# lopunch/CWBNWP-LETKF

Measured on AMD Instinct MI355X. Metric: analysis grid-points/sec (+ wall-clock per cycle) at k=40, 1/2/4/8 MI355X, higher is better.
Workload: dtype f64

## Files before the change

cwbnwp-letkf_amd/csrc/cwbl_abi.hip:

```cpp
#include "../../include/cwb_letkf_core.h"
#include "cwbl_internal.h"

#include <hip/hip_runtime.h>

#include <algorithm>
#include <chrono>
#include <condition_variable>
#include <functional>
#include <mutex>
#include <thread>
#include <cmath>
#include <cstdarg>
#include <cstdio>
#include <cstdlib>
#include <cstring>
#include <memory>
#include <string>
#include <vector>

namespace cwbl {
namespace {

std::string g_err;

// ... 112 lines not shown
      (*fn_)(i);
    }
  }
  void loop(unsigned long seen) {
    for (;;) {
      {
        std::unique_lock<std::mutex> lk(mu_);
        cv_.wait(lk, [&] { return gen_ != seen; });
        seen = gen_;
        if (quit_) return;
      }
      work();
      {
        std::lock_guard<std::mutex> lk(mu_);
        if (--busy_ == 0) done_.notify_all();
      }
    }
  }
  std::vector<std::thread> th_;
  std::mutex mu_;
  std::condition_variable cv_, done_;
  const std::function<void(int)> *fn_ = nullptr;
  int n_ = 0, next_ = 0, busy_ = 0;
  unsigned long gen_ = 0;
  bool quit_ = false;
};

struct ObsType {
  int family = 0, type_id = 0, nvar = 1, nobs = 0;
  std::vector<float> xyz;
  DevBuf obs, error, hdxb, qc;
  DevBuf dxyz;
  bool dxyz_ok = false;
};

struct TreeBufs {
  int entry = -1, dim = 0, depth = 0;
  int bin_div_opt = 0;
  float hinv = 0.0f, vinv = 0.0f;
  DevBuf nodes, rdata, ind, col_bg, col_omm, col_err, col_ok;
  DevBuf bxyz, bstart;
  HostTree host;
  HostBins bins;
  int mode = 0;
  int n = 0, bin_div_used = 0;
  DevBuf ncoord;
  IndexBounds bounds{};
  std::thread worker;
  bool worker_started = false, worker_joined = false, tree_ready = false;
  double worker_ms = 0.0;
  void join() {
    if (worker.joinable()) worker.join();
    worker_joined = worker_started;
  }
  void release() {
    join();
    nodes.release(); rdata.release(); ind.release(); col_bg.release();
    col_omm.release(); col_err.release(); col_ok.release(); bxyz.release(); bstart.release();
    ncoord.release();
  }
  ~TreeBufs() { join(); }
};

enum KernelId {
  KT_SEARCH_BINNED, KT_SEARCH_FLAGGED, KT_SEARCH_TREE, KT_ASSEMBLE_RECORD, KT_SOLVE_TQ40,
  KT_SOLVE_TQ40_MULTI, KT_SOLVE_TQ40_COLUMN, KT_FILL_TQ40_FACTOR, KT_SOLVE_TQ40_FACTOR, KT_SOLVE_TQ_MULTI2, KT_SOLVE_TQ_MULTI4, KT_SOLVE_TQ_MULTI8,
  KT_BIG_HANDOFF, KT_TQB_TAIL, KT_BIG_HANDOFF_MULTI2, KT_BIG_HANDOFF_MULTI4,
  KT_BIG_HANDOFF_MULTI8, KT_TQB_TAIL_MULTI2, KT_TQB_TAIL_MULTI4, KT_TQB_TAIL_MULTI8,
  KT_SOLVE_TQ, KT_SOLVE_TQ_BIG, KT_SOLVE_JACOBI, KT_TUNE_Q,
  KT_COUNT
};
struct KTime { long long launches = 0, points = 0; double ms = 0.0; };

struct RecordKey {
  unsigned long long gen;
  float multi_infl;
  int dims[7];
  cwbl_type_params gts[CWBL_NUM_GTS_TYPES], radar[CWBL_NUM_RADAR_TYPES];
};
struct RecordCache {
  bool valid = false;
  RecordKey key{};
  DevBuf rec, aux, info, sx, sy, salt, flag;
  PinBuf hflag;
  std::vector<std::pair<long long, int>> plan;
  std::vector<size_t> off;
  long long pts = 0;
  size_t nxy = 0, nalt = 0;
  int nt = 0, list_cap = 0;
  long long lz_truncated = 0, q1_undefined = 0;
  size_t bytes() const { return rec.n + aux.n + info.n + sx.n + sy.n + salt.n + flag.n; }
  void release() {
    valid = false;
    for (DevBuf *b : {&rec, &aux, &info, &sx, &sy, &salt, &flag}) b->release();
    hflag.release();
    plan.clear();
    off.clear();
    pts = 0;
  }
};

struct State {
  bool inited = false;
  int k = 0, kp = 0, device = 0, wf = 0, q1_mode = 0;
  int kp_natural = 0;
  float norain = -5.0f;
  size_t ws_bytes = size_t(2) << 30;
  hipStream_t stream = nullptr;
  std::vector<ObsType> obs;
  bool have_obs = false;
  std::vector<std::unique_ptr<TreeBufs>> tree_cache;
  DevBuf tdesc, nbr_cnt, nbr_idx, info, stats;
  DevBuf nbr_cnt2, nbr_idx2;
  hipStream_t sstream = nullptr;
  std::vector<hipEvent_t> cevents;
  int lead_div = 0;
  bool serial_search = false;
  long long max_batch = 160000;
  bool max_batch_set = false;
  long long info_window = 1LL << 25;
  DevBuf sx, sy, salt, svar;
  DevBuf bcol, byo, byb, bxb, bxa, bev, btri;
  DevBuf qxyz, qnf, qidx, qr2;
  DevBuf quad;
  DevBuf wsa;
  DevBuf flags;
  int index_mode = 0;
  DevBuf tdesc_tree;
  DevBuf ix_keys[2], ix_vals[2], ix_hist, ix_part;
  PinBuf ix_pin;
  std::vector<hipEvent_t> pevents;
  bool binned = true;
  int bin_div = 0;
  bool pageable_register = true;
  bool jacobi = false;
  int tq4 = 1;
  long long tq4_sub = 0;
  bool big_split = true;
  long long big_sub = 98304;
  std::vector<hipEvent_t> events;
  hipStream_t h2d = nullptr, d2h = nullptr;
  hipStream_t caller_stream = nullptr;
  hipEvent_t order_ev = nullptr;
  bool ktiming = false;
  KTime ktime[KT_COUNT];
  std::vector<hipEvent_t> kevents;
  int kev_used = 0;
  struct KPend { int id; hipEvent_t e0, e1; long long pts; };
  std::vector<KPend> kpend;
  size_t handoff_budget = 0;
  unsigned long long gen = 0;
  size_t reuse_budget = 0;
  bool factor_reuse = true;
  int column_share = 0;
  int column_levels = 0;
  int ncu = 0;
  RecordCache cache;
  static constexpr int kSlots = 3;
  PinBuf pin_in[kSlots], pin_out[kSlots];
  HostPool pool;
};

State S;

float search_r2() {
  const float gc1999 = 2.0f * std::sqrt(10.0f / 3.0f);
  return gc1999 * gc1999;
}

bool is_gts_assimilated(int id) {
  return id == CWBL_GTS_SYNOP || id == CWBL_GTS_METAR || id == CWBL_GTS_SHIPS ||
         id == CWBL_GTS_SOUND || id == CWBL_GTS_GPSPW;
}

int tree_depth(const HostTree &t, int node = 0) {
  if (t.nodes.empty()) return 0;
  int depth = 0;
  std::vector<std::pair<int, int>> st{{node, 1}};
  while (!st.empty()) {
    auto [nd, lv] = st.back();
    st.pop_back();
    depth = std::max(depth, lv);
    if (t.nodes[nd].cut_dim >= 0) {
      st.push_back({t.nodes[nd].left, lv + 1});
      st.push_back({t.nodes[nd].right, lv + 1});
    }
  }
  return depth;
}

hipError_t stage(DevBuf &dst, const void *src, size_t bytes, int memory) {
  hipError_t e = dst.ensure(bytes);
  if (e != hipSuccess || bytes == 0) return e;
  return hipMemcpyAsync(dst.p, src, bytes,
                        memory == CWBL_MEM_DEVICE ? hipMemcpyDeviceToDevice
                                                  : hipMemcpyHostToDevice,
                        S.stream);
}

hipError_t cevent(int i, hipEvent_t *out) {
  while ((int)S.cevents.size() <= i) {
    hipEvent_t e;
    hipError_t r = hipEventCreateWithFlags(&e, hipEventDisableTiming);
    if (r != hipSuccess) return r;
    S.cevents.push_back(e);
  }
  *out = S.cevents[i];
  return hipSuccess;
}

hipError_t event(int i, hipEvent_t *out) {
  while ((int)S.events.size() <= i) {
    hipEvent_t e;
    hipError_t r = hipEventCreate(&e);
    if (r != hipSuccess) return r;
    S.events.push_back(e);
  }
  *out = S.events[i];
  return hipSuccess;
}

float elapsed(int a, int b) {
  float ms = 0.0f;
  if (hipEventElapsedTime(&ms, S.events[a], S.events[b]) != hipSuccess) return 0.0f;
  return ms;
}

hipError_t kt_event(int i, hipEvent_t *out) {
  while ((int)S.kevents.size() <= i) {
    hipEvent_t e;
    hipError_t r = hipEventCreate(&e);
    if (r != hipSuccess) return r;
    S.kevents.push_back(e);
  }
  *out = S.kevents[i];
  return hipSuccess;
}

hipError_t kt_begin(hipStream_t s, int *ev) {
  *ev = -1;
  if (!S.ktiming) return hipSuccess;
  hipEvent_t e;
  hipError_t r = kt_event(S.kev_used, &e);
  if (r != hipSuccess) return r;
  *ev = S.kev_used;
  S.kev_used += 2;
  return hipEventRecord(e, s);
}

hipError_t kt_end(hipStream_t s, int ev, int id, long long pts) {
  if (ev < 0) return hipSuccess;
  hipEvent_t e;
  hipError_t r = kt_event(ev + 1, &e);
  if (r != hipSuccess) return r;
  S.kpend.push_back({id, S.kevents[ev], e, pts});
  return hipEventRecord(e, s);
}

hipError_t kt_pair(hipStream_t s, hipEvent_t e0, int id0, long long pts0, hipEvent_t e1,
                   int id1, long long pts1, const std::function<hipError_t()> &first,
                   const std::function<hipError_t()> &second) {
  hipError_t r = first();
  if (r != hipSuccess) return r;
  if (S.ktiming) {
    hipEvent_t mid;
    r = kt_event(S.kev_used++, &mid);
    if (r != hipSuccess) return r;
    r = hipEventRecord(mid, s);
    if (r != hipSuccess) return r;
    S.kpend.push_back({id0, e0, mid, pts0});
    S.kpend.push_back({id1, mid, e1, pts1});
  }
  return second();
}

void kt_collect() {
  for (const State::KPend &p : S.kpend) {
    float ms = 0.0f;
    if (hipEventElapsedTime(&ms, p.e0, p.e1) != hipSuccess) continue;
    KTime &t = S.ktime[p.id];
    t.launches += 1;
    t.points += p.pts;
    t.ms += ms;
  }
  S.kpend.clear();
  S.kev_used = 0;
}

std::string kernel_name(int id) {
  const std::string kp = std::to_string(S.kp);
  switch (id) {
    case KT_SEARCH_BINNED: return "search_binned_kernel";
    case KT_SEARCH_FLAGGED: return "search_kernel<FlagQuery>";
    case KT_SEARCH_TREE: return "search_kernel<SlabQuery>";
    case KT_ASSEMBLE_RECORD: return "assemble_record_kernel<" + std::to_string(kRecordWaves) + ">";
    case KT_SOLVE_TQ40: return "solve_tq40_kernel<" + kp + ", 0>";
    case KT_SOLVE_TQ40_MULTI: return "solve_tq40_multi_kernel<" + kp + ">";
    case KT_SOLVE_TQ40_COLUMN: return "solve_tq40_column_kernel<" + kp + ">";
    case KT_FILL_TQ40_FACTOR: return "fill_tq40_factor_kernel<" + kp + ">";
    case KT_SOLVE_TQ40_FACTOR: return "solve_tq40_factor_kernel<" + kp + ">";
    case KT_BIG_HANDOFF:
      return S.kp == 128 ? "solve_tq_rows_kernel<128, 64>"
                         : "solve_tq_big_kernel<" + kp + ", false, " +
                               std::to_string(big_split_j0(S.kp)) + ">";
    case KT_TQB_TAIL:
      return "solve_tqb_tail_kernel<" + kp + ", " + std::to_string(big_split_j0(S.kp)) +
// ... 249 lines not shown
}

int build_family(int family, const cwbl_var_params *vp, std::vector<TreeDesc> &descs,
                 int &list_cap, int &max_depth, std::vector<TreeBufs *> &tbs) {
  struct Pending { int entry; int type_id; const cwbl_type_params *tp; float hinv, vinv; };
  std::vector<Pending> pend;
  const int ntypes = family == 0 ? CWBL_NUM_GTS_TYPES : CWBL_NUM_RADAR_TYPES;
  for (int id = 1; id <= ntypes; ++id) {
    int entry = -1;
    for (size_t e = 0; e < S.obs.size(); ++e)
      if (S.obs[e].family == family && S.obs[e].type_id == id) entry = (int)e;
    if (entry < 0 || S.obs[entry].nobs <= 0) continue;
    if (family == 0 && !is_gts_assimilated(id)) continue;
    const cwbl_type_params *tp = family == 0 ? &vp->gts[id - 1] : &vp->radar[id - 1];
    if (!(tp->use_it && tp->hclr > 0.0f)) continue;
    if (tp->max_lz_pts < 0) return fail(CWBL_ERR_ARG, "max_lz_pts < 0 for type %d", id);
    const float hinv = 1.0f / (tp->hclr * 1e3f);
    const float vinv = tp->vclr > 0.0f ? 1.0f / (tp->vclr * 1e3f) : -1.0f;
    pend.push_back({entry, id, tp, hinv, vinv});
  }
  if (pend.empty()) return CWBL_OK;
  const bool fam3d = pend.back().vinv > 0.0f;
  for (const Pending &pd : pend) {
    ObsType &ot = S.obs[pd.entry];
    const bool own3d = pd.vinv > 0.0f;
    bool dim3 = S.q1_mode == CWBL_Q1_PER_TYPE ? own3d : fam3d;
    int q1u = 0;
    if (dim3 && !own3d) { dim3 = false; q1u = 1; }
    const int n = ot.nobs;
    const int tdim = dim3 ? 3 : 2;
    TreeBufs *tb = nullptr;
    if (S.index_mode == 1) {
      if (int rc = index_entry(pd.entry, tdim, dim3, pd.hinv, pd.vinv, pd.tp->max_lz_pts, tb))
        return rc;
    }
    for (auto &t : S.tree_cache)
      if (S.index_mode == 0 && t->mode == 0 && t->entry == pd.entry && t->dim == tdim &&
          t->hinv == pd.hinv && (!dim3 || t->vinv == pd.vinv) && t->bin_div_opt == S.bin_div)
        tb = t.get();
    if (!tb) {
      std::vector<float> nx(3 * (size_t)n);
      for (int j = 0; j < n; ++j) {
        nx[3 * j + 0] = ot.xyz[3 * j + 0] * pd.hinv;
        nx[3 * j + 1] = ot.xyz[3 * j + 1] * pd.hinv;
        nx[3 * j + 2] = dim3 ? ot.xyz[3 * j + 2] * pd.vinv : -1.0f;
      }
      auto nt = std::make_unique<TreeBufs>();
      nt->entry = pd.entry; nt->dim = tdim; nt->hinv = pd.hinv; nt->vinv = pd.vinv;
      nt->bin_div_opt = S.bin_div;
      nt->n = n;
      const auto t_tree = std::chrono::steady_clock::now();
      build_kdtree(nx.data(), n, tdim, nt->host);
      nt->depth = tree_depth(nt->host);
      P.ms_tree += ms_since(t_tree);
      ++P.trees_built;
      if (nt->depth >= kSearchStackDepth)
        return fail(CWBL_ERR_UNSUPPORTED, "k-d tree too deep (%d obs)", n);
      const HostTree &h = nt->host;
      HIPCHK(nt->nodes.ensure(h.nodes.size() * sizeof(TreeNode)));
      HIPCHK(nt->rdata.ensure(h.rdata.size() * sizeof(float)));
      HIPCHK(nt->ind.ensure(h.ind.size() * sizeof(int) + 4));
      HIPCHK(hipMemcpyAsync(nt->nodes.p, h.nodes.data(), h.nodes.size() * sizeof(TreeNode),
                            hipMemcpyHostToDevice, S.stream));
      HIPCHK(hipMemcpyAsync(nt->rdata.p, h.rdata.data(), h.rdata.size() * sizeof(float),
                            hipMemcpyHostToDevice, S.stream));
      if (!h.ind.empty())
        HIPCHK(hipMemcpyAsync(nt->ind.p, h.ind.data(), h.ind.size() * sizeof(int),
                              hipMemcpyHostToDevice, S.stream));
      const auto t_bins = std::chrono::steady_clock::now();
      build_bins(h, tdim, std::sqrt(search_r2()), nt->bins, bin_div_for(h, tdim));
      P.ms_bins += ms_since(t_bins);
      ++P.bins_built;
      const HostBins &hb = nt->bins;
      HIPCHK(nt->bxyz.ensure(hb.xyzs.size() * sizeof(float) + 16 * kBinPad));
      HIPCHK(nt->bstart.ensure(hb.start.size() * sizeof(int)));
      if (!hb.xyzs.empty())
        HIPCHK(hipMemcpyAsync(nt->bxyz.p, hb.xyzs.data(), hb.xyzs.size() * sizeof(float),
                              hipMemcpyHostToDevice, S.stream));
      HIPCHK(hipMemcpyAsync(nt->bstart.p, hb.start.data(), hb.start.size() * sizeof(int),
                            hipMemcpyHostToDevice, S.stream));
      tb = nt.get();
      S.tree_cache.push_back(std::move(nt));
    }
    const size_t ncol = (size_t)n * ot.nvar;
    HIPCHK(tb->col_bg.ensure(ncol * S.kp * sizeof(float)));
    HIPCHK(tb->col_omm.ensure(ncol * sizeof(float)));
    HIPCHK(tb->col_err.ensure(ncol * sizeof(float)));
    HIPCHK(tb->col_ok.ensure(ncol));
    const cwbl_type_params *tp = pd.tp;
    int is_assim[5] = {0, 0, 0, 0, 0};
    if (family == 0) {
      for (int v = 0; v < ot.nvar; ++v) is_assim[v] = tp->hclr > 0.0f ? tp->is_assim[v] : 0;
    } else {
      is_assim[0] = tp->hclr > 0.0f ? 1 : 0;
    }
    HIPCHK(prep_begin(S.stream, 1));
    HIPCHK(launch_obs_prep(S.stream, S.k, S.kp, family, ot.type_id, ot.nvar, n,
                           ot.obs.as<float>(), ot.error.as<float>(), ot.hdxb.as<float>(),
                           ot.qc.as<int>(), tp->err_muti, tp->err_rej, is_assim, S.norain,
                           tb->mode == 1 ? nullptr : tb->ind.as<int>(), tb->col_bg.as<float>(),
                           tb->col_omm.as<float>(), tb->col_err.as<float>(),
                           tb->col_ok.as<uint8_t>()));
    HIPCHK(prep_end(S.stream));
    TreeDesc d{};
    if (tb->mode == 1) {
      d.rdata = tb->ncoord.as<float4>();
    } else {
      d.nodes = tb->nodes.as<TreeNode>();
      d.rdata = tb->rdata.as<float4>();
      d.ind = tb->ind.as<int>();
    }
    d.col_bg = tb->col_bg.as<float>();
    d.col_omm = tb->col_omm.as<float>();
    d.col_err = tb->col_err.as<float>();
    d.col_ok = tb->col_ok.as<uint8_t>();
    d.hclr_inv = pd.hinv;
    d.vclr_inv = pd.vinv;
    d.tree_dim = dim3 ? 3 : 2;
    d.query3d = own3d ? 1 : 0;
    d.nvar = ot.nvar;
    d.max_lz = tp->max_lz_pts;
    d.list_off = list_cap;
    d.q1_undef = q1u;
    d.bxyz = tb->bxyz.as<float4>();
    d.bstart = tb->bstart.as<int>();
    d.bx0 = tb->bins.x0; d.by0 = tb->bins.y0; d.bz0 = tb->bins.z0; d.binv = tb->bins.binv;
    d.nbx = tb->bins.nbx; d.nby = tb->bins.nby; d.nbz = tb->bins.nbz;
    list_cap += list_span(tp->max_lz_pts);
    if (tb->mode == 0) max_depth = std::max(max_depth, tb->depth);
    descs.push_back(d);
    tbs.push_back(tb);
  }
  return CWBL_OK;
}

void release_obs() {
  for (auto &t : S.tree_cache) t->release();
  S.tree_cache.clear();
  for (auto &o : S.obs) {
    o.obs.release(); o.error.release(); o.hdxb.release(); o.qc.release(); o.dxyz.release();
  }
  S.obs.clear();
  S.have_obs = false;
}

void release_all() {
  release_obs();
  for (hipEvent_t e : S.cevents) (void)hipEventDestroy(e);
  S.cevents.clear();
  for (DevBuf *b : {&S.tdesc, &S.nbr_cnt, &S.nbr_idx, &S.nbr_cnt2, &S.nbr_idx2, &S.info, &S.stats, &S.sx,
                    &S.sy, &S.salt, &S.svar, &S.bcol, &S.byo, &S.byb, &S.bxb, &S.bxa, &S.bev, &S.btri,
                    &S.qxyz, &S.qnf, &S.qidx, &S.qr2, &S.quad, &S.wsa, &S.flags, &S.tdesc_tree,
                    &S.ix_keys[0], &S.ix_keys[1], &S.ix_vals[0], &S.ix_vals[1], &S.ix_hist,
                    &S.ix_part})
    b->release();
  S.ix_pin.release();
  S.cache.release();
  for (hipEvent_t e : S.pevents) (void)hipEventDestroy(e);
  S.pevents.clear();
  g_pspans.clear();
  g_pev_used = 0;
  for (hipEvent_t e : S.events) (void)hipEventDestroy(e);
  S.events.clear();
  for (hipEvent_t e : S.kevents) (void)hipEventDestroy(e);
  S.kevents.clear();
  for (int i = 0; i < State::kSlots; ++i) {
    S.pin_in[i].release();
    S.pin_out[i].release();
  }
  S.pool.stop();
  S.kpend.clear();
  S.kev_used = 0;
  S.ktiming = false;
  for (KTime &t : S.ktime) t = KTime{};
  if (S.order_ev) (void)hipEventDestroy(S.order_ev);
  S.order_ev = nullptr;
  S.caller_stream = nullptr;
  if (S.stream) (void)hipStreamDestroy(S.stream);
  S.stream = nullptr;
  if (S.sstream) (void)hipStreamDestroy(S.sstream);
  S.sstream = nullptr;
  for (hipStream_t *st : {&S.h2d, &S.d2h}) {
    if (*st) (void)hipStreamDestroy(*st);
    *st = nullptr;
  }
  S.inited = false;
}

void select_kp() {
  S.kp = S.kp_natural;
  if ((S.kp == 24 || S.kp == 32) && S.tq4 && !S.jacobi) S.kp = kTq4KP;
}

SolveConsts solve_consts(float inflat, int use_rtpp, float rtpp_a, int use_rtps, float rtps_a) {
  SolveConsts c{};
  c.k = S.k;
  c.kp = S.kp;
  c.weight_function = S.wf;
  c.inflat = inflat;
  c.use_rtpp = use_rtpp;
  c.use_rtps = use_rtps;
  c.rtpp_alpha = rtpp_a;
  c.rtps_alpha = rtps_a;
  c.nmember_inv = 1.0f / (float)S.k;
  c.r2 = search_r2();
  c.max_sweeps = 30;
  c.quad_r = S.quad.as<double2>();
  c.quad = c.quad_r;
#ifdef CWBL_DEBUG_KNOBS
  if (const char *e = std::getenv("CWBL_DEBUG_MAX_SWEEPS")) c.max_sweeps = std::atoi(e);
  if (const char *e = std::getenv("CWBL_DEBUG_TQ_STOP")) c.debug_stop = std::atoi(e);
  if (const char *e = std::getenv("CWBL_DEBUG_TQ_STEPS")) c.debug_steps = std::atoi(e);
#endif
  return c;
}

struct VarCall {
  const cwbl_var_params *vp = nullptr;
  const cwbl_slab *sl = nullptr;
  int nvar = 1;
  bool group = false;
  Tq40Vars tv{};
  long long npts = 0, L = 0;
  SlabDev sd{};
  size_t bvar = 0;
  bool host = false, piped = false, piped_back = false, bounce = false, registered = false;
  std::vector<TreeDesc> descs;
  std::vector<TreeBufs *> tbs;
  bool index1 = false, trees_ready = false;
  int list_cap = 0, max_depth = 1, nt = 0;
  std::vector<std::pair<long long, int>> plan;
  long long B = 0, Bc = 0, info_cap = 0, win0 = 0;
  SolveConsts c{};
  float rbox = 0.0f;
  int ev = 4, cev = 0;
  std::vector<std::pair<int, int>> search_ev, solve_ev;
  std::vector<int> done_ev, h2d_done, d2h_done;
  int reuse = 0;
  long long ncached = 0;
  bool full_hit = false;
  int colshare = 0, nlev = 1, lev = 1;
  long long ncol = 0;
  SlabDev full{};
};

bool record_path() { return S.tq4 && S.kp == kTq4KP && !S.jacobi; }
bool wave_path() { return !record_path() && S.kp <= kMaxWaveKP && !S.jacobi; }
bool handoff_path() {
  return (S.kp == 96 || S.kp == kBigSplitKP) && S.big_split && S.k > big_split_j0(S.kp) + 2;
}

void make_record_key(RecordKey &key, const cwbl_var_params *vp, const cwbl_slab *sl) {
  std::memset(&key, 0, sizeof key);
  key.gen = S.gen;
  key.multi_infl = vp->multi_infl;
  const int dims[7] = {sl->nx, sl->ny, sl->nz, sl->alt_nx, sl->alt_ny, sl->ix_lim, sl->iy_lim};
  std::memcpy(key.dims, dims, sizeof dims);
  std::memcpy(key.gts, vp->gts, sizeof key.gts);
  std::memcpy(key.radar, vp->radar, sizeof key.radar);
}

int coords_match(VarCall &v, bool &same) {
  RecordCache &C = S.cache;
  const auto t0 = std::chrono::steady_clock::now();
  int *flag = C.flag.as<int>();
  HIPCHK(hipMemsetAsync(flag, 0, sizeof(int), S.stream));
  HIPCHK(launch_coord_snapshot(S.stream, false, v.sd.x, C.sx.as<float>(), (long long)C.nxy, flag));
  HIPCHK(launch_coord_snapshot(S.stream, false, v.sd.y, C.sy.as<float>(), (long long)C.nxy, flag));
  HIPCHK(launch_coord_snapshot(S.stream, false, v.sd.alt, C.salt.as<float>(), (long long)C.nalt,
                               flag));
  HIPCHK(hipMemcpyAsync(C.hflag.p, flag, sizeof(int), hipMemcpyDeviceToHost, S.stream));
  HIPCHK(hipStreamSynchronize(S.stream));
  same = *C.hflag.as<int>() == 0;
  R.ms_compare = ms_since(t0);
  return CWBL_OK;
}

int begin_fill(VarCall &v, const RecordKey &key) {
  RecordCache &C = S.cache;
  C.valid = false;
  C.key = key;
  C.plan = v.plan;
  C.off.clear();
  C.pts = 0;
  size_t words = 0;
  for (const auto &b : v.plan) {
    const size_t need = ((size_t)b.second + 1) * AsmRecord<kTq4KP>::WORDS;
    if ((words + need) * sizeof(double) > S.reuse_budget) break;
    C.off.push_back(words);
    words += need;
    C.pts += b.second;
  }
  if (C.off.empty()) return CWBL_OK;
  const cwbl_slab *sl = v.sl;
  C.nxy = (size_t)sl->nx * sl->ny;
  C.nalt = (size_t)sl->alt_nx * sl->alt_ny * sl->nz;
  const size_t need = words * sizeof(double);
  bool ok = need <= C.rec.n ||
            C.rec.ensure(std::min(S.reuse_budget, need + need / 16)) == hipSuccess;
  if (S.factor_reuse) {
    const size_t aneed =
        words / AsmRecord<kTq4KP>::WORDS * FactorAux<kTq4KP>::WORDS * sizeof(double);
    ok = ok && (aneed <= C.aux.n || C.aux.ensure(aneed + aneed / 16) == hipSuccess);
  } else {
    C.aux.release();
  }
  ok = ok && C.info.ensure((size_t)C.pts * sizeof(int2)) == hipSuccess;
  ok = ok && C.sx.ensure(C.nxy * 4) == hipSuccess && C.sy.ensure(C.nxy * 4) == hipSuccess;
  ok = ok && C.salt.ensure(C.nalt * 4) == hipSuccess && C.flag.ensure(sizeof(int)) == hipSuccess;
  ok = ok && C.hflag.ensure(64) == hipSuccess;
  if (!ok) {
    (void)hipGetLastError();
    C.release();
    return CWBL_OK;
  }
  HIPCHK(launch_coord_snapshot(S.stream, true, v.sd.x, C.sx.as<float>(), (long long)C.nxy, nullptr));
  HIPCHK(launch_coord_snapshot(S.stream, true, v.sd.y, C.sy.as<float>(), (long long)C.nxy, nullptr));
  HIPCHK(launch_coord_snapshot(S.stream, true, v.sd.alt, C.salt.as<float>(), (long long)C.nalt,
                               nullptr));
  v.reuse = 1;
  v.ncached = (long long)C.off.size();
  return CWBL_OK;
}

int restore_info(VarCall &v, long long g) {
  const long long n = std::min<long long>(v.info_cap, S.cache.pts - g);
  if (v.reuse != 2 || n <= 0) return CWBL_OK;
  HIPCHK(hipMemcpyAsync(S.info.p, S.cache.info.as<int2>() + g, (size_t)n * sizeof(int2),
                        hipMemcpyDeviceToDevice, S.stream));
  return CWBL_OK;
}

int keep_info(VarCall &v, long long end) {
  const long long n = std::min<long long>(end, S.cache.pts) - v.win0;
  if (v.reuse != 1 || n <= 0) return CWBL_OK;
  HIPCHK(hipMemcpyAsync(S.cache.info.as<int2>() + v.win0, S.info.p, (size_t)n * sizeof(int2),
                        hipMemcpyDeviceToDevice, S.stream));
  return CWBL_OK;
}

int ready_trees(VarCall &v, hipStream_t s) {
  if (v.trees_ready) return CWBL_OK;
  std::vector<TreeDesc> sd = v.descs;
  for (size_t i = 0; i < sd.size(); ++i) {
    TreeBufs *tb = v.tbs[i];
    if (!tb->worker_started) continue;
    if (int rc = ready_tree(tb, s)) return rc;
    sd[i].nodes = tb->nodes.as<TreeNode>();
    sd[i].rdata = tb->rdata.as<float4>();
    sd[i].ind = tb->ind.as<int>();
    v.max_depth = std::max(v.max_depth, tb->depth);
  }
  HIPCHK(S.tdesc_tree.ensure(sd.size() * sizeof(TreeDesc)));
  HIPCHK(hipMemcpyAsync(S.tdesc_tree.p, sd.data(), sd.size() * sizeof(TreeDesc),
                        hipMemcpyHostToDevice, s));
  HIPCHK(hipStreamSynchronize(s));
  v.trees_ready = true;
  return CWBL_OK;
}

int plan_trees(VarCall &v) {
  v.index1 = S.index_mode == 1;
  if (int rc = build_family(0, v.vp, v.descs, v.list_cap, v.max_depth, v.tbs)) return rc;
  if (int rc = build_family(1, v.vp, v.descs, v.list_cap, v.max_depth, v.tbs)) return rc;
  v.nt = (int)v.descs.size();
  if (v.nt == 0 || v.npts == 0) return CWBL_OK;
  HIPCHK(S.tdesc.ensure(v.descs.size() * sizeof(TreeDesc)));
  HIPCHK(hipMemcpyAsync(S.tdesc.p, v.descs.data(), v.descs.size() * sizeof(TreeDesc),
                        hipMemcpyHostToDevice, S.stream));
  if (v.index1 && !S.binned)
    if (int rc = ready_trees(v, S.stream)) return rc;
  return CWBL_OK;
}

int stage_slab(VarCall &v) {
  const cwbl_slab *sl = v.sl;
  v.L = (long long)sl->nx * sl->ny * sl->nz;
  SlabDev &sd = v.sd;
  sd.nx = sl->nx; sd.ny = sl->ny; sd.nz = sl->nz; sd.alt_nx = sl->alt_nx;
  sd.alt_ny = sl->alt_ny; sd.ix_lim = sl->ix_lim; sd.iy_lim = sl->iy_lim; sd.L = v.L;
  const size_t bxy = (size_t)sl->nx * sl->ny * 4;
  const size_t balt = (size_t)sl->alt_nx * sl->alt_ny * sl->nz * 4;
  v.bvar = (size_t)v.L * S.k * 4;
  v.host = sl->memory != CWBL_MEM_DEVICE;
  const bool whole = v.group || v.colshare;
  v.piped = !whole && v.host && sl->ix_lim == sl->nx && sl->iy_lim == sl->ny;
  v.piped_back = v.piped && !v.vp->tune_q;
  v.bounce = !whole && v.host && v.bvar > 0 && !host_pinned(sl->var);
  if (v.bounce && S.pageable_register) {
    if (hipHostRegister(sl->var, v.bvar, hipHostRegisterDefault) == hipSuccess) {
      v.registered = true;
      v.bounce = false;
    } else {
      (void)hipGetLastError();
    }
  }
  if (!v.host) {
    sd.x = sl->x; sd.y = sl->y; sd.alt = sl->alt;
    for (int i = 0; i < v.nvar; ++i) v.tv.var[i] = v.sl[i].var;
  } else {
    HIPCHK(stage(S.sx, sl->x, bxy, CWBL_MEM_HOST));
    HIPCHK(stage(S.sy, sl->y, bxy, CWBL_MEM_HOST));
    HIPCHK(stage(S.salt, sl->alt, balt, CWBL_MEM_HOST));
    sd.x = S.sx.as<float>(); sd.y = S.sy.as<float>(); sd.alt = S.salt.as<float>();
    HIPCHK(S.svar.ensure(v.bvar * (size_t)v.nvar));
    for (int i = 0; i < v.nvar; ++i) {
      v.tv.var[i] = S.svar.as<float>() + (size_t)i * (size_t)v.L * S.k;
      if (v.bvar > 0 && !v.piped && !v.bounce)
        HIPCHK(hipMemcpyAsync(v.tv.var[i], v.sl[i].var, v.bvar, hipMemcpyHostToDevice, S.stream));
    }
  }
  sd.var = v.tv.var[0];
  return CWBL_OK;
}

void plan_batches(VarCall &v) {
  const long long npts = v.npts;
  const size_t per_pt = (size_t)v.list_cap * 4 + (size_t)v.nt * 4 + 8;
  long long B = (long long)(S.ws_bytes / per_pt);
  B = std::min<long long>(B, S.max_batch);
  if (!S.max_batch_set) B = std::min<long long>(B, std::max<long long>(npts / 6, 64000));
  B = std::max<long long>(std::min<long long>(B, npts), 256);
  B = std::min<long long>(B, 1 << 22);
  if (v.list_cap > 0)
    B = std::min<long long>(B, (long long)((((size_t)1 << 32) - 1) / ((size_t)v.list_cap * 4)) /
                                   kListLanes * kListLanes);
  const auto round_up = [](long long x) { return (x + kListLanes - 1) / kListLanes * kListLanes; };
  long long lead = S.lead_div > 0 ? round_up(npts / S.lead_div) : 0;
  if (lead < 4 * kListLanes || lead >= npts) lead = 0;
  if (lead > 0) v.plan.push_back({0, (int)std::min<long long>(lead, B)});
  const long long g1 = v.plan.empty() ? 0 : v.plan[0].second, rest = npts - g1;
  const long long nrest = (rest + B - 1) / B;
  const long long Br = round_up((rest + nrest - 1) / nrest);
  for (long long g = g1; g < npts; g += Br)
    v.plan.push_back({g, (int)std::min<long long>(Br, npts - g)});
  v.B = 0;
  for (const auto &b : v.plan) v.B = std::max<long long>(v.B, b.second);
  v.Bc = std::min<long long>(std::max<long long>(v.B, 1), std::max<long long>(v.L, 1));
  v.info_cap = std::max<long long>(v.B, std::min<long long>(npts, S.info_window));
}

int bounce_whole(VarCall &v, bool up) {
  std::vector<int> evs;
  long long pc0 = 0;
  int pcn = 0;
  const size_t pitch = (size_t)v.L * 4;
  float *const hvar = v.sl->var;
  for (long long c0 = 0, i = 0; c0 < v.L; c0 += v.Bc, ++i) {
    const int cn = (int)std::min<long long>(v.Bc, v.L - c0);
    PinBuf &slot = up ? S.pin_in[i & 1] : S.pin_out[i & 1];
    hipEvent_t e;
    HIPCHK(cevent(v.cev, &e));
    if (up) {
      if (i >= 2) HIPCHK(hipEventSynchronize(S.cevents[evs[(size_t)i - 2]]));
      bounce_rows(S.pool, slot.as<float>(), hvar, v.L, c0, cn, S.k, true);
      HIPCHK(hipMemcpy2DAsync(S.svar.as<float>() + c0, pitch, slot.p, (size_t)cn * 4,
                              (size_t)cn * 4, (size_t)S.k, hipMemcpyHostToDevice, S.stream));
    } else {
      HIPCHK(hipMemcpy2DAsync(slot.p, (size_t)cn * 4, S.svar.as<float>() + c0, pitch,
                              (size_t)cn * 4, (size_t)S.k, hipMemcpyDeviceToHost, S.stream));
    }
    HIPCHK(hipEventRecord(e, S.stream));
    evs.push_back(v.cev++);
    if (!up && i >= 1) {
      HIPCHK(hipEventSynchronize(S.cevents[evs[(size_t)i - 1]]));
      bounce_rows(S.pool, S.pin_out[(i - 1) & 1].as<float>(), hvar, v.L, pc0, pcn, S.k, false);
    }
    pc0 = c0;
    pcn = cn;
  }
  if (!up && !evs.empty()) {
    HIPCHK(hipEventSynchronize(S.cevents[evs.back()]));
    bounce_rows(S.pool, S.pin_out[(evs.size() - 1) & 1].as<float>(), hvar, v.L, pc0, pcn,
                S.k, false);
  }
  return CWBL_OK;
}

int bounce_fill(VarCall &v, long long b) {
  if (b >= State::kSlots) HIPCHK(hipEventSynchronize(S.cevents[v.h2d_done[b - State::kSlots]]));
  bounce_rows(S.pool, S.pin_in[b % State::kSlots].as<float>(), v.sl->var, v.L, v.plan[b].first,
              v.plan[b].second, S.k, true);
  return CWBL_OK;
}

int bounce_drain(VarCall &v, long long b) {
  HIPCHK(hipEventSynchronize(S.cevents[v.d2h_done[b]]));
  bounce_rows(S.pool, S.pin_out[b % State::kSlots].as<float>(), v.sl->var, v.L, v.plan[b].first,
              v.plan[b].second, S.k, false);
  return CWBL_OK;
}

int stage_bounce(VarCall &v) {
  if (v.registered) {
    for (int i = 0; i < State::kSlots; ++i) {
      S.pin_in[i].release();
      S.pin_out[i].release();
    }
  }
  if (!v.bounce) return CWBL_OK;
  const size_t slot_bytes = (size_t)v.Bc * S.k * 4;
  const int nin = v.piped ? State::kSlots : 2, nout = v.piped_back ? State::kSlots : 2;
  for (int i = 0; i < nin; ++i) HIPCHK(S.pin_in[i].ensure(slot_bytes));
  for (int i = 0; i < nout; ++i) HIPCHK(S.pin_out[i].ensure(slot_bytes));
  if (!v.piped) return bounce_whole(v, true);
  return CWBL_OK;
}

int alloc_call_buffers(VarCall &v) {
  const long long B = v.B;
  const size_t bytes_cnt = (size_t)B * v.nt * 4;
  const size_t bytes_idx =
      (size_t)((B + kListLanes - 1) / kListLanes) * kListLanes * std::max(v.list_cap, 1) * 4;
  HIPCHK(S.nbr_cnt.ensure(bytes_cnt));
  HIPCHK(S.nbr_idx.ensure(bytes_idx));
  if (v.plan.size() > 1) {
    HIPCHK(S.nbr_cnt2.ensure(bytes_cnt));
    HIPCHK(S.nbr_idx2.ensure(bytes_idx));
  }
  HIPCHK(S.flags.ensure((size_t)(B + 1) * sizeof(int)));
  HIPCHK(S.stats.ensure(sizeof(DevStats)));
  HIPCHK(hipMemsetAsync(S.stats.p, 0, sizeof(DevStats), S.stream));
  HIPCHK(S.info.ensure((size_t)v.info_cap * sizeof(int2)));
  v.c = solve_consts((float)(S.k - 1) / v.vp->multi_infl,
                     v.vp->use_rtpp, v.vp->rtpp_alpha, v.vp->use_rtps, v.vp->rtps_alpha);
  v.c.ntrees = v.nt;
  v.c.list_cap = v.list_cap;
  v.rbox = std::sqrt(search_r2()) * 1.0001f + 1e-5f;
  return CWBL_OK;
}

int search_batch(VarCall &v, long long bi, int *ncnt, int *nidx, hipEvent_t a, hipEvent_t b) {
  const long long g0 = v.plan[bi].first;
  const int nb = v.plan[bi].second;
  const TreeDesc *dtrees = S.tdesc.as<TreeDesc>();
  DevStats *dst = S.stats.as<DevStats>();
  hipStream_t ss = S.serial_search ? S.stream : S.sstream;
  if (bi >= 2) HIPCHK(hipStreamWaitEvent(ss, S.events[v.done_ev[bi - 2]], 0));
  HIPCHK(hipEventRecord(a, ss));
  int kt;
  if (S.binned) {
    int *fcnt = S.flags.as<int>(), *fidx = fcnt + 1;
    HIPCHK(hipMemsetAsync(fcnt, 0, sizeof(int), ss));
    HIPCHK(kt_begin(ss, &kt));
    HIPCHK(launch_search_binned(ss, dtrees, v.nt, v.list_cap, v.c.r2, v.rbox, v.sd, g0, nb, ncnt,
                                nidx, fcnt, fidx));
    HIPCHK(kt_end(ss, kt, KT_SEARCH_BINNED, nb));
    if (v.index1) {
      HIPCHK(S.ix_pin.ensure(64));
      int *hcnt = S.ix_pin.as<int>();
      HIPCHK(hipMemcpyAsync(hcnt, fcnt, sizeof(int), hipMemcpyDeviceToHost, ss));
      HIPCHK(hipStreamSynchronize(ss));
      if (*hcnt > 0) {
        ++P.flagged_batches;
        if (int rc = ready_trees(v, ss)) return rc;
        HIPCHK(kt_begin(ss, &kt));
        HIPCHK(launch_search_flagged(ss, S.tdesc_tree.as<TreeDesc>(), v.nt, v.max_depth,
                                     v.list_cap, v.c.r2, v.sd, g0, nb, fcnt, fidx, ncnt, nidx,
                                     dst, true));
        HIPCHK(kt_end(ss, kt, KT_SEARCH_FLAGGED, 0));
      }
    } else {
      HIPCHK(kt_begin(ss, &kt));
      HIPCHK(launch_search_flagged(ss, dtrees, v.nt, v.max_depth, v.list_cap, v.c.r2, v.sd, g0,
                                   nb, fcnt, fidx, ncnt, nidx, dst));
      HIPCHK(kt_end(ss, kt, KT_SEARCH_FLAGGED, 0));
    }
  } else if (v.index1) {
    HIPCHK(kt_begin(ss, &kt));
    HIPCHK(launch_search(ss, S.tdesc_tree.as<TreeDesc>(), v.nt, v.max_depth, v.list_cap, v.c.r2,
                         v.sd, g0, nb, ncnt, nidx, nullptr, dst, true));
    HIPCHK(kt_end(ss, kt, KT_SEARCH_TREE, nb));
  } else {
    HIPCHK(kt_begin(ss, &kt));
    HIPCHK(launch_search(ss, dtrees, v.nt, v.max_depth, v.list_cap, v.c.r2, v.sd, g0, nb, ncnt,
                         nidx, nullptr, dst));
    HIPCHK(kt_end(ss, kt, KT_SEARCH_TREE, nb));
  }
  return hipEventRecord(b, ss) == hipSuccess ? CWBL_OK
                                              : fail(CWBL_ERR_HIP, "search event record failed");
}

int upload_batch_var(VarCall &v, long long bi) {
  const long long g0 = v.plan[bi].first;
  const int nb = v.plan[bi].second;
  hipEvent_t hv;
  const int hv_i = v.cev++;
  HIPCHK(cevent(hv_i, &hv));
  const size_t pitch = (size_t)v.L * 4;
  if (v.bounce) {
    if (bi == 0)
      if (int rc = bounce_fill(v, 0)) return rc;
    HIPCHK(hipMemcpy2DAsync(S.svar.as<float>() + g0, pitch, S.pin_in[bi % State::kSlots].p,
                            (size_t)nb * 4, (size_t)nb * 4, (size_t)S.k, hipMemcpyHostToDevice,
                            S.h2d));
  } else {
    HIPCHK(hipMemcpy2DAsync(S.svar.as<float>() + g0, pitch, v.sl->var + g0, pitch,
                            (size_t)nb * 4, (size_t)S.k, hipMemcpyHostToDevice, S.h2d));
  }
  HIPCHK(hipEventRecord(hv, S.h2d));
  v.h2d_done.push_back(hv_i);
  HIPCHK(hipStreamWaitEvent(S.stream, hv, 0));
  return CWBL_OK;
}

int return_batch_var(VarCall &v, long long bi, hipEvent_t dn) {
  const long long g0 = v.plan[bi].first;
  const int nb = v.plan[bi].second;
  HIPCHK(hipStreamWaitEvent(S.d2h, dn, 0));
  const size_t pitch = (size_t)v.L * 4;
  if (v.bounce) {
    hipEvent_t dv;
    const int dv_i = v.cev++;
    HIPCHK(cevent(dv_i, &dv));
    HIPCHK(hipMemcpy2DAsync(S.pin_out[bi % State::kSlots].p, (size_t)nb * 4,
                            S.svar.as<float>() + g0, pitch, (size_t)nb * 4, (size_t)S.k,
                            hipMemcpyDeviceToHost, S.d2h));
    HIPCHK(hipEventRecord(dv, S.d2h));
    v.d2h_done.push_back(dv_i);
  } else {
    HIPCHK(hipMemcpy2DAsync(v.sl->var + g0, pitch, S.svar.as<float>() + g0, pitch,
                            (size_t)nb * 4, (size_t)S.k, hipMemcpyDeviceToHost, S.d2h));
  }
  return CWBL_OK;
}

long long sub_batch(int nb, long long cap) {
  const long long nsub = (nb + cap - 1) / cap;
  const long long Bs = (nb + nsub - 1) / nsub;
  return std::max<long long>(kListLanes, (Bs + kListLanes - 1) / kListLanes * kListLanes);
}

int solve_batch_path(VarCall &v, long long g0, int nb, const int *ncnt, const int *nidx,
                     int2 *infob, hipEvent_t b2, hipEvent_t dn, double *crec = nullptr,
                     bool hit = false, double *caux = nullptr) {
  const TreeDesc *dtrees = S.tdesc.as<TreeDesc>();
  const SolveConsts &c = v.c;
  const SlabDev &sd = v.sd;
  const int nt = v.nt, list_cap = v.list_cap;
  int kt;
  const bool handoff = handoff_path();
  if (record_path()) {
    const long long cap = std::min<long long>(S.tq4_sub > 0 ? S.tq4_sub : nb, 1 << 19);
    const long long Bs = std::min<long long>(sub_batch(nb, cap), 1 << 19);
    if (!crec) HIPCHK(S.wsa.ensure((size_t)(Bs + 1) * 8 * AsmRecord<kTq4KP>::WORDS));
    double *rec = crec ? crec : S.wsa.as<double>();
    const size_t rstep = crec ? AsmRecord<kTq4KP>::WORDS : 0;
    const bool factor = crec && S.factor_reuse && !v.group;
    const int kt_solve = factor ? (hit ? KT_SOLVE_TQ40_FACTOR : KT_FILL_TQ40_FACTOR)
                         : v.group ? KT_SOLVE_TQ40_MULTI : KT_SOLVE_TQ40;
    auto solve = [&](long long g, int n, double *r, int2 *inf) {
      if (factor) {
        double *const ax = caux + (size_t)(r - rec) / rstep * FactorAux<kTq4KP>::WORDS;
        return hit ? launch_solve_tq40_factor(S.stream, S.kp, c, sd, g, n, r, ax, inf)
                   : launch_fill_tq40_factor(S.stream, S.kp, c, sd, g, n, r, ax, inf);
      }
      return v.group ? launch_solve_tq40_multi(S.stream, S.kp, c, sd, v.tv, g, n, r, inf)
                     : launch_solve_tq40(S.stream, S.kp, c, sd, g, n, r, inf);
    };
    if (Bs >= nb && hit) {
      if (S.ktiming) S.kpend.push_back({kt_solve, b2, dn, nb});
      HIPCHK(solve(g0, nb, rec, infob));
      return CWBL_OK;
    }
    if (Bs >= nb) {
      auto asm_ = [&]() {
        return launch_assemble_record(S.stream, S.kp, dtrees, c, sd, g0, nb, ncnt, nidx, infob,
                                      rec);
      };
      auto tq40 = [&]() { return solve(g0, nb, rec, infob); };
      HIPCHK(kt_pair(S.stream, b2, KT_ASSEMBLE_RECORD, nb, dn, kt_solve, nb, asm_, tq40));
      return CWBL_OK;
    }
    for (long long s0 = 0; s0 < nb; s0 += Bs) {
      const int ns = (int)std::min<long long>(Bs, nb - s0);
      double *const srec = rec + (size_t)s0 * rstep;
      if (!hit) {
        HIPCHK(kt_begin(S.stream, &kt));
        HIPCHK(launch_assemble_record(S.stream, S.kp, dtrees, c, sd, g0 + s0, ns,
                                      ncnt + s0 * nt, nidx + s0 * list_cap, infob + s0, srec));
        HIPCHK(kt_end(S.stream, kt, KT_ASSEMBLE_RECORD, ns));
      }
      HIPCHK(kt_begin(S.stream, &kt));
      HIPCHK(solve(g0 + s0, ns, srec, infob + s0));
      HIPCHK(kt_end(S.stream, kt, kt_solve, ns));
    }
    return CWBL_OK;
  }
  if (handoff) {
    const int nv = v.group ? group_var_class(v.nvar) : 1;
    const size_t rec_bytes = 8 * big_handoff_words(S.kp, nv);
// ... 144 lines not shown
      if (n > 1)
        HIPCHK(launch_solve_tq40_multi(S.stream, S.kp, v.c, v.sd, v.tv, g0 + s0, ns, rec, inf));
      else
        HIPCHK(launch_solve_tq40(S.stream, S.kp, v.c, v.sd, g0 + s0, ns, rec, inf));
      HIPCHK(kt_end(S.stream, kt, n > 1 ? KT_SOLVE_TQ40_MULTI : KT_SOLVE_TQ40, (long long)ns * n));
    }
  }
  return CWBL_OK;
}

int finish_call(VarCall &v, cwbl_stats &st) {
  DevStats *dst = S.stats.as<DevStats>();
  if (v.npts > v.win0) {
    HIPCHK(launch_reduce_info(S.stream, S.info.as<int2>(), (int)(v.npts - v.win0), dst));
    if (int rc = keep_info(v, v.npts)) return rc;
  }
  int ev = v.ev;
  for (int i = 0; i < v.nvar; ++i) {
    if (!v.vp[i].tune_q) continue;
    hipEvent_t a, b;
    HIPCHK(event(ev, &a));
    HIPCHK(event(ev + 1, &b));
    HIPCHK(hipEventRecord(a, S.stream));
    SlabDev sdi = v.colshare ? v.full : v.sd;
    sdi.var = v.tv.var[i];
    int kt;
    HIPCHK(kt_begin(S.stream, &kt));
    HIPCHK(launch_tune_q(S.stream, sdi, S.k));
    HIPCHK(kt_end(S.stream, kt, KT_TUNE_Q, v.npts * v.nlev));
    HIPCHK(hipEventRecord(b, S.stream));
    v.solve_ev.push_back({ev, ev + 1});
    ev += 2;
  }
  hipEvent_t e_end, e_back;
  HIPCHK(event(ev, &e_end));
  HIPCHK(event(ev + 1, &e_back));
  if (v.host && !v.piped_back && !v.bounce)
    for (int i = 0; i < v.nvar; ++i)
      HIPCHK(hipMemcpyAsync(v.sl[i].var, v.tv.var[i], v.bvar, hipMemcpyDeviceToHost, S.stream));
  if (v.piped_back) {
    HIPCHK(hipEventRecord(e_back, S.d2h));
    HIPCHK(hipStreamWaitEvent(S.stream, e_back, 0));
  }
  const long long nbat = (long long)v.plan.size();
  if (v.bounce && v.piped_back)
    for (long long bj = std::max<long long>(0, nbat - (State::kSlots - 1)); bj < nbat; ++bj)
      if (int rc = bounce_drain(v, bj)) return rc;
  if (v.bounce && !v.piped_back)
    if (int rc = bounce_whole(v, false)) return rc;
  HIPCHK(hipEventRecord(e_end, S.stream));
  DevStats ds;
  HIPCHK(hipMemcpyAsync(&ds, S.stats.p, sizeof ds, hipMemcpyDeviceToHost, S.stream));
  HIPCHK(hipStreamSynchronize(S.stream));
  kt_collect();
  prep_collect();

  const long long lev = v.nlev;
  st.solved = (long long)ds.solved * lev;
  st.nobs_sum = (long long)ds.nobs_sum * lev;
  st.lz_truncated = v.reuse == 2 ? S.cache.lz_truncated : (long long)ds.lz_truncated * lev;
  st.nonconverged = (long long)ds.nonconverged * lev;
  st.sweeps_sum = (long long)ds.sweeps_sum * lev;
  st.max_p = (int)ds.max_p;
  st.max_sweeps = (int)ds.max_sweeps;
  st.ms_prep = elapsed(0, 1);
  for (auto &p : v.search_ev) st.ms_search += elapsed(p.first, p.second);
  for (auto &p : v.solve_ev) st.ms_solve += elapsed(p.first, p.second);
  st.ms_copy = elapsed(1, 2) + (v.host && !v.piped_back ? elapsed(ev - 1, ev) : 0.0f);
  if (v.bounce) st.ms_copy = g_bounce_ms;
  return CWBL_OK;
}

}

int set_last_error(int code, const char *msg) {
  g_err = msg;
  return code;
}

}

using namespace cwbl;

extern "C" {

int cwbl_abi_version(void) { return CWBL_ABI_VERSION; }

const char *cwbl_last_error(void) { return g_err.c_str(); }

int cwbl_init(const cwbl_init_params *p) {
  if (!p) return fail(CWBL_ERR_ARG, "cwbl_init: null params");
  if (S.inited) release_all();
  if (p->nmember < 2) return fail(CWBL_ERR_ARG, "nmember must be >= 2 (got %d)", p->nmember);
  const int kp = supported_kp(p->nmember);
  if (kp < 0)
    return fail(CWBL_ERR_UNSUPPORTED, "nmember %d > %d not supported by this build",
                p->nmember, CWBL_MAX_MEMBERS);
  int ndev = 0;
  if (hipGetDeviceCount(&ndev) != hipSuccess || ndev == 0)
    return fail(CWBL_ERR_NO_DEVICE, "no HIP device available (the core has no CPU path)");
  int dev = p->device;
  if (dev < 0) HIPCHK(hipGetDevice(&dev));
  if (dev >= ndev) return fail(CWBL_ERR_NO_DEVICE, "device %d >= device count %d", dev, ndev);
  HIPCHK(hipSetDevice(dev));
  hipDeviceProp_t prop;
  HIPCHK(hipGetDeviceProperties(&prop, dev));
  if (std::strncmp(prop.gcnArchName, "gfx950", 6) != 0)
    return fail(CWBL_ERR_NO_DEVICE, "device %d is %s; this library is built for gfx950", dev,
                prop.gcnArchName);
  if (p->weight_function != 0 && p->weight_function != 1)
    return fail(CWBL_ERR_ARG, "weight_function must be 0 or 1");
  S.k = p->nmember;
  S.kp = kp;
  S.device = dev;
  S.wf = p->weight_function;
  S.norain = p->norain_value;
  S.q1_mode = p->q1_mode;
  S.ws_bytes = p->workspace_bytes ? p->workspace_bytes : (size_t(2) << 30);
  size_t fr = 0, tot = 0;
  HIPCHK(hipMemGetInfo(&fr, &tot));
  if (p->workspace_bytes) {
    S.handoff_budget = p->workspace_bytes;
  } else {
    S.handoff_budget = std::min<size_t>((size_t)13 << 30, fr / 10 * 4);
  }
  S.reuse_budget = std::min<size_t>((size_t)40 << 30, fr / 10 * 4);
  ++S.gen;
  HIPCHK(hipStreamCreateWithFlags(&S.stream, hipStreamNonBlocking));
  HIPCHK(hipStreamCreateWithFlags(&S.sstream, hipStreamNonBlocking));
  HIPCHK(hipStreamCreateWithFlags(&S.h2d, hipStreamNonBlocking));
  HIPCHK(hipStreamCreateWithFlags(&S.d2h, hipStreamNonBlocking));
  {
    std::vector<double2> tab((size_t)4 * kQuadLevels * kQuadStride);
    const int rounds[4] = {2, 3, 4, 8};
    for (int r = 0; r < 4; ++r)
      for (int l = 1; l <= kQuadLevels; ++l)
        quad_table(l, &tab[((size_t)r * kQuadLevels + (l - 1)) * kQuadStride],
                   8 * rounds[r] - 1);
    HIPCHK(S.quad.ensure(tab.size() * sizeof(double2)));
    HIPCHK(hipMemcpy(S.quad.p, tab.data(), tab.size() * sizeof(double2), hipMemcpyHostToDevice));
  }
  S.jacobi = false;
  S.tq4 = 1;
  S.tq4_sub = 0;
  S.big_split = true;
  S.big_sub = 98304;
  S.binned = true;
  S.pageable_register = true;
  S.bin_div = 0;
  S.index_mode = 0;
  S.column_share = 0;
  S.column_levels = 0;
  S.factor_reuse = true;
  S.ncu = prop.multiProcessorCount;
  std::memset(&P, 0, sizeof P);
  std::memset(&CI, 0, sizeof CI);
  S.lead_div = 0;
  S.serial_search = false;
#ifdef CWBL_DEBUG_KNOBS
  if (const char *e = std::getenv("CWBL_DEBUG_SERIAL")) S.serial_search = std::atoi(e) != 0;
#endif
  S.kp_natural = kp;
  select_kp();
  S.max_batch = 160000;
  S.max_batch_set = false;
  S.info_window = 1LL << 25;
  S.inited = true;
  return CWBL_OK;
}

int cwbl_set_option(int option, long long value) {
  if (!S.inited) return fail(CWBL_ERR_STATE, "cwbl_set_option before cwbl_init");
  auto range = [&](long long lo, long long hi) { return value >= lo && value <= hi; };
  ++S.gen;
  switch (option) {
    case CWBL_OPT_SOLVER:
      if (!range(0, 1)) break;
      if (value == 1 && S.kp_natural > kMaxWaveKP)
        return fail(CWBL_ERR_UNSUPPORTED, "the Jacobi solver supports k <= %d", kMaxWaveKP);
      S.jacobi = value == 1;
      select_kp();
      return CWBL_OK;
    case CWBL_OPT_SPLIT40:
      if (!range(0, 1)) break;
      S.tq4 = (int)value;
      select_kp();
      return CWBL_OK;
    case CWBL_OPT_SPLIT40_BATCH:
      if (!range(0, 1 << 19)) break;
      S.tq4_sub = value;
      return CWBL_OK;
    case CWBL_OPT_SEARCH:
      if (!range(0, 1)) break;
      S.binned = value == 0;
      return CWBL_OK;
    case CWBL_OPT_BIG_PATH:
      if (!range(0, 1)) break;
      S.big_split = value == 1;
      return CWBL_OK;
    case CWBL_OPT_BIG_BATCH:
      if (!range(64, 1LL << 24)) break;
      S.big_sub = value;
      return CWBL_OK;
    case CWBL_OPT_PAGEABLE:
      if (!range(0, 1)) break;
      S.pageable_register = value == 0;
      return CWBL_OK;
    case CWBL_OPT_BIN_DIV:
      if (!range(0, 8)) break;
      S.bin_div = (int)value;
      return CWBL_OK;
    case CWBL_OPT_LEAD_DIV:
      if (!range(0, 1 << 20)) break;
      S.lead_div = (int)value;
      return CWBL_OK;
    case CWBL_OPT_MAX_BATCH:
      if (value != 0 && !range(256, 1LL << 31)) break;
      S.max_batch = value ? value : 160000;
      S.max_batch_set = value != 0;
      return CWBL_OK;
    case CWBL_OPT_INFO_WINDOW:
      if (value != 0 && !range(256, 1LL << 30)) break;
      S.info_window = value ? value : (1LL << 25);
      return CWBL_OK;
    case CWBL_OPT_INDEX:
      if (!range(0, 1)) break;
      S.index_mode = (int)value;
      return CWBL_OK;
    case CWBL_OPT_COLUMN_SHARE:
      if (!range(0, 2)) break;
      S.column_share = (int)value;
      return CWBL_OK;
    case CWBL_OPT_COLUMN_LEVELS:
      if (!range(0, 1 << 30)) break;
      S.column_levels = (int)value;
      return CWBL_OK;
    case CWBL_OPT_RECORD_REUSE:
      if (!range(0, 1LL << 24)) break;
      S.reuse_budget = (size_t)value << 20;
      S.cache.release();
      return CWBL_OK;
    case CWBL_OPT_FACTOR_REUSE:
      if (!range(0, 1)) break;
      S.factor_reuse = value == 1;
      return CWBL_OK;
    default:
      return fail(CWBL_ERR_ARG, "cwbl_set_option: unknown option %d", option);
  }
  return fail(CWBL_ERR_ARG, "cwbl_set_option: value %lld out of range for option %d", value,
              option);
}

int cwbl_set_stream(void *stream) {
  if (int rc = require_device()) return rc;
  S.caller_stream = static_cast<hipStream_t>(stream);
  return CWBL_OK;
}

int cwbl_set_kernel_timing(int enable) {
  if (int rc = require_device()) return rc;
  S.ktiming = enable != 0;
  for (KTime &t : S.ktime) t = KTime{};
  return CWBL_OK;
}

int cwbl_kernel_times(cwbl_kernel_time *out, int cap, int *n) {
  if (int rc = require_device()) return rc;
  if (!n || cap < 0 || (cap > 0 && !out)) return fail(CWBL_ERR_ARG, "cwbl_kernel_times: bad arguments");
  int m = 0;
  for (int id = 0; id < KT_COUNT; ++id) {
    const KTime &t = S.ktime[id];
    if (t.launches == 0) continue;
    if (m < cap) {
      cwbl_kernel_time &o = out[m];
      std::memset(&o, 0, sizeof o);
      std::snprintf(o.name, sizeof o.name, "%s", kernel_name(id).c_str());
      o.launches = t.launches;
      o.points = t.points;
      o.ms = t.ms;
    }
    ++m;
  }
  *n = m;
  return CWBL_OK;
}

int cwbl_reuse_info(cwbl_reuse_info_t *out) {
  if (int rc = require_device()) return rc;
  if (!out) return fail(CWBL_ERR_ARG, "cwbl_reuse_info: null argument");
  *out = R;
  return CWBL_OK;
}

int cwbl_column_info(cwbl_column_info_t *out) {
  if (int rc = require_device()) return rc;
  if (!out) return fail(CWBL_ERR_ARG, "cwbl_column_info: null argument");
  *out = CI;
  return CWBL_OK;
}

int cwbl_finalize(void) {
  if (S.inited) {
    (void)hipStreamSynchronize(S.stream);
    release_all();
  }
  return CWBL_OK;
}

int cwbl_set_obs(const cwbl_obs_set *o) {
  if (int rc = require_device()) return rc;
  if (!o) return fail(CWBL_ERR_ARG, "null obs set");
  if (o->n_gts < 0 || o->n_radar < 0 || (o->n_gts && !o->gts) || (o->n_radar && !o->radar))
    return fail(CWBL_ERR_ARG, "bad obs set counts/pointers");
  release_obs();
  ++S.gen;
  const int mem = o->memory;
  if (mem == CWBL_MEM_DEVICE) HIPCHK(order_after_caller());
  const size_t k = (size_t)S.k;
  bool seen_g[CWBL_NUM_GTS_TYPES + 1] = {}, seen_r[CWBL_NUM_RADAR_TYPES + 1] = {};
  for (int e = 0; e < o->n_gts; ++e) {
    const cwbl_gts_obs &g = o->gts[e];
    if (g.type_id < 1 || g.type_id > CWBL_NUM_GTS_TYPES || seen_g[g.type_id])
      return fail(CWBL_ERR_ARG, "gts entry %d: bad or duplicate type_id %d", e, g.type_id);
    if (g.nvar < 1 || g.nvar > CWBL_MAX_NVAR || g.nobs < 0)
      return fail(CWBL_ERR_ARG, "gts type %d: bad nvar/nobs", g.type_id);
    if (g.nobs > 0 && (!g.xyz || !g.obs || !g.error || !g.hdxb || !g.qc))
      return fail(CWBL_ERR_ARG, "gts type %d: null array", g.type_id);
    seen_g[g.type_id] = true;
    S.obs.emplace_back();
    ObsType &t = S.obs.back();
    t.family = 0; t.type_id = g.type_id; t.nvar = g.nvar; t.nobs = g.nobs;
    const size_t n = (size_t)g.nobs, nv = (size_t)g.nvar;
    t.xyz.resize(3 * n);
    if (n) {
      if (mem == CWBL_MEM_DEVICE)
        HIPCHK(hipMemcpyAsync(t.xyz.data(), g.xyz, 3 * n * 4, hipMemcpyDeviceToHost, S.stream));
      else
        std::memcpy(t.xyz.data(), g.xyz, 3 * n * 4);
    }
    HIPCHK(stage(t.obs, g.obs, n * nv * 4, mem));
    HIPCHK(stage(t.error, g.error, n * nv * 4, mem));
    HIPCHK(stage(t.hdxb, g.hdxb, n * nv * k * 4, mem));
    HIPCHK(stage(t.qc, g.qc, n * nv * k * 4, mem));
  }
  for (int e = 0; e < o->n_radar; ++e) {
    const cwbl_radar_obs &r = o->radar[e];
    if (r.type_id < 1 || r.type_id > CWBL_NUM_RADAR_TYPES || seen_r[r.type_id])
      return fail(CWBL_ERR_ARG, "radar entry %d: bad or duplicate type_id %d", e, r.type_id);
    if (r.nobs < 0) return fail(CWBL_ERR_ARG, "radar type %d: bad nobs", r.type_id);
    if (r.nobs > 0 && (!r.xyz || !r.obs || !r.hdxb))
      return fail(CWBL_ERR_ARG, "radar type %d: null array", r.type_id);
    seen_r[r.type_id] = true;
    S.obs.emplace_back();
    ObsType &t = S.obs.back();
    t.family = 1; t.type_id = r.type_id; t.nvar = 1; t.nobs = r.nobs;
    const size_t n = (size_t)r.nobs;
    t.xyz.resize(3 * n);
    if (n) {
      if (mem == CWBL_MEM_DEVICE)
        HIPCHK(hipMemcpyAsync(t.xyz.data(), r.xyz, 3 * n * 4, hipMemcpyDeviceToHost, S.stream));
      else
        std::memcpy(t.xyz.data(), r.xyz, 3 * n * 4);
    }
    HIPCHK(stage(t.obs, r.obs, n * 4, mem));
    HIPCHK(stage(t.hdxb, r.hdxb, n * k * 4, mem));
  }
  HIPCHK(hipStreamSynchronize(S.stream));
  S.have_obs = true;
  return CWBL_OK;
}

static int check_slab(const cwbl_var_params *vp, const cwbl_slab *sl) {
  if (!vp || !sl) return fail(CWBL_ERR_ARG, "null argument");
  if (sl->nx < 0 || sl->ny < 0 || sl->nz < 0 || sl->ix_lim < 0 || sl->iy_lim < 0 ||
      sl->ix_lim > sl->nx || sl->iy_lim > sl->ny || sl->ix_lim > sl->alt_nx ||
      sl->iy_lim > sl->alt_ny)
    return fail(CWBL_ERR_ARG, "slab bounds: nx=%d ny=%d ix_lim=%d iy_lim=%d alt=%dx%d",
                sl->nx, sl->ny, sl->ix_lim, sl->iy_lim, sl->alt_nx, sl->alt_ny);
  if (!(vp->multi_infl > 0.0f)) return fail(CWBL_ERR_ARG, "multi_infl must be > 0");
  const long long npts = (long long)sl->ix_lim * sl->iy_lim * sl->nz;
  if (npts >= (1LL << 32))
    return fail(CWBL_ERR_ARG, "slab of %lld points: at most 2^32 - 1 per call", npts);
  return CWBL_OK;
}

static int begin_call(const cwbl_slab *sl) {
  if (sl->memory == CWBL_MEM_DEVICE) HIPCHK(order_after_caller());
  S.kpend.clear();
  S.kev_used = 0;
  g_bounce_ms = 0.0;
  std::memset(&P, 0, sizeof P);
  std::memset(&R, 0, sizeof R);
  std::memset(&CI, 0, sizeof CI);
  g_pspans.clear();
  g_pev_used = 0;
  return CWBL_OK;
}

static int analyze_call(VarCall &v, cwbl_stats *stats) {
  const cwbl_var_params *vp = v.vp;
  const cwbl_slab *sl = v.sl;
  if (int rc = begin_call(sl)) return rc;
  const auto t_start = std::chrono::steady_clock::now();
  cwbl_stats st;
  std::memset(&st, 0, sizeof st);
  const long long npts = (long long)sl->ix_lim * sl->iy_lim * sl->nz;
  st.points = v.npts = npts;
  RecordCache &C = S.cache;
  auto finish = [&]() {
    R.bytes_held = (long long)C.bytes();
    st.ms_total =
        std::chrono::duration<double, std::milli>(std::chrono::steady_clock::now() - t_start).count();
    if (stats) *stats = st;
    return CWBL_OK;
  };
  struct Unregister {
    VarCall &v;
    ~Unregister() {
      if (!v.registered) return;
      (void)hipStreamSynchronize(S.h2d);
      (void)hipStreamSynchronize(S.d2h);
      (void)hipStreamSynchronize(S.stream);
      (void)hipGetLastError();
      (void)hipHostUnregister(v.sl->var);
    }
  } unreg{v};

  hipEvent_t e0, e1, e2, e_ready;
  HIPCHK(event(0, &e0));
  HIPCHK(hipEventRecord(e0, S.stream));
  CI.reason = column_reason(v);
  const bool col_candidate = CI.reason == CWBL_COLUMN_SHARED;
  const bool reuse_on =
      !v.group && !col_candidate && record_path() && S.reuse_budget > 0 && npts > 0;
  RecordKey key;
  bool staged = false;
  if (reuse_on) {
    make_record_key(key, vp, sl);
    if (C.valid && std::memcmp(&key, &C.key, sizeof key) == 0) {
      if (int rc = stage_slab(v)) return rc;
      staged = true;
      bool same = false;
      if (int rc = coords_match(v, same)) return rc;
      if (same) {
        v.reuse = 2;
        v.ncached = (long long)C.off.size();
        v.full_hit = C.off.size() == C.plan.size();
      }
    }
    if (v.reuse != 2) C.valid = false;
  }
  if (v.full_hit) {
    v.nt = C.nt;
    v.list_cap = C.list_cap;
  } else if (int rc = plan_trees(v)) {
    return rc;
  }
  st.ntrees = v.nt;
  if (v.nt == 0 || npts == 0) {
    if (col_candidate) CI.reason = CWBL_COLUMN_REASON_NO_TREES;
    HIPCHK(hipStreamSynchronize(S.stream));
    prep_collect();
    return finish();
  }
  for (const TreeDesc &d : v.descs) st.q1_undefined += d.q1_undef ? npts : 0;
  if (v.full_hit) st.q1_undefined = C.q1_undefined;
  for (const TreeDesc &d : v.descs) {
    if (CI.reason == CWBL_COLUMN_SHARED && (d.tree_dim != 2 || d.query3d))
      CI.reason = CWBL_COLUMN_REASON_3D;
    if ((CI.reason == CWBL_COLUMN_SHARED || CI.reason == CWBL_COLUMN_REASON_3D) && d.q1_undef)
      CI.reason = CWBL_COLUMN_REASON_Q1;
  }
  if (CI.reason == CWBL_COLUMN_SHARED) v.colshare = S.column_share;
  HIPCHK(event(1, &e1));
  HIPCHK(hipEventRecord(e1, S.stream));
  HIPCHK(event(2, &e2));
  if (!staged)
    if (int rc = stage_slab(v)) return rc;
  HIPCHK(hipEventRecord(e2, S.stream));
  if (v.colshare) {
    v.full = v.sd;
    v.sd.nz = 1;
    v.nlev = sl->nz;
    v.npts = v.ncol = (long long)sl->ix_lim * sl->iy_lim;
    CI.shared = 1;
    CI.columns = v.ncol;
    CI.levels = v.nlev;
  }
  plan_batches(v);
  if (v.reuse == 2 && v.plan != C.plan)
    return fail(CWBL_ERR_STATE, "record reuse: the batch plan changed under an equal key");
  if (int rc = stage_bounce(v)) return rc;
  if (int rc = alloc_call_buffers(v)) return rc;
  if (reuse_on && v.reuse != 2)
    if (int rc = begin_fill(v, key)) return rc;
  if (int rc = restore_info(v, 0)) return rc;
  HIPCHK(event(3, &e_ready));
  HIPCHK(hipEventRecord(e_ready, S.stream));
  HIPCHK(hipStreamWaitEvent(S.sstream, e_ready, 0));

  const long long nbat = (long long)v.plan.size();
  for (long long bi = 0; bi < nbat; ++bi) {
    const long long g0 = v.plan[bi].first;
    const int nb = v.plan[bi].second;
    if (g0 + nb - v.win0 > v.info_cap) {
      HIPCHK(launch_reduce_info(S.stream, S.info.as<int2>(), (int)(g0 - v.win0),
                                S.stats.as<DevStats>()));
      if (int rc = keep_info(v, g0)) return rc;
      v.win0 = g0;
      if (int rc = restore_info(v, g0)) return rc;
    }
    int2 *const infob = S.info.as<int2>() + (g0 - v.win0);
    int *ncnt = (bi & 1) ? S.nbr_cnt2.as<int>() : S.nbr_cnt.as<int>();
    int *nidx = (bi & 1) ? S.nbr_idx2.as<int>() : S.nbr_idx.as<int>();
    const int ev = v.ev;
    hipEvent_t a, b, b2, dn;
    HIPCHK(event(ev, &a));
    HIPCHK(event(ev + 1, &b));
    HIPCHK(event(ev + 2, &b2));
    HIPCHK(event(ev + 3, &dn));
    double *const crec = bi < v.ncached ? C.rec.as<double>() + C.off[bi] : nullptr;
    const size_t aoff =
        crec ? C.off[bi] / AsmRecord<kTq4KP>::WORDS * FactorAux<kTq4KP>::WORDS : 0;
    double *const caux = crec && S.factor_reuse ? C.aux.as<double>() + aoff : nullptr;
    const bool hit = crec && v.reuse == 2;
    if (!hit) {
      if (int rc = search_batch(v, bi, ncnt, nidx, a, b)) return rc;
      HIPCHK(hipStreamWaitEvent(S.stream, b, 0));
    }
    if (v.piped)
      if (int rc = upload_batch_var(v, bi)) return rc;
    HIPCHK(hipEventRecord(b2, S.stream));
    if (v.colshare) {
      if (int rc = solve_batch_column(v, g0, nb, ncnt, nidx, infob, b2, dn)) return rc;
    } else if (int rc = solve_batch_path(v, g0, nb, ncnt, nidx, infob, b2, dn, crec, hit,
                                       caux)) {
      return rc;
    }
    HIPCHK(hipEventRecord(dn, S.stream));
    if (v.piped_back)
      if (int rc = return_batch_var(v, bi, dn)) return rc;
    if (v.bounce && v.piped) {
      if (bi + 1 < nbat)
        if (int rc = bounce_fill(v, bi + 1)) return rc;
      if (v.piped_back && bi >= State::kSlots - 1)
        if (int rc = bounce_drain(v, bi - (State::kSlots - 1))) return rc;
    }
    if (!hit) v.search_ev.push_back({ev, ev + 1});
    v.solve_ev.push_back({ev + 2, ev + 3});
    v.done_ev.push_back(ev + 3);
    v.ev += 4;
  }
  if (int rc = finish_call(v, st)) return rc;
  if (v.reuse == 1) {
    C.nt = v.nt;
    C.list_cap = v.list_cap;
    C.lz_truncated = st.lz_truncated;
    C.q1_undefined = st.q1_undefined;
    C.valid = true;
  }
  R.batches_reused = v.reuse == 2 ? v.ncached : 0;
  R.batches_assembled = nbat - R.batches_reused;
  return finish();
}

int cwbl_analyze_var(const cwbl_var_params *vp, const cwbl_slab *sl, cwbl_stats *stats) {
  if (int rc = require_device()) return rc;
  if (!S.have_obs) return fail(CWBL_ERR_STATE, "cwbl_set_obs has not been called");
  if (int rc = check_slab(vp, sl)) return rc;
  VarCall v;
  v.vp = vp;
  v.sl = sl;
  return analyze_call(v, stats);
}

static int check_group(int nvar, const cwbl_var_params *vp, const cwbl_slab *sl) {
  if (nvar < 1 || nvar > CWBL_MAX_GROUP_VARS)
    return fail(CWBL_ERR_ARG, "cwbl_analyze_vars: nvar = %d, must be 1..%d", nvar,
                CWBL_MAX_GROUP_VARS);
  if (int rc = check_slab(vp, sl)) return rc;
  const cwbl_slab &s0 = sl[0];
  const size_t bvar = (size_t)s0.nx * s0.ny * s0.nz * (size_t)S.k * sizeof(float);
  for (int i = 1; i < nvar; ++i) {
    const cwbl_slab &s = sl[i];
    const struct { const char *name; bool same; } f[] = {
        {"nx", s.nx == s0.nx}, {"ny", s.ny == s0.ny}, {"nz", s.nz == s0.nz},
        {"alt_nx", s.alt_nx == s0.alt_nx}, {"alt_ny", s.alt_ny == s0.alt_ny},
        {"ix_lim", s.ix_lim == s0.ix_lim}, {"iy_lim", s.iy_lim == s0.iy_lim},
        {"memory", s.memory == s0.memory}, {"x (pointer)", s.x == s0.x},
        {"y (pointer)", s.y == s0.y}, {"alt (pointer)", s.alt == s0.alt},
        {"multi_infl", std::memcmp(&vp[i].multi_infl, &vp[0].multi_infl, sizeof(float)) == 0},
        {"gts", std::memcmp(vp[i].gts, vp[0].gts, sizeof vp[0].gts) == 0},
        {"radar", std::memcmp(vp[i].radar, vp[0].radar, sizeof vp[0].radar) == 0}};
    for (const auto &e : f)
      if (!e.same)
        return fail(CWBL_ERR_ARG, "cwbl_analyze_vars: variable %d differs from variable 0 in %s",
                    i, e.name);
  }
  for (int i = 0; i < nvar; ++i)
    for (int j = i + 1; j < nvar && bvar > 0; ++j) {
      const uintptr_t a = (uintptr_t)sl[i].var, b = (uintptr_t)sl[j].var;
      if (a < b + bvar && b < a + bvar)
        return fail(CWBL_ERR_ARG, "cwbl_analyze_vars: the var arrays of variables %d and %d overlap",
                    i, j);
    }
  return CWBL_OK;
}

int cwbl_analyze_vars(int nvar, const cwbl_var_params *vp, const cwbl_slab *slabs,
                      cwbl_stats *stats) {
  if (int rc = require_device()) return rc;
  if (!S.have_obs) return fail(CWBL_ERR_STATE, "cwbl_set_obs has not been called");
  if (int rc = check_group(nvar, vp, slabs)) return rc;
  if (record_path() || ((wave_path() || (handoff_path() && !S.jacobi)) && nvar > 1)) {
    VarCall v;
    v.vp = vp;
    v.sl = slabs;
    v.nvar = nvar;
    v.group = true;
    v.tv.nvar = nvar;
    for (int i = 0; i < nvar; ++i) {
      v.tv.use_rtpp[i] = vp[i].use_rtpp;
      v.tv.use_rtps[i] = vp[i].use_rtps;
      v.tv.rtpp_alpha[i] = vp[i].rtpp_alpha;
      v.tv.rtps_alpha[i] = vp[i].rtps_alpha;
    }
    return analyze_call(v, stats);
  }
  const auto t_start = std::chrono::steady_clock::now();
  cwbl_stats st;
  std::memset(&st, 0, sizeof st);
  for (int i = 0; i < nvar; ++i) {
    cwbl_stats si;
    if (int rc = cwbl_analyze_var(&vp[i], &slabs[i], &si)) return rc;
    if (i == 0) {
      st = si;
    } else {
      st.ms_prep += si.ms_prep;
      st.ms_search += si.ms_search;
      st.ms_solve += si.ms_solve;
      st.ms_copy += si.ms_copy;
    }
  }
  st.ms_total =
      std::chrono::duration<double, std::milli>(std::chrono::steady_clock::now() - t_start).count();
  if (stats) *stats = st;
  return CWBL_OK;
}

int cwbl_solve_batch(int npts, const long long *col_off, const float *yo, const float *yb,
                     const float *xb, float inflat, int use_rtpp, float rtpp_alpha,
                     int use_rtps, float rtps_alpha, float *xa, double *evals, int memory) {
  if (int rc = require_device()) return rc;
  if (npts < 0 || (npts > 0 && (!col_off || !xb || !xa)))
    return fail(CWBL_ERR_ARG, "cwbl_solve_batch: bad arguments");
  if (npts == 0) return CWBL_OK;
  const size_t k = (size_t)S.k;
  std::vector<long long> hoff;
  const long long *doff = col_off;
  long long ncol;
  if (memory == CWBL_MEM_DEVICE) {
    HIPCHK(order_after_caller());
    HIPCHK(hipMemcpyAsync(&ncol, col_off + npts, 8, hipMemcpyDeviceToHost, S.stream));
    HIPCHK(hipStreamSynchronize(S.stream));
  } else {
    ncol = col_off[npts];
    for (int i = 0; i < npts; ++i)
      if (col_off[i + 1] < col_off[i]) return fail(CWBL_ERR_ARG, "col_off not monotone");
  }
  if (ncol > 0 && (!yo || !yb)) return fail(CWBL_ERR_ARG, "cwbl_solve_batch: null yo/yb");
  const float *dyo = yo, *dyb = yb, *dxb = xb;
  float *dxa = xa;
  double *dev = evals;
  if (memory != CWBL_MEM_DEVICE) {
    HIPCHK(stage(S.bcol, col_off, (size_t)(npts + 1) * 8, memory));
    HIPCHK(stage(S.byo, yo, (size_t)ncol * 4, memory));
    HIPCHK(stage(S.byb, yb, (size_t)ncol * k * 4, memory));
    HIPCHK(stage(S.bxb, xb, (size_t)npts * k * 4, memory));
    HIPCHK(S.bxa.ensure((size_t)npts * k * 4));
    if (evals) HIPCHK(S.bev.ensure((size_t)npts * k * 8));
    doff = S.bcol.as<long long>(); dyo = S.byo.as<float>(); dyb = S.byb.as<float>();
    dxb = S.bxb.as<float>(); dxa = S.bxa.as<float>(); dev = evals ? S.bev.as<double>() : nullptr;
  }
  HIPCHK(S.info.ensure((size_t)npts * sizeof(int2)));
  SolveConsts c = solve_consts(inflat, use_rtpp, rtpp_alpha, use_rtps, rtps_alpha);
  const bool jacobi = S.jacobi && S.kp <= kMaxWaveKP;
  double *tri = nullptr;
  if (dev && !jacobi) {
    HIPCHK(S.btri.ensure((size_t)npts * 2 * S.kp * sizeof(double)));
    tri = S.btri.as<double>();
  }
  if (S.kp > kMaxWaveKP)
    HIPCHK(launch_solve_tq_big(S.stream, S.kp, true, nullptr, c, SlabDev{}, 0, npts, nullptr,
                               nullptr, doff, dyo, dyb, dxb, dxa, S.info.as<int2>(), tri));
  else if (jacobi)
    HIPCHK(launch_solve_assembled(S.stream, S.kp, c, npts, doff, dyo, dyb, dxb, dxa, dev,
                                  S.info.as<int2>()));
  else
    HIPCHK(launch_solve_tq(S.stream, S.kp, true, nullptr, c, SlabDev{}, 0, npts, nullptr,
                           nullptr, doff, dyo, dyb, dxb, dxa, S.info.as<int2>(), tri));
  if (tri) HIPCHK(launch_tridiag_eigvals(S.stream, S.kp, S.k, npts, tri, dev));
// ... 237 lines not shown
```

cwbnwp-letkf_amd/csrc/cwbl_internal.h:

```cpp
#pragma once

#include <hip/hip_runtime.h>

#include <cstddef>
#include <cstdint>
#include <vector>

namespace cwbl {

struct TreeNode {
  float cut_val, cut_val_left, cut_val_right;
  int   cut_dim;
  float lo[3];
  float hi[3];
  int   left, right;
  int   l, u;
  int   pad_[2];
};
static_assert(sizeof(TreeNode) == 64, "TreeNode layout");

struct HostTree {
  int dim = 3;
  int n = 0;
  std::vector<TreeNode> nodes;
// ... 37 lines not shown
  float x0, y0, z0, binv;
  int nbx, nby, nbz;
};
constexpr int kIndexBoundWords = 12;
struct IndexBounds {
  float lo[3], hi[3];
  float alo[3], ahi[3];
  bool aseen;
};
int index_bound_blocks(int n);
int index_sort_blocks(int n);
hipError_t launch_index_normalize(hipStream_t s, const float *xyz, int n, int dim, float hinv,
                                  float vinv, float4 *ncoord, float *part);
void index_finish_bounds(const float *part, int nblocks, IndexBounds &b);
hipError_t launch_index_sort(hipStream_t s, int n, int ncell, const float4 *ncoord, int dim,
                             IndexGrid g, int *keys[2], int *vals[2], int *hist, int *which);
hipError_t launch_index_finish(hipStream_t s, const float4 *ncoord, int n, int ncell,
                               const int *skeys, const int *svals, float4 *bxyz, int *bstart);

struct SolveConsts {
  int   k;
  int   kp;
  int   ntrees;
  int   list_cap;
  int   weight_function;
  int   use_rtpp, use_rtps;
  float inflat, rtpp_alpha, rtps_alpha;
  float nmember_inv;
  float r2;
  int   max_sweeps;
  const double2 *quad;
  const double2 *quad_r;
  int   debug_stop;
  int   debug_steps;
};
#ifdef CWBL_DEBUG_KNOBS
#define CWBL_DBG_STOP(c) ((c).debug_stop)
#define CWBL_DBG_STEPS(c) ((c).debug_steps)
#else
#define CWBL_DBG_STOP(c) 0
#define CWBL_DBG_STEPS(c) 0
#endif

constexpr int kQuadNodes = 31;
constexpr int kQuadLevels = 24;
constexpr int kQuadLevels31 = 12;
constexpr int kQuadStride = 64;
void quad_table(int level, double2 *out64, int nodes = kQuadNodes);
__host__ __device__ constexpr int quad_rounds(int level) {
  return level <= 3 ? 2 : level <= 5 ? 3 : level <= kQuadLevels31 ? 4 : 8;
}
__host__ __device__ constexpr int quad_passes(int level) { return level <= kQuadLevels31 ? 1 : 2; }
__host__ __device__ inline const double2 *quad_rule(const double2 *quad_r, int R, int level) {
  return quad_r + ((size_t)(R == 8 ? 3 : R - 2) * kQuadLevels + (level - 1)) * kQuadStride;
}

struct SlabDev {
  int nx, ny, nz, alt_nx, alt_ny, ix_lim, iy_lim;
  long long L;
  const float *x, *y, *alt;
  float *var;
};

struct DevStats {
  unsigned long long solved, nobs_sum, lz_truncated, nonconverged, q1_undefined, sweeps_sum;
  unsigned int max_p, max_sweeps;
};

hipError_t launch_obs_prep(hipStream_t s, int k, int kp, int family, int type_id, int nvar,
                           int nobs, const float *obs, const float *error, const float *hdxb,
                           const int *qc, const float err_muti[5], const float err_rej[5],
                           const int is_assim[5], float norain, const int *slot_obs,
                           float *col_bg, float *col_omm, float *col_err, uint8_t *col_ok);

constexpr int kMaxRankDim = 64;
struct Decomp {
  int nx, ny, nz, px, py;
  int cols_before[kMaxRankDim];
  int rows_before[kMaxRankDim];
};
void make_decomp(Decomp &d, int nx, int ny, int nz, int px, int py);
hipError_t launch_pack_columns(hipStream_t s, const float *global, const Decomp &d,
                               float *send);
hipError_t launch_unpack_columns(hipStream_t s, const float *recv, const Decomp &d,
                                 float *global);
hipError_t launch_transpose_columns(hipStream_t s, bool unpack, const float *src,
                                    long long sstride, int nm, const Decomp &d, float *dst,
                                    long long dstride);
hipError_t launch_vcoord_mean(hipStream_t s, const float *ph, long long n2d, int nz_ph, int k,
                              int stagger, float alpha, float *alt);
hipError_t launch_member_sum(hipStream_t s, const float *fields, long long n, int nm,
                             float *out);
hipError_t launch_scale(hipStream_t s, float *x, long long n, float alpha);

hipError_t launch_tune_q(hipStream_t st, SlabDev s, int k);

hipError_t launch_search(hipStream_t s, const TreeDesc *trees, int ntrees, int depth,
                         int list_cap, float r2, SlabDev slab, long long g0, int npts,
                         int *nbr_cnt, int *nbr_idx, float *nbr_r2, DevStats *stats,
                         bool obs_slots = false);

hipError_t launch_solve_neighbors(hipStream_t s, int kp, const TreeDesc *trees,
                                  SolveConsts c, SlabDev slab, long long g0, int npts,
                                  const int *nbr_cnt, const int *nbr_idx, int2 *info);

hipError_t launch_solve_assembled(hipStream_t s, int kp, SolveConsts c, int npts,
                                  const long long *col_off, const float *yo, const float *yb,
                                  const float *xb, float *xa, double *evals, int2 *info);

hipError_t launch_solve_tq(hipStream_t s, int kp, bool assembled, const TreeDesc *trees,
                           SolveConsts c, SlabDev slab, long long g0, int npts,
                           const int *nbr_cnt, const int *nbr_idx,
                           const long long *col_off, const float *yo, const float *yb,
                           const float *xb, float *xa, int2 *info, double *tri = nullptr);

constexpr int kTq4KP = 40;

constexpr int kTq40J0 = 8;
constexpr int kRecordWaves = 4;
template <int KP>
struct AsmRecord {
  static constexpr int TA = 0;
  static constexpr int U1 = KP * (KP + 1) / 2;
  static constexpr int WORDS = (U1 + KP + 1) / 2 * 2;
};
template <int KP>
struct FactorRecord {
  static constexpr int D = 0;
  static constexpr int U1 = KP;
  static constexpr int COL = 2 * KP;
  static constexpr int col(int j) { return COL + j * (KP - 1) - j * (j - 1) / 2; }
  static constexpr int EL = col(KP - 2);
  static constexpr int WORDS = EL + 1;
};
static_assert(FactorRecord<kTq4KP>::WORDS == AsmRecord<kTq4KP>::WORDS,
              "a factor takes its record's slot");
template <int KP>
struct FactorAux {
  static constexpr int B = 0;
  static constexpr int T = KP;
  static constexpr int WORDS = 2 * KP;
};
hipError_t launch_assemble_record(hipStream_t s, int kp, const TreeDesc *trees, SolveConsts c,
                                  SlabDev slab, long long g0, int npts, const int *nbr_cnt,
                                  const int *nbr_idx, int2 *info, double *ws);
hipError_t launch_solve_tq40(hipStream_t s, int kp, SolveConsts c, SlabDev slab, long long g0,
                             int npts, double *ws, int2 *info);
hipError_t launch_fill_tq40_factor(hipStream_t s, int kp, SolveConsts c, SlabDev slab,
                                   long long g0, int npts, double *ws, double *aux, int2 *info);
hipError_t launch_solve_tq40_factor(hipStream_t s, int kp, SolveConsts c, SlabDev slab,
                                    long long g0, int npts, const double *ws, const double *aux,
                                    int2 *info);

constexpr int kMaxGroupVars = 8;
struct Tq40Vars {
  float *var[kMaxGroupVars];
  float rtpp_alpha[kMaxGroupVars], rtps_alpha[kMaxGroupVars];
  int use_rtpp[kMaxGroupVars], use_rtps[kMaxGroupVars];
  int nvar;
};
hipError_t launch_solve_tq40_multi(hipStream_t s, int kp, SolveConsts c, SlabDev slab,
                                   const Tq40Vars &vars, long long g0, int npts, double *ws,
                                   int2 *info);

hipError_t launch_solve_tq40_column(hipStream_t s, int kp, SolveConsts c, SlabDev slab,
                                    long long g0, int npts, int nz, int lw, double *ws,
                                    int2 *info);

constexpr int group_var_class(int nvar) { return nvar <= 2 ? 2 : nvar <= 4 ? 4 : 8; }
hipError_t launch_solve_tq_multi(hipStream_t s, int kp, const TreeDesc *trees, SolveConsts c,
                                 SlabDev slab, const Tq40Vars &vars, long long g0, int npts,
                                 const int *nbr_cnt, const int *nbr_idx, int2 *info);

constexpr int kBigSplitKP = 128;
constexpr int kBigJ0 = 64;
constexpr int big_split_j0(int kp) { return kp - 64; }
template <int KP, int J0>
struct BigHandoff {
  static constexpr int KT = KP - J0;
  static constexpr int TA = 0;
  static constexpr int HV = TA + KT * KT;
  static constexpr int D = HV + J0 * KP;
  static constexpr int E = D + J0;
  static constexpr int TAU = E + J0;
  static constexpr int U1 = TAU + J0;
  static constexpr int U2 = U1 + KP;
  static constexpr int BT = U2 + KP;
  static constexpr int WORDS = BT + KT * KT;
};
hipError_t launch_big_handoff(hipStream_t s, int kp, const TreeDesc *trees, SolveConsts c,
                              SlabDev slab, long long g0, int npts, const int *nbr_cnt,
                              const int *nbr_idx, int2 *info, double *ws);
hipError_t launch_rows_handoff(hipStream_t s, const TreeDesc *trees, SolveConsts c, SlabDev slab,
                               long long g0, int npts, const int *nbr_cnt, const int *nbr_idx,
                               int2 *info, double *ws);
hipError_t launch_solve_tqb_tail(hipStream_t s, int kp, SolveConsts c, SlabDev slab,
                                 long long g0, int npts, double *ws, int2 *info);

template <int KP, int J0, int NV>
struct BigHandoffMulti : BigHandoff<KP, J0> {
  using Base = BigHandoff<KP, J0>;
  static constexpr int U2X = Base::WORDS;
  static constexpr int WORDS = U2X + (NV - 1) * KP;
  __host__ __device__ static constexpr int u2(int i) { return i == 0 ? Base::U2 : U2X + (i - 1) * KP; }
};
constexpr size_t big_handoff_words(int kp, int nv) {
  return (size_t)(kp == 96 ? BigHandoff<96, 32>::WORDS : BigHandoff<kBigSplitKP, kBigJ0>::WORDS) +
         (size_t)(nv > 1 ? nv - 1 : 0) * kp;
}
hipError_t launch_big_handoff_multi(hipStream_t s, int kp, const TreeDesc *trees, SolveConsts c,
                                    SlabDev slab, const Tq40Vars &vars, long long g0, int npts,
                                    const int *nbr_cnt, const int *nbr_idx, int2 *info,
                                    double *ws);
hipError_t launch_rows_handoff_multi(hipStream_t s, const TreeDesc *trees, SolveConsts c,
                                     SlabDev slab, const Tq40Vars &vars, long long g0, int npts,
                                     const int *nbr_cnt, const int *nbr_idx, int2 *info,
                                     double *ws);
hipError_t launch_solve_tqb_tail_multi(hipStream_t s, int kp, SolveConsts c, SlabDev slab,
                                       const Tq40Vars &vars, long long g0, int npts, double *ws,
                                       int2 *info);

hipError_t launch_solve_tq_big(hipStream_t s, int kp, bool assembled, const TreeDesc *trees,
                               SolveConsts c, SlabDev slab, long long g0, int npts,
                               const int *nbr_cnt, const int *nbr_idx,
                               const long long *col_off, const float *yo, const float *yb,
                               const float *xb, float *xa, int2 *info, double *tri = nullptr);

hipError_t launch_tridiag_eigvals(hipStream_t s, int kp, int k, int npts, const double *tri,
                                  double *evals);

hipError_t launch_search_binned(hipStream_t s, const TreeDesc *trees, int ntrees, int list_cap,
                                float r2, float rbox, SlabDev slab, long long g0, int npts,
                                int *nbr_cnt, int *nbr_idx, int *flag_cnt, int *flag_idx);
hipError_t launch_search_flagged(hipStream_t s, const TreeDesc *trees, int ntrees, int depth,
                                 int list_cap, float r2, SlabDev slab, long long g0, int npts,
                                 const int *flag_cnt, const int *flag_idx, int *nbr_cnt,
                                 int *nbr_idx, DevStats *stats, bool obs_slots = false);

hipError_t launch_search_single(hipStream_t s, const TreeDesc *tree, int depth, float r2,
                                int nq, const float *q_xyz, int max_lz, int *nfound, int *idx,
                                float *r2out);

hipError_t launch_reduce_info(hipStream_t s, const int2 *info, int n, DevStats *stats);

hipError_t launch_coord_snapshot(hipStream_t s, bool store, const float *cur, float *snap,
                                 long long n, int *flag);

constexpr int kSearchStackDepth = 40;

constexpr int kListLanes = 64;
constexpr int kListGroup = 4;
constexpr int kBinPad = 8;
__host__ __device__ inline int list_span(int max_lz) {
  return (max_lz + kListGroup - 1) / kListGroup * kListGroup;
}
__host__ __device__ inline long long list_index(long long g, int cap, int off) {
  return (g / kListLanes) * (long long)cap * kListLanes + (long long)off * kListLanes +
         (g % kListLanes) * kListGroup;
}
__host__ __device__ inline unsigned list_slot(int s) {
  return (unsigned)s / kListGroup * (kListGroup * kListLanes) + (unsigned)s % kListGroup;
}

int supported_kp(int k);
int set_last_error(int code, const char *msg);
constexpr int kMaxWaveKP = 64;

}
```

cwbnwp-letkf_amd/csrc/cwbl_tq40_fill.hip:

```cpp
#include "cwbl_tq40_common.h"

#include <utility>

namespace cwbl {

namespace {

__device__ __forceinline__ void rsum16x2(double &a, double &b) {
  double ab[2] = {a, b};
  rsum16xN(ab);
  a = ab[0];
  b = ab[1];
}

__device__ __forceinline__ void touch(double &x) { asm volatile("" : "+v"(x)); }
__device__ __forceinline__ int touched(int x) {
  asm volatile("" : "+v"(x));
  return x;
}
__device__ __forceinline__ long long touched(long long x) {
  asm volatile("" : "+v"(x));
  return x;
}

template <int KP>
__device__ __forceinline__ void tq40_load_xb(const SlabDev &slab, const long long g0,
                                             const bool valid, const int gi, const int l,
                                             const int k, float (&xv)[Tq40Layout<KP>::NV]) {
  const float *__restrict__ const var = slab.var;
  const long long P = tq40_var_index(slab, g0, valid ? gi : 0);
  sfor<Tq40Layout<KP>::NV>([&](auto vv) {
    constexpr int vs = decltype(vv)::value;
    const int i = tq40_vrow<KP>(l, vs);
    xv[vs] = var[P + slab.L * ((valid && i < k) ? i : 0)];
  });
}

template <int KP, bool AHEAD>
__device__ __forceinline__ void tq40_factor_solve(
    const SolveConsts &c, const SlabDev &slab, Tq40Smem<KP> &sm,
    double (&A)[Tq40Layout<KP>::NS][KP], const float (&xbv)[Tq40Layout<KP>::NV], const long long g0,
    const bool valid, const int ptot, const int gi, const int q, const int l,
    int2 *__restrict__ info) {
  using LY = Tq40Layout<KP>;
  constexpr int J0 = LY::J0, KT = LY::KT, NS = LY::NS, NV = LY::NV, H = LY::H;
  using SM = Tq40Smem<KP>;
  const int k = c.k;
  const int lp = l < J0 ? l : 0;
  const bool pre = l < J0;
  auto vrow = [&](int vs) { return tq40_vrow<KP>(l, vs); };
  int *const pkeep = reinterpret_cast<int *>(&sm.tq[q][KP][3]);
  *pkeep = ptot;
  const double trace = tq40_trace(sm, q, l, k);

  const double m = (double)c.inflat;
  const double ratio = trace / m - (double)(k - 1);
  int level = 1;
  double dec = 10.0;
  while (level < kQuadLevels && dec < ratio) {
    dec *= 10.0;
    ++level;
  }
  const int R = tq40_wave_rounds(level);
  const int NQ = 8 * R - 1;
  const double2 *qtab = quad_rule(c.quad_r, R, level);
  double2 twn;
  if constexpr (AHEAD) twn = qtab[min(l & 7, NQ - 1)];
  const int side = l >> 3, n8 = l & 7;
  const double(*T)[4] = sm.tq[q];
  char *const smb = reinterpret_cast<char *>(&sm);
  auto lds = [&](unsigned off) { return *reinterpret_cast<const double *>(smb + off); };
  auto sts = [&](unsigned off, double v) { *reinterpret_cast<double *>(smb + off) = v; };
  const unsigned tq0 = (unsigned)(offsetof(SM, tq) + (size_t)q * sizeof(sm.tq[0])) +
                       (side ? (KP - 1) * 32u : 0u);
  const unsigned dirb = side ? (unsigned)-32 : 32u;
  const unsigned csb = side ? 40u : 8u;
  const unsigned qs0 = (unsigned)(offsetof(SM, qs) + (size_t)q * sizeof(sm.qs[0])) +
                       (side ? (KP - H) * 8u : (H - 1) * 8u);
  const unsigned qz0 = (unsigned)(offsetof(SM, qz) + (size_t)q * sizeof(sm.qz[0]));
  const unsigned bdir = side ? 8u : (unsigned)-8;
  const double sk = sqrt((double)(k - 1));
  auto touch_cols = [&]() {
    sfor<KT - 2>([&](auto jj) {
      constexpr int jl = decltype(jj)::value, J1 = jl + 1, R1 = J1 / 16;
      sfor<NS>([&](auto rr) {
        constexpr int r = decltype(rr)::value;
        if constexpr (16 * r + 15 > J1 || r == R1) touch(A[r][J0 + jl]);
      });
    });
  };

  float *__restrict__ const var = slab.var;
  const int use_rtpp = c.use_rtpp, use_rtps = c.use_rtps;
  const float rtpp_alpha = c.rtpp_alpha, rtps_alpha = c.rtps_alpha;

  float xbl[NV];
  double xb_mean;
  {
    sfor<NV>([&](auto vv) {
      constexpr int vs = decltype(vv)::value;
      const bool mem = valid && vrow(vs) < k;
      xbl[vs] = mem ? xbv[vs] : 0.0f;
    });
    xb_mean = (double)(seq_sum_f32<KP>(xbl) * c.nmember_inv);
  }
  double uxP = pre && l < k ? (double)xbl[0] - xb_mean : 0.0, ux[NS];
  sfor<NS>([&](auto rr) {
    constexpr int r = decltype(rr)::value;
    const int t = J0 + l + 16 * r;
    ux[r] = t < k ? (double)xbl[r + 1] - xb_mean : 0.0;
  });

  sfor<J0>([&](auto jj) {
    constexpr int j = decltype(jj)::value, J1 = j + 1;
    const double *pj = sm.pv[q][j];
    const double scal = pj[0], tau = sm.tau[q][j];
    double u2a;
    if constexpr (J1 < J0) u2a = rbcast<J1>(uxP);
    else u2a = rbcast<0>(ux[0]);
    const double xP = (pre && l > J1) ? pj[lp] : 0.0;
    double x[NS], xu = xP * uxP;
    sfor<NS>([&](auto rr) {
      constexpr int r = decltype(rr)::value;
      x[r] = pj[J0 + l + 16 * r];
      xu = fma(x[r], ux[r], xu);
    });
    xu = rsum16(xu);
    const double xsP = xP * scal;
    const double vP = (pre && l == J1) ? 1.0 : xsP;
    const double s2 = fma(scal, xu, u2a);
    uxP = fma(-tau * s2, vP, uxP);
    sfor<NS>([&](auto rr) {
      constexpr int r = decltype(rr)::value;
      const double xs = x[r] * scal;
      double vr;
      if constexpr (J1 == J0 && r == 0) vr = l == 0 ? 1.0 : xs;
      else vr = xs;
      ux[r] = fma(-tau * s2, vr, ux[r]);
    });
  });
  sfor<KT - 2>([&](auto jj) {
    constexpr int jl = decltype(jj)::value, j = J0 + jl;
    constexpr int J1 = jl + 1, R1 = J1 / 16, L1 = J1 % 16;
    sfor<NS>([&](auto rr) {
      constexpr int r = decltype(rr)::value;
      if constexpr (16 * r + 15 > J1 || r == R1) touch(A[r][j]);
    });
    const double scal = rbcast<L1>(A[R1][j]), tau = sm.tau[q][j];
    double x[NS], xu = 0.0;
    sfor<NS>([&](auto rr) {
      constexpr int r = decltype(rr)::value;
      if constexpr (16 * r + 15 > J1) {
        const int t = l + 16 * r;
        if constexpr (r == R1) x[r] = t == J1 ? 0.0 : A[r][j];
        else x[r] = A[r][j];
        xu = fma(x[r], ux[r], xu);
      } else {
        x[r] = 0.0;
      }
    });
    xu = rsum16(xu);
    const double s2 = fma(scal, xu, rbcast<L1>(ux[R1]));
    sfor<NS>([&](auto rr) {
      constexpr int r = decltype(rr)::value;
      const int t = l + 16 * r;
      const double xs = x[r] * scal;
      const double vr = t == J1 ? 1.0 : xs;
      ux[r] = fma(-tau * s2, vr, ux[r]);
    });
  });
  if (pre) sm.tq[q][l][3] = uxP;
  sfor<NS>([&](auto rr) {
    constexpr int r = decltype(rr)::value;
    sm.tq[q][J0 + l + 16 * r][3] = ux[r];
  });
  __syncthreads();

  double ys[NV], z[NV];
  sfor<NV>([&](auto vv) { ys[decltype(vv)::value] = 0.0; });
  for (int round = 0; round < R; ++round) {
    const int node = 8 * round + n8;
    double2 tw;
    if constexpr (AHEAD) {
      tw = twn;
      if (round + 1 < R) twn = qtab[min(node + 8, NQ - 1)];
    } else {
      tw = qtab[min(node, NQ - 1)];
    }
    const double sigma = node < NQ ? m * tw.x : 0.0;
    const double omega = node < NQ ? sqrt(m) * tw.y : 1.0;
    double hh[H], mm[H];
    unsigned pw = tq0;
    double dl = lds(pw) + sigma, gt = lds(pw + 24);
    double nd, nc, ng;
    auto next_row = [&]() {
      pw += dirb;
      nd = lds(pw);
      nc = lds(pw + csb);
      ng = lds(pw + 24);
    };
    if constexpr (AHEAD) next_row();
    sfor<H - 1>([&](auto tt) {
      constexpr int t = decltype(tt)::value + 1;
      if constexpr (!AHEAD) {
        asm volatile("" : "+v"(pw) : "v"(dl));
        next_row();
      }
      const double dt = nd, ct = nc, g = ng;
      if constexpr (AHEAD && t < H - 1) {
        asm volatile("" : "+v"(pw) : "v"(dl));
        next_row();
      }
      const double rdl = rcp64(dl);
      const double lt = ct * rdl;
      hh[t - 1] = gt * rdl;
      mm[t - 1] = lt;
      dl = fma(-lt, ct, dt + sigma);
      gt = fma(-lt, gt, g);
    });
    const double cm = T[H][1];
    const double dlo = ror8(dl), go = ror8(gt);
    double xv = (gt * dlo - cm * go) / fma(dl, dlo, -cm * cm);
    const bool last = round == R - 1;
    const bool zlane = last && n8 == 7;
    const double om = zlane ? 0.0 : omega;
    unsigned ps = qs0;
    unsigned pz = qz0 + (zlane ? qs0 - (unsigned)offsetof(SM, qs) - (unsigned)q * KP * 8u
                               : KP * 8u);
    const unsigned zdir = zlane ? bdir : 0u;
    auto emit = [&](double x) {
      double s = om * x;
      s += dpp_f64<0xB1>(s);
      s += dpp_f64<0x4E>(s);
      s += dpp_f64<0x141>(s);
      sts(ps, s);
      sts(pz, x);
    };
    emit(xv);
    sfor<H - 1>([&](auto tt) {
      constexpr int t = H - 2 - decltype(tt)::value;
      xv = fma(-mm[t], xv, hh[t]);
      ps += bdir;
      pz += zdir;
      asm volatile("" : "+v"(ps), "+v"(pz) : "v"(xv));
      emit(xv);
    });
    __syncthreads();
    sfor<NV>([&](auto vv) {
      constexpr int vs = decltype(vv)::value;
      const int i = vrow(vs);
      const int ic = i < KP ? i : 0;
      ys[vs] += i < KP ? sm.qs[q][ic] : 0.0;
      if (last) z[vs] = i < KP ? sm.qz[q][ic] : 0.0;
    });
    __syncthreads();
  }
  double dpart = 0.0;
  sfor<NV>([&](auto vv) {
    constexpr int vs = decltype(vv)::value;
    const int i = vrow(vs);
    const double u1 = sm.tq[q][i < KP ? i : 0][2];
    dpart = i < KP ? fma(u1, z[vs], dpart) : dpart;
  });
  const double d = rsum16(dpart);

  double y[NV];
  sfor<NV>([&](auto vv) { y[decltype(vv)::value] = ys[decltype(vv)::value]; });
  touch_cols();
  const int lb = touched(l);
  sfor<KT - 2>([&](auto jj) {
    constexpr int jl = KT - 3 - decltype(jj)::value, j = J0 + jl, J1 = jl + 1;
    constexpr int R1 = J1 / 16, L1 = J1 % 16;
    const double tj = sm.tau[q][j];
    const double scal = rbcast<L1>(A[R1][j]);
    double vv[NS], a = 0.0;
    sfor<NS>([&](auto rr) {
      constexpr int r = decltype(rr)::value;
      if constexpr (16 * r + 15 >= J1) {
        const int t = lb + 16 * r;
        if constexpr (16 * r + 15 > J1) vv[r] = t == J1 ? 1.0 : A[r][j] * scal;
        else vv[r] = t == J1 ? 1.0 : 0.0;
        a = fma(vv[r], y[r + 1], a);
      } else {
        vv[r] = 0.0;
      }
    });
    a = rsum16(a);
    sfor<NS>([&](auto rr) {
      constexpr int r = decltype(rr)::value;
      if constexpr (16 * r + 15 >= J1) y[r + 1] = fma(-tj * a, vv[r], y[r + 1]);
    });
  });
  sfor<J0>([&](auto jj) {
    constexpr int j = J0 - 1 - decltype(jj)::value, J1 = j + 1;
    const double tj = sm.tau[q][j];
    const double *pj = sm.pv[q][j];
    const double scal = pj[0];
    const double v0 = lb == J1 ? 1.0 : (lb < J0 && lb > J1) ? pj[lb] * scal : 0.0;
    double vv[NS];
    double a = v0 * y[0];
    sfor<NS>([&](auto rr) {
      constexpr int r = decltype(rr)::value;
      const double pr = pj[J0 + lb + 16 * r] * scal;
      if constexpr (J1 == J0 && r == 0) vv[r] = lb == 0 ? 1.0 : pr;
      else vv[r] = pr;
      a = fma(vv[r], y[r + 1], a);
    });
    a = rsum16(a);
    y[0] = fma(-tj * a, v0, y[0]);
    sfor<NS>([&](auto rr) {
      constexpr int r = decltype(rr)::value;
      y[r + 1] = fma(-tj * a, vv[r], y[r + 1]);
    });
  });

  float xa[NV];
  sfor<NV>([&](auto vv) {
    constexpr int vs = decltype(vv)::value;
    xa[vs] = vrow(vs) < k ? (float)(xb_mean + (d + sk * y[vs])) : 0.0f;
  });
  if (use_rtpp || use_rtps) {
    const float xa_mean = seq_sum_f32<KP>(xa) * c.nmember_inv;
    double xpl[NV];
    float xap[NV];
    sfor<NV>([&](auto vv) {
      constexpr int vs = decltype(vv)::value;
      const bool mem = vrow(vs) < k;
      xpl[vs] = mem ? (double)xbl[vs] - xb_mean : 0.0;
      xap[vs] = 0.0f;
      if (mem) {
        xap[vs] = xa[vs] - xa_mean;
        if (use_rtpp)
          xap[vs] = (float)((double)((1.0f - rtpp_alpha) * xap[vs]) +
                            (double)rtpp_alpha * xpl[vs]);
      }
    });
    if (use_rtps) {
      double d8 = 0.0, sq8[NV];
      sfor<NV>([&](auto vv) {
        constexpr int vs = decltype(vv)::value;
        sq8[vs] = xpl[vs] * xpl[vs];
        dpp_pin(sq8[vs]);
      });
      sfor<KP>([&](auto mm) {
        constexpr int mb = decltype(mm)::value;
        constexpr int vs = mb < J0 ? 0 : 1 + (mb - J0) / 16, ln = mb < J0 ? mb : (mb - J0) % 16;
        d8 = fmac_row<ln>(d8, sq8[vs], 1.0);
      });
      const float xb_std = (float)d8;
      float sq[NV];
      sfor<NV>([&](auto vv) {
        constexpr int vs = decltype(vv)::value;
        sq[vs] = xap[vs] * xap[vs];
      });
      const float xa_std = seq_sum_f32<KP>(sq);
      const float f = rtps_alpha * sqrtf(xb_std / xa_std) - rtps_alpha + 1.0f;
      sfor<NV>([&](auto vv) { xap[decltype(vv)::value] = xap[decltype(vv)::value] * f; });
    }
    sfor<NV>([&](auto vv) { xa[decltype(vv)::value] = xa_mean + xap[decltype(vv)::value]; });
  }
  const int pt = *pkeep;
  if (valid && pt > 0) {
    const long long P = tq40_var_index(slab, g0, touched(gi));
    sfor<NV>([&](auto vv) {
      constexpr int vs = decltype(vv)::value;
      const int i = vrow(vs);
      if (i < k) var[P + slab.L * i] = xa[vs];
    });
    if (l == 0) info[gi] = make_int2(pt, ratio > dec ? -level : level);
  }
}

}

template <int KP>
__global__ void __launch_bounds__(64, 2)
fill_tq40_factor_kernel(SolveConsts c, SlabDev slab, long long g0, int npts,
                        double *__restrict__ ws, double *__restrict__ aux,
                        int2 *__restrict__ info) {
  using LY = Tq40Layout<KP>;
  using FR = FactorRecord<KP>;
  using FA = FactorAux<KP>;
  constexpr int J0 = LY::J0, KT = LY::KT, NS = LY::NS;
  using SM = Tq40Smem<KP>;
  __shared__ SM sm;

  const int lane = threadIdx.x, q = lane >> 4, l = lane & 15;
  const int g4 = xcd_remap_rev(blockIdx.x, gridDim.x);
  const int gi = 4 * g4 + q;
  const bool valid = gi < npts;
  const int k = c.k;
  const int ptot = valid ? info[gi].x : 0;

  double A[NS][KP];
  double Pb[J0];
  const bool pre = l < J0;
  double ubP, ub[NS];
  tq40_load_record<KP>(ws, g4, q, l, valid, npts, A, Pb, ubP, ub);

  sfor<J0>([&](auto jj) {
    constexpr int j = decltype(jj)::value, J1 = j + 1;
    const double dj = rbcast<j>(Pb[j]);
    double alpha, u1a;
    if constexpr (J1 < J0) {
      alpha = rbcast<J1>(Pb[j]);
      u1a = rbcast<J1>(ubP);
    } else {
      alpha = rbcast<0>(A[0][j]);
      u1a = rbcast<0>(ub[0]);
    }
    const double xP = (pre && l > J1 && l < k) ? Pb[j] : 0.0;
    double x[NS];
    double xx = xP * xP, xb = xP * ubP;
    sfor<NS>([&](auto rr) {
      constexpr int r = decltype(rr)::value;
      const int i = J0 + l + 16 * r;
      x[r] = (i > J1 && i < k) ? A[r][j] : 0.0;
      xx = fma(x[r], x[r], xx);
      xb = fma(x[r], ub[r], xb);
    });
    rsum16x2(xx, xb);
    auto src_of = [&](auto cc, const double &vp, const double (&vs)[NS]) -> const double & {
      constexpr int col = decltype(cc)::value;
      if constexpr (col < J0) return vp;
      else return vs[(col - J0) / 16];
    };
    auto lane_of = [](int col) { return col < J0 ? col : (col - J0) % 16; };
    const Refl h = dlarfg(alpha, xx);
    sm.tq[q][j][0] = dj;
    sm.tq[q][J1][1] = h.beta;
    sm.tau[q][j] = h.tau;
    const double tau = h.tau;
    const double xsP = xP * h.scal;
    double vP = (pre && l == J1) ? 1.0 : xsP;
    double v[NS];
    sm.pv[q][j][(pre && l > 1) ? l : 1] = xP;
    sfor<NS>([&](auto rr) {
      constexpr int r = decltype(rr)::value;
      const double xs = x[r] * h.scal;
      if constexpr (J1 == J0 && r == 0) v[r] = l == 0 ? 1.0 : xs;
      else v[r] = xs;
      sm.pv[q][j][J0 + l + 16 * r] = x[r];
    });
    sm.pv[q][j][0] = h.scal;
    const double s3 = fma(h.scal, xb, u1a);
    ubP = fma(-tau * s3, vP, ubP);
    sfor<NS>([&](auto rr) {
      constexpr int r = decltype(rr)::value;
      ub[r] = fma(-tau * s3, v[r], ub[r]);
    });
    dpp_pin(vP);
    sfor<NS>([&](auto rr) { dpp_pin(v[decltype(rr)::value]); });
    double pa[kNA][NS], pP = 0.0;
    sfor<kNA * NS>([&](auto ii) { pa[decltype(ii)::value / NS][decltype(ii)::value % NS] = 0.0; });
    sfor<KP - J1>([&](auto cc) {
      constexpr int col = J1 + decltype(cc)::value;
      constexpr int LC = lane_of(col);
      const double &vs = src_of(std::integral_constant<int, col>{}, vP, v);
      sfor<NS>([&](auto rr) {
        constexpr int r = decltype(rr)::value;
        constexpr int a = (col - J1) % kNA;
        pa[a][r] = fmac_row<LC>(pa[a][r], vs, A[r][col]);
      });
      if constexpr (col < J0) pP = fmac_row<LC>(pP, vs, Pb[col]);
    });
    if constexpr (J1 < J0) {
      constexpr int NC = J0 - J1, CH = 3;
      sfor<(NC + CH - 1) / CH>([&](auto kk) {
        constexpr int c0 = J1 + CH * decltype(kk)::value;
        constexpr int n = J0 - c0 < CH ? J0 - c0 : CH;
        double cs[n];
        sfor<n>([&](auto cc) {
          constexpr int col = c0 + decltype(cc)::value;
          double s = 0.0;
          sfor<NS>([&](auto rr) {
            constexpr int r = decltype(rr)::value;
            s = fma(A[r][col], v[r], s);
          });
          cs[decltype(cc)::value] = s;
        });
        rsum16xN(cs);
        sfor<n>([&](auto cc) {
          constexpr int col = c0 + decltype(cc)::value;
          pP += l == col ? cs[decltype(cc)::value] : 0.0;
        });
      });
    }
    double pp[NS];
    double sp = vP * pP;
    sfor<NS>([&](auto rr) {
      constexpr int r = decltype(rr)::value;
      pp[r] = acc_sum(pa, r);
      sp = fma(v[r], pp[r], sp);
    });
    const double s1 = tau * rsum16(sp);
    const double wP = fma(-0.5 * tau * s1, vP, tau * pP);
    double wv[NS];
    sfor<NS>([&](auto rr) {
      constexpr int r = decltype(rr)::value;
      wv[r] = fma(-0.5 * tau * s1, v[r], tau * pp[r]);
    });
    double wPp = wP;
    dpp_pin(wPp);
    sfor<NS>([&](auto rr) { dpp_pin(wv[decltype(rr)::value]); });
    sfor<(KP - J1 + kUG - 1) / kUG>([&](auto pp) {
      constexpr int c0 = J1 + kUG * decltype(pp)::value;
      sfor<2>([&](auto hh) {
        constexpr int h = decltype(hh)::value;
        sfor<kUG>([&](auto ee) {
          constexpr int col = c0 + decltype(ee)::value;
          if constexpr (col < KP) {
            constexpr int LC = lane_of(col);
            const double &vs = src_of(std::integral_constant<int, col>{}, vP, v);
            const double &ws = src_of(std::integral_constant<int, col>{}, wPp, wv);
            sfor<NS>([&](auto rr) {
              constexpr int r = decltype(rr)::value;
              if constexpr (h == 0) A[r][col] = fnmac_row<LC>(A[r][col], vs, wv[r]);
              else A[r][col] = fnmac_row<LC>(A[r][col], ws, v[r]);
            });
            if constexpr (col < J0) {
              if constexpr (h == 0) Pb[col] = fnmac_row<LC>(Pb[col], vs, wPp);
              else Pb[col] = fnmac_row<LC>(Pb[col], ws, vP);
            }
          }
        });
      });
// ... 11 lines not shown
      const double alpha = rbcast<L1>(A[R1][j]);
      double x[NS], xx = 0.0, xb = 0.0;
      sfor<NS>([&](auto rr) {
        constexpr int r = decltype(rr)::value;
        if constexpr (16 * r + 15 > J1) {
          const int i = J0 + l + 16 * r;
          x[r] = (i > j + 1 && i < k) ? A[r][j] : 0.0;
          xx = fma(x[r], x[r], xx);
          xb = fma(x[r], ub[r], xb);
        } else {
          x[r] = 0.0;
        }
      });
      rsum16x2(xx, xb);
      const Refl h = dlarfg(alpha, xx);
      const double tau = h.tau;
      sm.tq[q][j][0] = dj;
      sm.tq[q][j + 1][1] = h.beta;
      sm.tau[q][j] = tau;
      double v[NS];
      sfor<NS>([&](auto rr) {
        constexpr int r = decltype(rr)::value;
        const int t = l + 16 * r;
        const double xs = x[r] * h.scal;
        v[r] = t == J1 ? 1.0 : xs;
        if constexpr (r == R1) A[r][j] = t == J1 ? h.scal : x[r];
        else if constexpr (16 * r + 15 > J1) A[r][j] = x[r];
      });
      const double s3 = fma(h.scal, xb, rbcast<L1>(ub[R1]));
      sfor<NS>([&](auto rr) {
        constexpr int r = decltype(rr)::value;
        ub[r] = fma(-tau * s3, v[r], ub[r]);
      });
      double pa[kNA][NS];
      sfor<kNA * NS>([&](auto ii) { pa[decltype(ii)::value / NS][decltype(ii)::value % NS] = 0.0; });
      sfor<NS>([&](auto rr) { dpp_pin(v[decltype(rr)::value]); });
      sfor<KT - J1>([&](auto cc) {
        constexpr int cl = J1 + decltype(cc)::value;
        sfor<NS>([&](auto rr) {
          constexpr int r = decltype(rr)::value;
          if constexpr (16 * r + 15 > jl) {
            constexpr int a = (cl - J1) % kNA;
            pa[a][r] = fmac_row<cl % 16>(pa[a][r], v[cl / 16], A[r][J0 + cl]);
          }
        });
      });
      double pp[NS], sp = 0.0;
      sfor<NS>([&](auto rr) {
        constexpr int r = decltype(rr)::value;
        pp[r] = acc_sum(pa, r);
        if constexpr (16 * r + 15 > jl) sp = fma(v[r], pp[r], sp);
      });
      const double s1 = tau * rsum16(sp);
      double wv[NS];
      sfor<NS>([&](auto rr) {
        constexpr int r = decltype(rr)::value;
        wv[r] = fma(-0.5 * tau * s1, v[r], tau * pp[r]);
      });
      sfor<NS>([&](auto rr) { dpp_pin(wv[decltype(rr)::value]); });
      sfor<(KT - J1 + kUG - 1) / kUG>([&](auto pp) {
        constexpr int c0 = J1 + kUG * decltype(pp)::value;
        sfor<2>([&](auto hh) {
          constexpr int h = decltype(hh)::value;
          sfor<kUG>([&](auto ee) {
            constexpr int cl = c0 + decltype(ee)::value;
            if constexpr (cl < KT) {
              sfor<NS>([&](auto rr) {
                constexpr int r = decltype(rr)::value;
                if constexpr (16 * r + 15 > jl) {
                  if constexpr (h == 0)
                    A[r][J0 + cl] = fnmac_row<cl % 16>(A[r][J0 + cl], v[cl / 16], wv[r]);
                  else
                    A[r][J0 + cl] = fnmac_row<cl % 16>(A[r][J0 + cl], wv[cl / 16], v[r]);
                }
              });
            }
          });
        });
      });
    } else {
      const double ej = rbcast<LJ>(A[RJ][j - 1]);
      sm.tq[q][j][0] = dj;
      if constexpr (jl == KT - 1) sm.tq[q][j][1] = ej;
    }
  });
  sfor<NS>([&](auto rr) {
    constexpr int r = decltype(rr)::value;
    const int i = J0 + l + 16 * r;
    sm.tq[q][i][2] = ub[r];
  });
  if (l == 0) {
    sm.tq[q][0][1] = 0.0;
    sm.tq[q][KP][1] = 0.0;
  }
  __syncthreads();

  if (valid) {
    const unsigned wb = (unsigned)gi * (unsigned)FR::WORDS;
    auto st = [&](unsigned w, double x) { gst(ws, 8u * (wb + w), x); };
    sfor<(KP + 15) / 16>([&](auto rr) {
      constexpr int r = decltype(rr)::value;
      const int i = l + 16 * r;
      if (16 * r + 15 < KP || i < KP) st((unsigned)(FR::D + i), sm.tq[q][i][0]);
    });
    if (pre) st((unsigned)(FR::U1 + l), ubP);
    sfor<NS>([&](auto rr) {
      constexpr int r = decltype(rr)::value;
      st((unsigned)(FR::U1 + J0 + l + 16 * r), ub[r]);
    });
    sfor<J0>([&](auto jj) {
      constexpr int j = decltype(jj)::value, J1 = j + 1;
      const double *pj = sm.pv[q][j];
      if (pre && l >= J1) st((unsigned)(FR::col(j) + l - J1), pj[l == J1 ? 0 : l]);
      sfor<NS>([&](auto rr) {
        constexpr int r = decltype(rr)::value;
        const int i = J0 + l + 16 * r;
        if constexpr (J1 == J0 && r == 0) st((unsigned)(FR::col(j) + i - J1), pj[l == 0 ? 0 : i]);
        else st((unsigned)(FR::col(j) + i - J1), pj[i]);
      });
    });
    sfor<KT - 2>([&](auto jj) {
      constexpr int jl = decltype(jj)::value, j = J0 + jl, J1 = jl + 1;
      sfor<NS>([&](auto rr) {
        constexpr int r = decltype(rr)::value;
        if constexpr (16 * r + 15 >= J1) {
          const int t = l + 16 * r;
          if (t >= J1) st((unsigned)(FR::col(j) + t - J1), A[r][j]);
        }
      });
    });
    if (l == 0) st((unsigned)FR::EL, 0.0);
    const unsigned ab = (unsigned)gi * (unsigned)FA::WORDS;
    sfor<(KP + 15) / 16>([&](auto rr) {
      constexpr int r = decltype(rr)::value;
      const int i = l + 16 * r;
      if (16 * r + 15 < KP || i < KP) {
        gst(aux, 8u * (ab + (unsigned)(FA::B + i)), sm.tq[q][i][1]);
        const double tj = sm.tau[q][i < KP - 2 ? i : 0];
        gst(aux, 8u * (ab + (unsigned)(FA::T + i)), i < KP - 2 ? tj : 0.0);
      }
    });
  }

  float xv[LY::NV];
  tq40_load_xb<KP>(slab, g0, valid, gi, l, k, xv);
  tq40_factor_solve<KP, false>(c, slab, sm, A, xv, g0, valid, ptot, gi, q, l, info);
}

template <int KP>
__global__ void __launch_bounds__(64, 2)
solve_tq40_factor_kernel(SolveConsts c, SlabDev slab, long long g0, int npts,
                         const double *__restrict__ ws, const double *__restrict__ aux,
                         int2 *__restrict__ info) {
  using LY = Tq40Layout<KP>;
  using FR = FactorRecord<KP>;
  using FA = FactorAux<KP>;
  constexpr int J0 = LY::J0, KT = LY::KT, NS = LY::NS;
  using SM = Tq40Smem<KP>;
  __shared__ SM sm;

  const int lane = threadIdx.x, q = lane >> 4, l = lane & 15;
  const int g4 = xcd_remap_rev(blockIdx.x, gridDim.x);
  const int gi = 4 * g4 + q;
  const bool valid = gi < npts;
  const int ptot = valid ? info[gi].x : 0;
  const bool pre = l < J0;

  const __amdgpu_buffer_rsrc_t rs = rec_rsrc(ws + (size_t)(4 * g4) * FR::WORDS, 4 * FR::WORDS);
  const unsigned rq = (unsigned)(valid ? q : npts - 4 * g4) * (unsigned)FR::WORDS;
  auto rw = [&](unsigned vword, unsigned cword) {
    const unsigned cb = 8u * cword;
    const auto v = __builtin_amdgcn_raw_buffer_load_b64(rs, (int)(8u * vword + (cb & 4095u)),
                                                        (int)(cb & ~4095u), 0);
    return __longlong_as_double(((long long)v[1] << 32) | (unsigned)v[0]);
  };
  auto rwb = [&](unsigned vbyte, unsigned cword) {
    const unsigned cb = 8u * cword;
    const auto v = __builtin_amdgcn_raw_buffer_load_b64(rs, (int)(vbyte + (cb & 4095u)),
                                                        (int)(cb & ~4095u), 0);
    return __longlong_as_double(((long long)v[1] << 32) | (unsigned)v[0]);
  };
  const unsigned rl = rq + (unsigned)l;
  double dg[(KP + 15) / 16];
  sfor<(KP + 15) / 16>([&](auto rr) {
    constexpr int r = decltype(rr)::value;
    const int i = l + 16 * r;
    dg[r] = rw(rq + (unsigned)(i < KP ? i : 0), (unsigned)FR::D);
  });
  double ubP, ub[NS];
  {
    const double b = rw(rq + (unsigned)(pre ? l : 0), (unsigned)FR::U1);
    ubP = pre ? b : 0.0;
  }
  sfor<NS>([&](auto rr) {
    constexpr int r = decltype(rr)::value;
    ub[r] = rw(rl, (unsigned)(FR::U1 + J0 + 16 * r));
  });
  const __amdgpu_buffer_rsrc_t ra = rec_rsrc(aux + (size_t)(4 * g4) * FA::WORDS, 4 * FA::WORDS);
  const unsigned aq = (unsigned)(valid ? q : npts - 4 * g4) * (unsigned)FA::WORDS;
  constexpr int NA = (KP + 15) / 16;
  static_assert(16 * (NA - 1) + 8 == KP, "the last run of an aux half is half a row");
  const int l2 = l < 8 ? l + 16 * (NA - 1) : l + 16 * (NA - 2);
  auto arow = [&](int r) { return r < NA - 1 ? l + 16 * r : l2; };
  double bt[NA], ta[NA];
  sfor<NA>([&](auto rr) {
    constexpr int r = decltype(rr)::value;
    const unsigned off = 8u * (aq + (unsigned)arow(r));
    const auto vb = __builtin_amdgcn_raw_buffer_load_b64(ra, (int)(off + 8u * FA::B), 0, 0);
    const auto vt = __builtin_amdgcn_raw_buffer_load_b64(ra, (int)(off + 8u * FA::T), 0, 0);
    bt[r] = __longlong_as_double(((long long)vb[1] << 32) | (unsigned)vb[0]);
    ta[r] = __longlong_as_double(((long long)vt[1] << 32) | (unsigned)vt[0]);
  });
  double A[NS][KP];
  double c1P[J0], c1[J0][NS];
  sfor<J0>([&](auto jj) {
    constexpr int j = decltype(jj)::value, J1 = j + 1;
    c1P[j] = rw(rq + (unsigned)((pre && l > J1) ? l - J1 : 0), (unsigned)FR::col(j));
    sfor<NS>([&](auto rr) {
      constexpr int r = decltype(rr)::value;
      if constexpr (J1 == J0 && r == 0)
        c1[j][r] = rwb(rec_off(l != 0, (int)rl), (unsigned)(FR::col(j) + J0 + 16 * r - J1));
      else
        c1[j][r] = rw(rl, (unsigned)(FR::col(j) + J0 + 16 * r - J1));
    });
  });
  float xv[LY::NV];
  tq40_load_xb<KP>(slab, g0, valid, gi, l, c.k, xv);
  sfor<KT - 2>([&](auto jj) {
    constexpr int jl = decltype(jj)::value, j = J0 + jl, J1 = jl + 1;
    sfor<NS>([&](auto rr) {
      constexpr int r = decltype(rr)::value;
      if constexpr (16 * r >= J1) {
        A[r][j] = rw(rl, (unsigned)(FR::col(j) + 16 * r - J1));
      } else if constexpr (16 * r + 15 >= J1) {
        const int t = l + 16 * r;
        A[r][j] = rwb(rec_off(t >= J1, (int)rq + t - J1), (unsigned)FR::col(j));
      }
    });
  });

  sfor<(KP + 15) / 16>([&](auto rr) {
    constexpr int r = decltype(rr)::value;
    const int i = l + 16 * r;
    sm.tq[q][i < KP ? i : KP][0] = dg[r];
  });
  sm.tq[q][pre ? l : KP][2] = ubP;
  sfor<NS>([&](auto rr) {
    constexpr int r = decltype(rr)::value;
    sm.tq[q][J0 + l + 16 * r][2] = ub[r];
  });
  sfor<NA>([&](auto rr) {
    constexpr int r = decltype(rr)::value;
    sm.tq[q][arow(r)][1] = bt[r];
    sm.tau[q][arow(r)] = ta[r];
  });
  sm.tq[q][KP][1] = 0.0;

  sfor<J0>([&](auto jj) {
    constexpr int j = decltype(jj)::value, J1 = j + 1;
    sm.pv[q][j][(pre && l > J1) ? l : 0] = c1P[j];
    sfor<NS>([&](auto rr) {
      constexpr int r = decltype(rr)::value;
      sm.pv[q][j][J0 + l + 16 * r] = c1[j][r];
    });
  });
  __syncthreads();

  tq40_factor_solve<KP, true>(c, slab, sm, A, xv, g0, valid, ptot, gi, q, l, info);
}

hipError_t launch_fill_tq40_factor(hipStream_t s, int kp, SolveConsts c, SlabDev slab,
                                   long long g0, int npts, double *ws, double *aux, int2 *info) {
  if (npts <= 0) return hipSuccess;
  if (c.quad_r == nullptr || aux == nullptr || kp != kTq4KP) return hipErrorInvalidValue;
  const dim3 grid((npts + 3) / 4);
  hipLaunchKernelGGL((fill_tq40_factor_kernel<kTq4KP>), grid, dim3(64), 0, s, c, slab, g0, npts,
                     ws, aux, info);
  return hipGetLastError();
}

hipError_t launch_solve_tq40_factor(hipStream_t s, int kp, SolveConsts c, SlabDev slab,
                                    long long g0, int npts, const double *ws, const double *aux,
                                    int2 *info) {
  if (npts <= 0) return hipSuccess;
  if (c.quad_r == nullptr || aux == nullptr || kp != kTq4KP) return hipErrorInvalidValue;
  const dim3 grid((npts + 3) / 4);
  hipLaunchKernelGGL((solve_tq40_factor_kernel<kTq4KP>), grid, dim3(64), 0, s, c, slab, g0, npts,
                     ws, aux, info);
  return hipGetLastError();
}

}
```

cwbnwp-letkf_amd/cwbl/abi.py:

```python
import ctypes as C
import os

import numpy as np

ABI_VERSION = 2
MAX_NVAR = 5
NUM_GTS_TYPES = 29
NUM_RADAR_TYPES = 4
MAX_MEMBERS = 128

GTS_SOUND, GTS_SYNOP, GTS_GPSPW, GTS_METAR, GTS_SHIPS = 1, 2, 8, 10, 11
RADAR_DBZ, RADAR_VR, RADAR_ZDR, RADAR_KDP = 1, 2, 3, 4
MEM_HOST, MEM_DEVICE = 0, 1
Q1_REPLICATE, Q1_PER_TYPE = 0, 1

GTS_NVAR = {GTS_SOUND: 4, GTS_SYNOP: 5, GTS_GPSPW: 1, GTS_METAR: 5, GTS_SHIPS: 5}

OPT_SOLVER, OPT_SPLIT40, OPT_SPLIT40_BATCH, OPT_SEARCH = 1, 2, 3, 5
OPT_BIG_PATH, OPT_BIG_BATCH, OPT_PAGEABLE, OPT_BIN_DIV, OPT_LEAD_DIV, OPT_MAX_BATCH = 6, 7, 8, 9, 10, 11
OPT_INFO_WINDOW, OPT_INDEX, OPT_RECORD_REUSE = 12, 13, 14
OPT_COLUMN_SHARE, OPT_COLUMN_LEVELS, OPT_FACTOR_REUSE = 15, 16, 17
OPTIONS = {"solver": OPT_SOLVER, "split40": OPT_SPLIT40, "split40_batch": OPT_SPLIT40_BATCH,
           "search": OPT_SEARCH,
           "big_path": OPT_BIG_PATH, "big_batch": OPT_BIG_BATCH, "pageable": OPT_PAGEABLE,
           "bin_div": OPT_BIN_DIV, "lead_div": OPT_LEAD_DIV, "max_batch": OPT_MAX_BATCH,
           "info_window": OPT_INFO_WINDOW, "index": OPT_INDEX,
           "record_reuse": OPT_RECORD_REUSE, "column_share": OPT_COLUMN_SHARE,
           "column_levels": OPT_COLUMN_LEVELS, "factor_reuse": OPT_FACTOR_REUSE}

(COLUMN_SHARED, COLUMN_REASON_OFF, COLUMN_REASON_3D, COLUMN_REASON_Q1, COLUMN_REASON_NZ,
 COLUMN_REASON_PATH, COLUMN_REASON_GROUP, COLUMN_REASON_NO_TREES) = range(8)

ERRORS = {1: "CWBL_ERR_ARG", 2: "CWBL_ERR_STATE", 3: "CWBL_ERR_NO_DEVICE", 4: "CWBL_ERR_HIP",
          5: "CWBL_ERR_UNSUPPORTED", 6: "CWBL_ERR_OOM"}


class InitParams(C.Structure):
    _fields_ = [("nmember", C.c_int), ("device", C.c_int), ("weight_function", C.c_int),
                ("norain_value", C.c_float), ("q1_mode", C.c_int), ("reserved", C.c_int),
                ("workspace_bytes", C.c_size_t)]


class GtsObs(C.Structure):
    _fields_ = [("type_id", C.c_int), ("nvar", C.c_int), ("nobs", C.c_int),
                ("reserved", C.c_int), ("xyz", C.c_void_p), ("obs", C.c_void_p),
                ("error", C.c_void_p), ("hdxb", C.c_void_p), ("qc", C.c_void_p)]


class RadarObs(C.Structure):
    _fields_ = [("type_id", C.c_int), ("nobs", C.c_int), ("xyz", C.c_void_p),
                ("obs", C.c_void_p), ("hdxb", C.c_void_p)]


class ObsSet(C.Structure):
    _fields_ = [("n_gts", C.c_int), ("n_radar", C.c_int), ("gts", C.POINTER(GtsObs)),
                ("radar", C.POINTER(RadarObs)), ("memory", C.c_int), ("reserved", C.c_int)]


class TypeParams(C.Structure):
    _fields_ = [("use_it", C.c_int), ("max_lz_pts", C.c_int), ("hclr", C.c_float),
                ("vclr", C.c_float), ("err_muti", C.c_float * MAX_NVAR),
                ("err_rej", C.c_float * MAX_NVAR), ("is_assim", C.c_int * MAX_NVAR)]


class VarParams(C.Structure):
    _fields_ = [("multi_infl", C.c_float), ("use_rtpp", C.c_int), ("rtpp_alpha", C.c_float),
                ("use_rtps", C.c_int), ("rtps_alpha", C.c_float), ("tune_q", C.c_int),
                ("gts", TypeParams * NUM_GTS_TYPES), ("radar", TypeParams * NUM_RADAR_TYPES)]


class Slab(C.Structure):
    _fields_ = [("nx", C.c_int), ("ny", C.c_int), ("nz", C.c_int), ("alt_nx", C.c_int),
                ("alt_ny", C.c_int), ("ix_lim", C.c_int), ("iy_lim", C.c_int),
                ("memory", C.c_int), ("x", C.c_void_p), ("y", C.c_void_p),
                ("alt", C.c_void_p), ("var", C.c_void_p)]


class Stats(C.Structure):
    _fields_ = [("points", C.c_longlong), ("solved", C.c_longlong), ("nobs_sum", C.c_longlong),
                ("lz_truncated", C.c_longlong), ("nonconverged", C.c_longlong),
                ("q1_undefined", C.c_longlong), ("sweeps_sum", C.c_longlong),
                ("max_p", C.c_int), ("max_sweeps", C.c_int),
                ("ntrees", C.c_int), ("reserved", C.c_int), ("ms_total", C.c_double),
                ("ms_prep", C.c_double), ("ms_search", C.c_double), ("ms_solve", C.c_double),
                ("ms_copy", C.c_double)]

    def as_dict(self):
        return {name: getattr(self, name) for name, _ in self._fields_ if name != "reserved"}


class KernelTime(C.Structure):
    _fields_ = [("name", C.c_char * 64), ("launches", C.c_longlong), ("points", C.c_longlong),
                ("ms", C.c_double)]


class BinGrid(C.Structure):
    _fields_ = [("x0", C.c_float), ("y0", C.c_float), ("z0", C.c_float), ("binv", C.c_float),
                ("nbx", C.c_int), ("nby", C.c_int), ("nbz", C.c_int), ("div", C.c_int)]


class PrepInfo(C.Structure):
    _fields_ = [("trees_built", C.c_int), ("bins_built", C.c_int), ("bins_on_device", C.c_int),
                ("flagged_batches", C.c_int), ("ms_tree", C.c_double), ("ms_bins", C.c_double),
                ("ms_columns", C.c_double), ("ms_tree_wait", C.c_double)]

    def as_dict(self):
        return {name: getattr(self, name) for name, _ in self._fields_}


class ReuseInfo(C.Structure):
    _fields_ = [("batches_reused", C.c_longlong), ("batches_assembled", C.c_longlong),
                ("bytes_held", C.c_longlong), ("ms_compare", C.c_double)]

    def as_dict(self):
        return {name: getattr(self, name) for name, _ in self._fields_}


class ColumnInfo(C.Structure):
    _fields_ = [("shared", C.c_int), ("reason", C.c_int), ("columns", C.c_longlong),
                ("levels", C.c_int), ("levels_per_wave", C.c_int), ("chunk_launches", C.c_int),
                ("reserved", C.c_int)]

    def as_dict(self):
        return {name: getattr(self, name) for name, _ in self._fields_ if name != "reserved"}


EXPORTS = ["cwbl_init", "cwbl_set_stream", "cwbl_set_obs", "cwbl_analyze_var", "cwbl_analyze_vars",
           "cwbl_solve_batch", "cwbl_search",
           "cwbl_pack_columns", "cwbl_unpack_columns", "cwbl_pack_members",
           "cwbl_unpack_members", "cwbl_vcoord_mean", "cwbl_member_sum", "cwbl_scale", "cwbl_set_kernel_timing", "cwbl_kernel_times",
           "cwbl_set_option", "cwbl_bin_index", "cwbl_prep_info", "cwbl_reuse_info",
           "cwbl_column_info", "cwbl_finalize", "cwbl_last_error", "cwbl_abi_version"]


def _ptr(a):
    if a is None:
        return None
    if isinstance(a, int):
        return a
    if hasattr(a, "data_ptr"):
        return a.data_ptr()
    return a.ctypes.data


def _f4(a):
    return np.ascontiguousarray(a, dtype=np.float32)


def check_array(a, kind, memory, name):
    want = {"f4": np.float32, "i4": np.int32}[kind]
    if memory == MEM_HOST:
        if not isinstance(a, np.ndarray):
            raise TypeError(f"{name}: MEM_HOST needs a numpy array, got {type(a).__name__}")
        if a.dtype != want:
            raise TypeError(f"{name}: dtype {a.dtype}, expected {np.dtype(want)}")
        if not a.flags.c_contiguous:
            raise ValueError(f"{name}: not C-contiguous")
    elif memory == MEM_DEVICE:
        if not hasattr(a, "data_ptr") or not getattr(a, "is_cuda", False):
            raise TypeError(f"{name}: MEM_DEVICE needs a device tensor, got {type(a).__name__}")
        if str(a.dtype) != f"torch.{np.dtype(want).name}":
            raise TypeError(f"{name}: dtype {a.dtype}, expected torch.{np.dtype(want).name}")
        if not a.is_contiguous():
            raise ValueError(f"{name}: not contiguous")
    else:
        raise ValueError(f"{name}: memory must be MEM_HOST or MEM_DEVICE, got {memory}")


def _i4(a):
    return np.ascontiguousarray(a, dtype=np.int32)


class ObsSetBuilder:

    def __init__(self, memory=MEM_HOST):
        self.memory = memory
        self.gts, self.radar, self._keep = [], [], []

    def _hold(self, a, conv, name):
        if self.memory == MEM_HOST:
            a = conv(a)
# ... 277 lines not shown
```

include/cwb_letkf_core.h:

```cpp
#ifndef CWB_LETKF_CORE_H
#define CWB_LETKF_CORE_H

#include <stddef.h>

#ifdef __cplusplus
extern "C" {
#endif

#define CWBL_ABI_VERSION 2

#define CWBL_MAX_NVAR        5
#define CWBL_NUM_GTS_TYPES  29
#define CWBL_NUM_RADAR_TYPES 4
#define CWBL_MAX_MEMBERS    128

enum {
  CWBL_GTS_SOUND = 1, CWBL_GTS_SYNOP = 2, CWBL_GTS_GPSPW = 8,
  CWBL_GTS_METAR = 10, CWBL_GTS_SHIPS = 11
};
enum { CWBL_RADAR_DBZ = 1, CWBL_RADAR_VR = 2, CWBL_RADAR_ZDR = 3, CWBL_RADAR_KDP = 4 };

enum { CWBL_MEM_HOST = 0, CWBL_MEM_DEVICE = 1 };

enum {
// ... 8 lines not shown

enum { CWBL_Q1_REPLICATE = 0, CWBL_Q1_PER_TYPE = 1 };

typedef struct cwbl_init_params {
  int    nmember;
  int    device;
  int    weight_function;
  float  norain_value;
  int    q1_mode;
  int    reserved;
  size_t workspace_bytes;
} cwbl_init_params;

typedef struct cwbl_gts_obs {
  int          type_id;
  int          nvar;
  int          nobs;
  int          reserved;
  const float *xyz;
  const float *obs;
  const float *error;
  const float *hdxb;
  const int   *qc;
} cwbl_gts_obs;

typedef struct cwbl_radar_obs {
  int          type_id;
  int          nobs;
  const float *xyz;
  const float *obs;
  const float *hdxb;
} cwbl_radar_obs;

typedef struct cwbl_obs_set {
  int                   n_gts;
  int                   n_radar;
  const cwbl_gts_obs   *gts;
  const cwbl_radar_obs *radar;
  int                   memory;
  int                   reserved;
} cwbl_obs_set;

typedef struct cwbl_type_params {
  int   use_it;
  int   max_lz_pts;
  float hclr;
  float vclr;
  float err_muti[CWBL_MAX_NVAR];
  float err_rej[CWBL_MAX_NVAR];
  int   is_assim[CWBL_MAX_NVAR];
} cwbl_type_params;

typedef struct cwbl_var_params {
  float multi_infl;
  int   use_rtpp;
  float rtpp_alpha;
  int   use_rtps;
  float rtps_alpha;
  int   tune_q;
  cwbl_type_params gts[CWBL_NUM_GTS_TYPES];
  cwbl_type_params radar[CWBL_NUM_RADAR_TYPES];
} cwbl_var_params;

typedef struct cwbl_slab {
  int          nx, ny, nz;
  int          alt_nx, alt_ny;
  int          ix_lim, iy_lim;
  int          memory;
  const float *x;
  const float *y;
  const float *alt;
  float       *var;
} cwbl_slab;

typedef struct cwbl_stats {
  long long points;
  long long solved;
  long long nobs_sum;
  long long lz_truncated;
  long long nonconverged;
  long long q1_undefined;
  long long sweeps_sum;
  int       max_p;
  int       max_sweeps;
  int       ntrees;
  int       reserved;
  double    ms_total;
  double    ms_prep;
  double    ms_search;
  double    ms_solve;
  double    ms_copy;
} cwbl_stats;

int         cwbl_init(const cwbl_init_params *params);
int         cwbl_set_stream(void *stream);
int         cwbl_set_obs(const cwbl_obs_set *obs);
int         cwbl_analyze_var(const cwbl_var_params *vp, const cwbl_slab *slab,
                             cwbl_stats *stats );

#define CWBL_MAX_GROUP_VARS 8
int         cwbl_analyze_vars(int nvar, const cwbl_var_params *vp ,
                              const cwbl_slab *slabs ,
                              cwbl_stats *stats );

int         cwbl_solve_batch(int npts, const long long *col_off, const float *yo,
                             const float *yb, const float *xb, float inflat,
                             int use_rtpp, float rtpp_alpha, int use_rtps, float rtps_alpha,
                             float *xa, double *evals, int memory);

int         cwbl_search(int nobs, const float *obs_xyz, float hclr, float vclr,
                        int max_lz_pts, int nq, const float *q_xyz,
                        int *nfound, int *idx, float *r2, int memory);


int         cwbl_pack_columns(const float *global, int nx, int ny, int nz, int px, int py,
                              float *send);
int         cwbl_unpack_columns(const float *recv, int nx, int ny, int nz, int px, int py,
                                float *global);
int         cwbl_pack_members(const float *global, long long gstride, int nm, int nx, int ny,
                              int nz, int px, int py, float *send, long long sstride);
int         cwbl_unpack_members(const float *recv, long long rstride, int nm, int nx, int ny,
                                int nz, int px, int py, float *global, long long gstride);
int         cwbl_vcoord_mean(const float *ph, long long n2d, int nz_ph, int k, int stagger,
                             float g, float *alt);

int         cwbl_member_sum(const float *fields, long long n, int nm, float *out);
int         cwbl_scale(float *x, long long n, float alpha);

typedef struct cwbl_kernel_time {
  char      name[64];
  long long launches;
  long long points;
  double    ms;
} cwbl_kernel_time;
int         cwbl_set_kernel_timing(int enable);
int         cwbl_kernel_times(cwbl_kernel_time *out, int cap, int *n);

enum {
  CWBL_OPT_SOLVER = 1,
  CWBL_OPT_SPLIT40 = 2,
  CWBL_OPT_SPLIT40_BATCH = 3,
  CWBL_OPT_SEARCH = 5,
  CWBL_OPT_BIG_PATH = 6,
  CWBL_OPT_BIG_BATCH = 7,
  CWBL_OPT_PAGEABLE = 8,
  CWBL_OPT_BIN_DIV = 9,
  CWBL_OPT_LEAD_DIV = 10,
  CWBL_OPT_MAX_BATCH = 11,
  CWBL_OPT_INFO_WINDOW = 12,
  CWBL_OPT_INDEX = 13,
  CWBL_OPT_RECORD_REUSE = 14,
  CWBL_OPT_COLUMN_SHARE = 15,
  CWBL_OPT_COLUMN_LEVELS = 16,
  CWBL_OPT_FACTOR_REUSE = 17
};
int         cwbl_set_option(int option, long long value);

typedef struct cwbl_bin_grid {
  float x0, y0, z0, binv;
  int   nbx, nby, nbz;
  int   div;
} cwbl_bin_grid;
int         cwbl_bin_index(int nobs, const float *obs_xyz, float hclr, float vclr, int div,
                           cwbl_bin_grid *grid, long long start_cap, int *start, int *order,
                           int memory);

typedef struct cwbl_prep_info_t {
  int    trees_built;
  int    bins_built;
  int    bins_on_device;
  int    flagged_batches;
  double ms_tree;
  double ms_bins;
  double ms_columns;
  double ms_tree_wait;
} cwbl_prep_info_t;
int         cwbl_prep_info(cwbl_prep_info_t *out);

typedef struct cwbl_reuse_info_t {
  long long batches_reused;
  long long batches_assembled;
  long long bytes_held;
  double    ms_compare;
} cwbl_reuse_info_t;
int         cwbl_reuse_info(cwbl_reuse_info_t *out);

enum {
  CWBL_COLUMN_SHARED = 0,
  CWBL_COLUMN_REASON_OFF = 1,
  CWBL_COLUMN_REASON_3D = 2,
  CWBL_COLUMN_REASON_Q1 = 3,
  CWBL_COLUMN_REASON_NZ = 4,
  CWBL_COLUMN_REASON_PATH = 5,
  CWBL_COLUMN_REASON_GROUP = 6,
  CWBL_COLUMN_REASON_NO_TREES = 7
};
typedef struct cwbl_column_info_t {
  int       shared;
  int       reason;
  long long columns;
  int       levels;
  int       levels_per_wave;
  int       chunk_launches;
  int       reserved;
} cwbl_column_info_t;
int         cwbl_column_info(cwbl_column_info_t *out);

int         cwbl_finalize(void);
const char *cwbl_last_error(void);
int         cwbl_abi_version(void);

#ifdef __cplusplus
}
#endif

#endif
```

Measured before the change: 434.1 million.

## Merge cached-factor hit batches into one multi-segment solve launch

When the record cache fully hits, consecutive cached batches are described as segments in a device table, and a single 2D-grid kernel solves all of them instead of one launch per batch. The first non-cached batch's search is issued before the merged solve so it can overlap with it. The shared per-block solve body is moved into a header so both kernels reuse it. This cuts per-batch launch and event overhead, at the cost of an extra small H2D copy and idle blocks in segments shorter than the longest one.

New measurement: 452.0 million (median of 6 runs). 1.04x the previous value.

```diff
diff --git a/cwbnwp-letkf_amd/csrc/cwbl_abi.hip b/cwbnwp-letkf_amd/csrc/cwbl_abi.hip
--- a/cwbnwp-letkf_amd/csrc/cwbl_abi.hip
+++ b/cwbnwp-letkf_amd/csrc/cwbl_abi.hip
@@ -288,6 +288,9 @@
   unsigned long long gen = 0;
   size_t reuse_budget = 0;
   bool factor_reuse = true;
+  bool hit_merge = true;
+  DevBuf hitseg;
+  PinBuf hitseg_pin;
   int column_share = 0;
   int column_levels = 0;
   int ncu = 0;
@@ -843,9 +846,10 @@
                     &S.sy, &S.salt, &S.svar, &S.bcol, &S.byo, &S.byb, &S.bxb, &S.bxa, &S.bev, &S.btri,
                     &S.qxyz, &S.qnf, &S.qidx, &S.qr2, &S.quad, &S.wsa, &S.flags, &S.tdesc_tree,
                     &S.ix_keys[0], &S.ix_keys[1], &S.ix_vals[0], &S.ix_vals[1], &S.ix_hist,
-                    &S.ix_part})
+                    &S.ix_part, &S.hitseg})
     b->release();
   S.ix_pin.release();
+  S.hitseg_pin.release();
   S.cache.release();
   for (hipEvent_t e : S.pevents) (void)hipEventDestroy(e);
   S.pevents.clear();
@@ -930,6 +934,8 @@
   int reuse = 0;
   long long ncached = 0;
   bool full_hit = false;
+  bool merge = false;
+  size_t hitseg_used = 0;
   int colshare = 0, nlev = 1, lev = 1;
   long long ncol = 0;
   SlabDev full{};
@@ -1227,7 +1233,8 @@
   const TreeDesc *dtrees = S.tdesc.as<TreeDesc>();
   DevStats *dst = S.stats.as<DevStats>();
   hipStream_t ss = S.serial_search ? S.stream : S.sstream;
-  if (bi >= 2) HIPCHK(hipStreamWaitEvent(ss, S.events[v.done_ev[bi - 2]], 0));
+  if (bi >= 2 && bi - 2 < (long long)v.done_ev.size())
+    HIPCHK(hipStreamWaitEvent(ss, S.events[v.done_ev[bi - 2]], 0));
   HIPCHK(hipEventRecord(a, ss));
   int kt;
   if (S.binned) {
@@ -1678,6 +1685,7 @@
   S.column_share = 0;
   S.column_levels = 0;
   S.factor_reuse = true;
+  S.hit_merge = true;
   S.ncu = prop.multiProcessorCount;
   std::memset(&P, 0, sizeof P);
   std::memset(&CI, 0, sizeof CI);
@@ -1698,6 +1706,13 @@
 int cwbl_set_option(int option, long long value) {
   if (!S.inited) return fail(CWBL_ERR_STATE, "cwbl_set_option before cwbl_init");
   auto range = [&](long long lo, long long hi) { return value >= lo && value <= hi; };
+  if (option == CWBL_OPT_HIT_MERGE) {
+    if (!range(0, 1))
+      return fail(CWBL_ERR_ARG, "cwbl_set_option: value %lld out of range for option %d", value,
+                  option);
+    S.hit_merge = value == 1;
+    return CWBL_OK;
+  }
   ++S.gen;
   switch (option) {
     case CWBL_OPT_SOLVER:
@@ -1923,6 +1938,60 @@
   return CWBL_OK;
 }
 
+static long long hit_segments(int nb, long long *Bs_out = nullptr) {
+  const long long cap = std::min<long long>(S.tq4_sub > 0 ? S.tq4_sub : nb, 1 << 19);
+  const long long Bs = std::min<long long>(sub_batch(nb, cap), 1 << 19);
+  if (Bs_out) *Bs_out = Bs;
+  return Bs >= nb ? 1 : (nb + Bs - 1) / Bs;
+}
+
+static int plan_hit_merge(VarCall &v) {
+  v.merge = S.hit_merge && v.reuse == 2 && S.factor_reuse && !v.group && !v.colshare &&
+            !v.piped && !v.piped_back && !v.bounce && v.ncached > 0;
+  if (!v.merge) return CWBL_OK;
+  long long nseg = 0;
+  for (long long bi = 0; bi < v.ncached; ++bi) nseg += hit_segments(v.plan[bi].second);
+  if (nseg > 65535) {
+    v.merge = false;
+    return CWBL_OK;
+  }
+  HIPCHK(S.hitseg.ensure((size_t)nseg * sizeof(HitSeg)));
+  HIPCHK(S.hitseg_pin.ensure((size_t)nseg * sizeof(HitSeg)));
+  return CWBL_OK;
+}
+
+static int solve_hits_merged(VarCall &v, long long b0, long long b1, hipEvent_t b2,
+                             hipEvent_t dn) {
+  RecordCache &C = S.cache;
+  HitSeg *const hseg = S.hitseg_pin.as<HitSeg>() + v.hitseg_used;
+  int nseg = 0, maxns = 0;
+  long long pts = 0;
+  for (long long bi = b0; bi < b1; ++bi) {
+    const long long g0 = v.plan[bi].first;
+    const int nb = v.plan[bi].second;
+    const long long ord = (long long)(C.off[bi] / AsmRecord<kTq4KP>::WORDS);
+    long long Bs;
+    hit_segments(nb, &Bs);
+    for (long long s0 = 0; s0 < nb; s0 += Bs) {
+      const int ns = (int)std::min<long long>(Bs, nb - s0);
+      hseg[nseg++] = HitSeg{g0 + s0, ord + s0, ns, (int)(g0 + s0 - v.win0)};
+      maxns = std::max(maxns, ns);
+    }
+    pts += nb;
+  }
+  HitSeg *const dseg = S.hitseg.as<HitSeg>() + v.hitseg_used;
+  HIPCHK(hipMemcpyAsync(dseg, hseg, (size_t)nseg * sizeof(HitSeg), hipMemcpyHostToDevice,
+                        S.stream));
+  v.hitseg_used += (size_t)nseg;
+  HIPCHK(hipEventRecord(b2, S.stream));
+  if (S.ktiming) S.kpend.push_back({KT_SOLVE_TQ40_FACTOR, b2, dn, pts});
+  HIPCHK(launch_solve_tq40_factor_merged(S.stream, S.kp, v.c, v.sd, dseg, nseg, maxns,
+                                         C.rec.as<double>(), C.aux.as<double>(),
+                                         S.info.as<int2>()));
+  HIPCHK(hipEventRecord(dn, S.stream));
+  return CWBL_OK;
+}
+
 static int analyze_call(VarCall &v, cwbl_stats *stats) {
   const cwbl_var_params *vp = v.vp;
   const cwbl_slab *sl = v.sl;
@@ -2020,12 +2089,15 @@
   if (int rc = alloc_call_buffers(v)) return rc;
   if (reuse_on && v.reuse != 2)
     if (int rc = begin_fill(v, key)) return rc;
+  if (int rc = plan_hit_merge(v)) return rc;
   if (int rc = restore_info(v, 0)) return rc;
   HIPCHK(event(3, &e_ready));
   HIPCHK(hipEventRecord(e_ready, S.stream));
   HIPCHK(hipStreamWaitEvent(S.sstream, e_ready, 0));
 
   const long long nbat = (long long)v.plan.size();
+  long long searched = -1;
+  hipEvent_t searched_ev = nullptr;
   for (long long bi = 0; bi < nbat; ++bi) {
     const long long g0 = v.plan[bi].first;
     const int nb = v.plan[bi].second;
@@ -2050,9 +2122,30 @@
         crec ? C.off[bi] / AsmRecord<kTq4KP>::WORDS * FactorAux<kTq4KP>::WORDS : 0;
     double *const caux = crec && S.factor_reuse ? C.aux.as<double>() + aoff : nullptr;
     const bool hit = crec && v.reuse == 2;
+    if (hit && v.merge) {
+      long long be = bi + 1;
+      while (be < v.ncached && v.plan[be].first + v.plan[be].second - v.win0 <= v.info_cap) ++be;
+      if (be == v.ncached && be < nbat) {
+        int *const nc = (be & 1) ? S.nbr_cnt2.as<int>() : S.nbr_cnt.as<int>();
+        int *const ni = (be & 1) ? S.nbr_idx2.as<int>() : S.nbr_idx.as<int>();
+        if (int rc = search_batch(v, be, nc, ni, a, b)) return rc;
+        v.search_ev.push_back({ev, ev + 1});
+        searched = be;
+        searched_ev = b;
+      }
+      if (int rc = solve_hits_merged(v, bi, be, b2, dn)) return rc;
+      v.solve_ev.push_back({ev + 2, ev + 3});
+      for (long long bj = bi; bj < be; ++bj) v.done_ev.push_back(ev + 3);
+      v.ev += 4;
+      bi = be - 1;
+      continue;
+    }
     if (!hit) {
-      if (int rc = search_batch(v, bi, ncnt, nidx, a, b)) return rc;
-      HIPCHK(hipStreamWaitEvent(S.stream, b, 0));
+      if (bi != searched) {
+        if (int rc = search_batch(v, bi, ncnt, nidx, a, b)) return rc;
+        searched_ev = b;
+      }
+      HIPCHK(hipStreamWaitEvent(S.stream, searched_ev, 0));
     }
     if (v.piped)
       if (int rc = upload_batch_var(v, bi)) return rc;
@@ -2072,7 +2165,7 @@
       if (v.piped_back && bi >= State::kSlots - 1)
         if (int rc = bounce_drain(v, bi - (State::kSlots - 1))) return rc;
     }
-    if (!hit) v.search_ev.push_back({ev, ev + 1});
+    if (!hit && bi != searched) v.search_ev.push_back({ev, ev + 1});
     v.solve_ev.push_back({ev + 2, ev + 3});
     v.done_ev.push_back(ev + 3);
     v.ev += 4;
diff --git a/cwbnwp-letkf_amd/csrc/cwbl_internal.h b/cwbnwp-letkf_amd/csrc/cwbl_internal.h
--- a/cwbnwp-letkf_amd/csrc/cwbl_internal.h
+++ b/cwbnwp-letkf_amd/csrc/cwbl_internal.h
@@ -213,6 +213,16 @@
                                     long long g0, int npts, const double *ws, const double *aux,
                                     int2 *info);
 
+struct HitSeg {
+  long long g0;
+  long long ord;
+  int ns;
+  int info;
+};
+hipError_t launch_solve_tq40_factor_merged(hipStream_t s, int kp, SolveConsts c, SlabDev slab,
+                                           const HitSeg *seg, int nseg, int maxns,
+                                           const double *ws, const double *aux, int2 *info);
+
 constexpr int kMaxGroupVars = 8;
 struct Tq40Vars {
   float *var[kMaxGroupVars];
diff --git a/cwbnwp-letkf_amd/csrc/cwbl_tq40_factor.h b/cwbnwp-letkf_amd/csrc/cwbl_tq40_factor.h
--- /dev/null
+++ b/cwbnwp-letkf_amd/csrc/cwbl_tq40_factor.h
@@ -0,0 +1,502 @@
+#pragma once
+
+#include "cwbl_tq40_common.h"
+
+#include <utility>
+
+namespace cwbl {
+
+namespace {
+
+__device__ __forceinline__ void rsum16x2(double &a, double &b) {
+  double ab[2] = {a, b};
+  rsum16xN(ab);
+  a = ab[0];
+  b = ab[1];
+}
+
+__device__ __forceinline__ void touch(double &x) { asm volatile("" : "+v"(x)); }
+__device__ __forceinline__ int touched(int x) {
+  asm volatile("" : "+v"(x));
+  return x;
+}
+__device__ __forceinline__ long long touched(long long x) {
+  asm volatile("" : "+v"(x));
+  return x;
+}
+
+template <int KP>
+__device__ __forceinline__ void tq40_load_xb(const SlabDev &slab, const long long g0,
+                                             const bool valid, const int gi, const int l,
+                                             const int k, float (&xv)[Tq40Layout<KP>::NV]) {
+  const float *__restrict__ const var = slab.var;
+  const long long P = tq40_var_index(slab, g0, valid ? gi : 0);
+  sfor<Tq40Layout<KP>::NV>([&](auto vv) {
+    constexpr int vs = decltype(vv)::value;
+    const int i = tq40_vrow<KP>(l, vs);
+    xv[vs] = var[P + slab.L * ((valid && i < k) ? i : 0)];
+  });
+}
+
+template <int KP, bool AHEAD>
+__device__ __forceinline__ void tq40_factor_solve(
+    const SolveConsts &c, const SlabDev &slab, Tq40Smem<KP> &sm,
+    double (&A)[Tq40Layout<KP>::NS][KP], const float (&xbv)[Tq40Layout<KP>::NV], const long long g0,
+    const bool valid, const int ptot, const int gi, const int q, const int l,
+    int2 *__restrict__ info) {
+  using LY = Tq40Layout<KP>;
+  constexpr int J0 = LY::J0, KT = LY::KT, NS = LY::NS, NV = LY::NV, H = LY::H;
+  using SM = Tq40Smem<KP>;
+  const int k = c.k;
+  const int lp = l < J0 ? l : 0;
+  const bool pre = l < J0;
+  auto vrow = [&](int vs) { return tq40_vrow<KP>(l, vs); };
+  int *const pkeep = reinterpret_cast<int *>(&sm.tq[q][KP][3]);
+  *pkeep = ptot;
+  const double trace = tq40_trace(sm, q, l, k);
+
+  const double m = (double)c.inflat;
+  const double ratio = trace / m - (double)(k - 1);
+  int level = 1;
+  double dec = 10.0;
+  while (level < kQuadLevels && dec < ratio) {
+    dec *= 10.0;
+    ++level;
+  }
+  const int R = tq40_wave_rounds(level);
+  const int NQ = 8 * R - 1;
+  const double2 *qtab = quad_rule(c.quad_r, R, level);
+  double2 twn;
+  if constexpr (AHEAD) twn = qtab[min(l & 7, NQ - 1)];
+  const int side = l >> 3, n8 = l & 7;
+  const double(*T)[4] = sm.tq[q];
+  char *const smb = reinterpret_cast<char *>(&sm);
+  auto lds = [&](unsigned off) { return *reinterpret_cast<const double *>(smb + off); };
+  auto sts = [&](unsigned off, double v) { *reinterpret_cast<double *>(smb + off) = v; };
+  const unsigned tq0 = (unsigned)(offsetof(SM, tq) + (size_t)q * sizeof(sm.tq[0])) +
+                       (side ? (KP - 1) * 32u : 0u);
+  const unsigned dirb = side ? (unsigned)-32 : 32u;
+  const unsigned csb = side ? 40u : 8u;
+  const unsigned qs0 = (unsigned)(offsetof(SM, qs) + (size_t)q * sizeof(sm.qs[0])) +
+                       (side ? (KP - H) * 8u : (H - 1) * 8u);
+  const unsigned qz0 = (unsigned)(offsetof(SM, qz) + (size_t)q * sizeof(sm.qz[0]));
+  const unsigned bdir = side ? 8u : (unsigned)-8;
+  const double sk = sqrt((double)(k - 1));
+  auto touch_cols = [&]() {
+    sfor<KT - 2>([&](auto jj) {
+      constexpr int jl = decltype(jj)::value, J1 = jl + 1, R1 = J1 / 16;
+      sfor<NS>([&](auto rr) {
+        constexpr int r = decltype(rr)::value;
+        if constexpr (16 * r + 15 > J1 || r == R1) touch(A[r][J0 + jl]);
+      });
+    });
+  };
+
+  float *__restrict__ const var = slab.var;
+  const int use_rtpp = c.use_rtpp, use_rtps = c.use_rtps;
+  const float rtpp_alpha = c.rtpp_alpha, rtps_alpha = c.rtps_alpha;
+
+  float xbl[NV];
+  double xb_mean;
+  {
+    sfor<NV>([&](auto vv) {
+      constexpr int vs = decltype(vv)::value;
+      const bool mem = valid && vrow(vs) < k;
+      xbl[vs] = mem ? xbv[vs] : 0.0f;
+    });
+    xb_mean = (double)(seq_sum_f32<KP>(xbl) * c.nmember_inv);
+  }
+  double uxP = pre && l < k ? (double)xbl[0] - xb_mean : 0.0, ux[NS];
+  sfor<NS>([&](auto rr) {
+    constexpr int r = decltype(rr)::value;
+    const int t = J0 + l + 16 * r;
+    ux[r] = t < k ? (double)xbl[r + 1] - xb_mean : 0.0;
+  });
+
+  sfor<J0>([&](auto jj) {
+    constexpr int j = decltype(jj)::value, J1 = j + 1;
+    const double *pj = sm.pv[q][j];
+    const double scal = pj[0], tau = sm.tau[q][j];
+    double u2a;
+    if constexpr (J1 < J0) u2a = rbcast<J1>(uxP);
+    else u2a = rbcast<0>(ux[0]);
+    const double xP = (pre && l > J1) ? pj[lp] : 0.0;
+    double x[NS], xu = xP * uxP;
+    sfor<NS>([&](auto rr) {
+      constexpr int r = decltype(rr)::value;
+      x[r] = pj[J0 + l + 16 * r];
+      xu = fma(x[r], ux[r], xu);
+    });
+    xu = rsum16(xu);
+    const double xsP = xP * scal;
+    const double vP = (pre && l == J1) ? 1.0 : xsP;
+    const double s2 = fma(scal, xu, u2a);
+    uxP = fma(-tau * s2, vP, uxP);
+    sfor<NS>([&](auto rr) {
+      constexpr int r = decltype(rr)::value;
+      const double xs = x[r] * scal;
+      double vr;
+      if constexpr (J1 == J0 && r == 0) vr = l == 0 ? 1.0 : xs;
+      else vr = xs;
+      ux[r] = fma(-tau * s2, vr, ux[r]);
+    });
+  });
+  sfor<KT - 2>([&](auto jj) {
+    constexpr int jl = decltype(jj)::value, j = J0 + jl;
+    constexpr int J1 = jl + 1, R1 = J1 / 16, L1 = J1 % 16;
+    sfor<NS>([&](auto rr) {
+      constexpr int r = decltype(rr)::value;
+      if constexpr (16 * r + 15 > J1 || r == R1) touch(A[r][j]);
+    });
+    const double scal = rbcast<L1>(A[R1][j]), tau = sm.tau[q][j];
+    double x[NS], xu = 0.0;
+    sfor<NS>([&](auto rr) {
+      constexpr int r = decltype(rr)::value;
+      if constexpr (16 * r + 15 > J1) {
+        const int t = l + 16 * r;
+        if constexpr (r == R1) x[r] = t == J1 ? 0.0 : A[r][j];
+        else x[r] = A[r][j];
+        xu = fma(x[r], ux[r], xu);
+      } else {
+        x[r] = 0.0;
+      }
+    });
+    xu = rsum16(xu);
+    const double s2 = fma(scal, xu, rbcast<L1>(ux[R1]));
+    sfor<NS>([&](auto rr) {
+      constexpr int r = decltype(rr)::value;
+      const int t = l + 16 * r;
+      const double xs = x[r] * scal;
+      const double vr = t == J1 ? 1.0 : xs;
+      ux[r] = fma(-tau * s2, vr, ux[r]);
+    });
+  });
+  if (pre) sm.tq[q][l][3] = uxP;
+  sfor<NS>([&](auto rr) {
+    constexpr int r = decltype(rr)::value;
+    sm.tq[q][J0 + l + 16 * r][3] = ux[r];
+  });
+  __syncthreads();
+
+  double ys[NV], z[NV];
+  sfor<NV>([&](auto vv) { ys[decltype(vv)::value] = 0.0; });
+  for (int round = 0; round < R; ++round) {
+    const int node = 8 * round + n8;
+    double2 tw;
+    if constexpr (AHEAD) {
+      tw = twn;
+      if (round + 1 < R) twn = qtab[min(node + 8, NQ - 1)];
+    } else {
+      tw = qtab[min(node, NQ - 1)];
+    }
+    const double sigma = node < NQ ? m * tw.x : 0.0;
+    const double omega = node < NQ ? sqrt(m) * tw.y : 1.0;
+    double hh[H], mm[H];
+    unsigned pw = tq0;
+    double dl = lds(pw) + sigma, gt = lds(pw + 24);
+    double nd, nc, ng;
+    auto next_row = [&]() {
+      pw += dirb;
+      nd = lds(pw);
+      nc = lds(pw + csb);
+      ng = lds(pw + 24);
+    };
+    if constexpr (AHEAD) next_row();
+    sfor<H - 1>([&](auto tt) {
+      constexpr int t = decltype(tt)::value + 1;
+      if constexpr (!AHEAD) {
+        asm volatile("" : "+v"(pw) : "v"(dl));
+        next_row();
+      }
+      const double dt = nd, ct = nc, g = ng;
+      if constexpr (AHEAD && t < H - 1) {
+        asm volatile("" : "+v"(pw) : "v"(dl));
+        next_row();
+      }
+      const double rdl = rcp64(dl);
+      const double lt = ct * rdl;
+      hh[t - 1] = gt * rdl;
+      mm[t - 1] = lt;
+      dl = fma(-lt, ct, dt + sigma);
+      gt = fma(-lt, gt, g);
+    });
+    const double cm = T[H][1];
+    const double dlo = ror8(dl), go = ror8(gt);
+    double xv = (gt * dlo - cm * go) / fma(dl, dlo, -cm * cm);
+    const bool last = round == R - 1;
+    const bool zlane = last && n8 == 7;
+    const double om = zlane ? 0.0 : omega;
+    unsigned ps = qs0;
+    unsigned pz = qz0 + (zlane ? qs0 - (unsigned)offsetof(SM, qs) - (unsigned)q * KP * 8u
+                               : KP * 8u);
+    const unsigned zdir = zlane ? bdir : 0u;
+    auto emit = [&](double x) {
+      double s = om * x;
+      s += dpp_f64<0xB1>(s);
+      s += dpp_f64<0x4E>(s);
+      s += dpp_f64<0x141>(s);
+      sts(ps, s);
+      sts(pz, x);
+    };
+    emit(xv);
+    sfor<H - 1>([&](auto tt) {
+      constexpr int t = H - 2 - decltype(tt)::value;
+      xv = fma(-mm[t], xv, hh[t]);
+      ps += bdir;
+      pz += zdir;
+      asm volatile("" : "+v"(ps), "+v"(pz) : "v"(xv));
+      emit(xv);
+    });
+    __syncthreads();
+    sfor<NV>([&](auto vv) {
+      constexpr int vs = decltype(vv)::value;
+      const int i = vrow(vs);
+      const int ic = i < KP ? i : 0;
+      ys[vs] += i < KP ? sm.qs[q][ic] : 0.0;
+      if (last) z[vs] = i < KP ? sm.qz[q][ic] : 0.0;
+    });
+    __syncthreads();
+  }
+  double dpart = 0.0;
+  sfor<NV>([&](auto vv) {
+    constexpr int vs = decltype(vv)::value;
+    const int i = vrow(vs);
+    const double u1 = sm.tq[q][i < KP ? i : 0][2];
+    dpart = i < KP ? fma(u1, z[vs], dpart) : dpart;
+  });
+  const double d = rsum16(dpart);
+
+  double y[NV];
+  sfor<NV>([&](auto vv) { y[decltype(vv)::value] = ys[decltype(vv)::value]; });
+  touch_cols();
+  const int lb = touched(l);
+  sfor<KT - 2>([&](auto jj) {
+    constexpr int jl = KT - 3 - decltype(jj)::value, j = J0 + jl, J1 = jl + 1;
+    constexpr int R1 = J1 / 16, L1 = J1 % 16;
+    const double tj = sm.tau[q][j];
+    const double scal = rbcast<L1>(A[R1][j]);
+    double vv[NS], a = 0.0;
+    sfor<NS>([&](auto rr) {
+      constexpr int r = decltype(rr)::value;
+      if constexpr (16 * r + 15 >= J1) {
+        const int t = lb + 16 * r;
+        if constexpr (16 * r + 15 > J1) vv[r] = t == J1 ? 1.0 : A[r][j] * scal;
+        else vv[r] = t == J1 ? 1.0 : 0.0;
+        a = fma(vv[r], y[r + 1], a);
+      } else {
+        vv[r] = 0.0;
+      }
+    });
+    a = rsum16(a);
+    sfor<NS>([&](auto rr) {
+      constexpr int r = decltype(rr)::value;
+      if constexpr (16 * r + 15 >= J1) y[r + 1] = fma(-tj * a, vv[r], y[r + 1]);
+    });
+  });
+  sfor<J0>([&](auto jj) {
+    constexpr int j = J0 - 1 - decltype(jj)::value, J1 = j + 1;
+    const double tj = sm.tau[q][j];
+    const double *pj = sm.pv[q][j];
+    const double scal = pj[0];
+    const double v0 = lb == J1 ? 1.0 : (lb < J0 && lb > J1) ? pj[lb] * scal : 0.0;
+    double vv[NS];
+    double a = v0 * y[0];
+    sfor<NS>([&](auto rr) {
+      constexpr int r = decltype(rr)::value;
+      const double pr = pj[J0 + lb + 16 * r] * scal;
+      if constexpr (J1 == J0 && r == 0) vv[r] = lb == 0 ? 1.0 : pr;
+      else vv[r] = pr;
+      a = fma(vv[r], y[r + 1], a);
+    });
+    a = rsum16(a);
+    y[0] = fma(-tj * a, v0, y[0]);
+    sfor<NS>([&](auto rr) {
+      constexpr int r = decltype(rr)::value;
+      y[r + 1] = fma(-tj * a, vv[r], y[r + 1]);
+    });
+  });
+
+  float xa[NV];
+  sfor<NV>([&](auto vv) {
+    constexpr int vs = decltype(vv)::value;
+    xa[vs] = vrow(vs) < k ? (float)(xb_mean + (d + sk * y[vs])) : 0.0f;
+  });
+  if (use_rtpp || use_rtps) {
+    const float xa_mean = seq_sum_f32<KP>(xa) * c.nmember_inv;
+    double xpl[NV];
+    float xap[NV];
+    sfor<NV>([&](auto vv) {
+      constexpr int vs = decltype(vv)::value;
+      const bool mem = vrow(vs) < k;
+      xpl[vs] = mem ? (double)xbl[vs] - xb_mean : 0.0;
+      xap[vs] = 0.0f;
+      if (mem) {
+        xap[vs] = xa[vs] - xa_mean;
+        if (use_rtpp)
+          xap[vs] = (float)((double)((1.0f - rtpp_alpha) * xap[vs]) +
+                            (double)rtpp_alpha * xpl[vs]);
+      }
+    });
+    if (use_rtps) {
+      double d8 = 0.0, sq8[NV];
+      sfor<NV>([&](auto vv) {
+        constexpr int vs = decltype(vv)::value;
+        sq8[vs] = xpl[vs] * xpl[vs];
+        dpp_pin(sq8[vs]);
+      });
+      sfor<KP>([&](auto mm) {
+        constexpr int mb = decltype(mm)::value;
+        constexpr int vs = mb < J0 ? 0 : 1 + (mb - J0) / 16, ln = mb < J0 ? mb : (mb - J0) % 16;
+        d8 = fmac_row<ln>(d8, sq8[vs], 1.0);
+      });
+      const float xb_std = (float)d8;
+      float sq[NV];
+      sfor<NV>([&](auto vv) {
+        constexpr int vs = decltype(vv)::value;
+        sq[vs] = xap[vs] * xap[vs];
+      });
+      const float xa_std = seq_sum_f32<KP>(sq);
+      const float f = rtps_alpha * sqrtf(xb_std / xa_std) - rtps_alpha + 1.0f;
+      sfor<NV>([&](auto vv) { xap[decltype(vv)::value] = xap[decltype(vv)::value] * f; });
+    }
+    sfor<NV>([&](auto vv) { xa[decltype(vv)::value] = xa_mean + xap[decltype(vv)::value]; });
+  }
+  const int pt = *pkeep;
+  if (valid && pt > 0) {
+    const long long P = tq40_var_index(slab, g0, touched(gi));
+    sfor<NV>([&](auto vv) {
+      constexpr int vs = decltype(vv)::value;
+      const int i = vrow(vs);
+      if (i < k) var[P + slab.L * i] = xa[vs];
+    });
+    if (l == 0) info[gi] = make_int2(pt, ratio > dec ? -level : level);
+  }
+}
+
+}
+
+template <int KP>
+__device__ __forceinline__ void tq40_factor_hit(const SolveConsts &c, const SlabDev &slab,
+                                                const long long g0,
+                                                const int npts, const double *__restrict__ ws,
+                                                const double *__restrict__ aux,
+                                                int2 *__restrict__ info, const int b,
+                                                const int nblk) {
+  using LY = Tq40Layout<KP>;
+  using FR = FactorRecord<KP>;
+  using FA = FactorAux<KP>;
+  constexpr int J0 = LY::J0, KT = LY::KT, NS = LY::NS;
+  using SM = Tq40Smem<KP>;
+  __shared__ SM sm;
+
+  const int lane = threadIdx.x, q = lane >> 4, l = lane & 15;
+  const int g4 = xcd_remap_rev(b, nblk);
+  const int gi = 4 * g4 + q;
+  const bool valid = gi < npts;
+  const int ptot = valid ? info[gi].x : 0;
+  const bool pre = l < J0;
+
+  const __amdgpu_buffer_rsrc_t rs = rec_rsrc(ws + (size_t)(4 * g4) * FR::WORDS, 4 * FR::WORDS);
+  const unsigned rq = (unsigned)(valid ? q : npts - 4 * g4) * (unsigned)FR::WORDS;
+  auto rw = [&](unsigned vword, unsigned cword) {
+    const unsigned cb = 8u * cword;
+    const auto v = __builtin_amdgcn_raw_buffer_load_b64(rs, (int)(8u * vword + (cb & 4095u)),
+                                                        (int)(cb & ~4095u), 0);
+    return __longlong_as_double(((long long)v[1] << 32) | (unsigned)v[0]);
+  };
+  auto rwb = [&](unsigned vbyte, unsigned cword) {
+    const unsigned cb = 8u * cword;
+    const auto v = __builtin_amdgcn_raw_buffer_load_b64(rs, (int)(vbyte + (cb & 4095u)),
+                                                        (int)(cb & ~4095u), 0);
+    return __longlong_as_double(((long long)v[1] << 32) | (unsigned)v[0]);
+  };
+  const unsigned rl = rq + (unsigned)l;
+  double dg[(KP + 15) / 16];
+  sfor<(KP + 15) / 16>([&](auto rr) {
+    constexpr int r = decltype(rr)::value;
+    const int i = l + 16 * r;
+    dg[r] = rw(rq + (unsigned)(i < KP ? i : 0), (unsigned)FR::D);
+  });
+  double ubP, ub[NS];
+  {
+    const double b = rw(rq + (unsigned)(pre ? l : 0), (unsigned)FR::U1);
+    ubP = pre ? b : 0.0;
+  }
+  sfor<NS>([&](auto rr) {
+    constexpr int r = decltype(rr)::value;
+    ub[r] = rw(rl, (unsigned)(FR::U1 + J0 + 16 * r));
+  });
+  const __amdgpu_buffer_rsrc_t ra = rec_rsrc(aux + (size_t)(4 * g4) * FA::WORDS, 4 * FA::WORDS);
+  const unsigned aq = (unsigned)(valid ? q : npts - 4 * g4) * (unsigned)FA::WORDS;
+  constexpr int NA = (KP + 15) / 16;
+  static_assert(16 * (NA - 1) + 8 == KP, "the last run of an aux half is half a row");
+  const int l2 = l < 8 ? l + 16 * (NA - 1) : l + 16 * (NA - 2);
+  auto arow = [&](int r) { return r < NA - 1 ? l + 16 * r : l2; };
+  double bt[NA], ta[NA];
+  sfor<NA>([&](auto rr) {
+    constexpr int r = decltype(rr)::value;
+    const unsigned off = 8u * (aq + (unsigned)arow(r));
+    const auto vb = __builtin_amdgcn_raw_buffer_load_b64(ra, (int)(off + 8u * FA::B), 0, 0);
+    const auto vt = __builtin_amdgcn_raw_buffer_load_b64(ra, (int)(off + 8u * FA::T), 0, 0);
+    bt[r] = __longlong_as_double(((long long)vb[1] << 32) | (unsigned)vb[0]);
+    ta[r] = __longlong_as_double(((long long)vt[1] << 32) | (unsigned)vt[0]);
+  });
+  double A[NS][KP];
+  double c1P[J0], c1[J0][NS];
+  sfor<J0>([&](auto jj) {
+    constexpr int j = decltype(jj)::value, J1 = j + 1;
+    c1P[j] = rw(rq + (unsigned)((pre && l > J1) ? l - J1 : 0), (unsigned)FR::col(j));
+    sfor<NS>([&](auto rr) {
+      constexpr int r = decltype(rr)::value;
+      if constexpr (J1 == J0 && r == 0)
+        c1[j][r] = rwb(rec_off(l != 0, (int)rl), (unsigned)(FR::col(j) + J0 + 16 * r - J1));
+      else
+        c1[j][r] = rw(rl, (unsigned)(FR::col(j) + J0 + 16 * r - J1));
+    });
+  });
+  float xv[LY::NV];
+  tq40_load_xb<KP>(slab, g0, valid, gi, l, c.k, xv);
+  sfor<KT - 2>([&](auto jj) {
+    constexpr int jl = decltype(jj)::value, j = J0 + jl, J1 = jl + 1;
+    sfor<NS>([&](auto rr) {
+      constexpr int r = decltype(rr)::value;
+      if constexpr (16 * r >= J1) {
+        A[r][j] = rw(rl, (unsigned)(FR::col(j) + 16 * r - J1));
+      } else if constexpr (16 * r + 15 >= J1) {
+        const int t = l + 16 * r;
+        A[r][j] = rwb(rec_off(t >= J1, (int)rq + t - J1), (unsigned)FR::col(j));
+      }
+    });
+  });
+
+  sfor<(KP + 15) / 16>([&](auto rr) {
+    constexpr int r = decltype(rr)::value;
+    const int i = l + 16 * r;
+    sm.tq[q][i < KP ? i : KP][0] = dg[r];
+  });
+  sm.tq[q][pre ? l : KP][2] = ubP;
+  sfor<NS>([&](auto rr) {
+    constexpr int r = decltype(rr)::value;
+    sm.tq[q][J0 + l + 16 * r][2] = ub[r];
+  });
+  sfor<NA>([&](auto rr) {
+    constexpr int r = decltype(rr)::value;
+    sm.tq[q][arow(r)][1] = bt[r];
+    sm.tau[q][arow(r)] = ta[r];
+  });
+  sm.tq[q][KP][1] = 0.0;
+
+  sfor<J0>([&](auto jj) {
+    constexpr int j = decltype(jj)::value, J1 = j + 1;
+    sm.pv[q][j][(pre && l > J1) ? l : 0] = c1P[j];
+    sfor<NS>([&](auto rr) {
+      constexpr int r = decltype(rr)::value;
+      sm.pv[q][j][J0 + l + 16 * r] = c1[j][r];
+    });
+  });
+  __syncthreads();
+
+  tq40_factor_solve<KP, true>(c, slab, sm, A, xv, g0, valid, ptot, gi, q, l, info);
+}
+
+}
diff --git a/cwbnwp-letkf_amd/csrc/cwbl_tq40_fill.hip b/cwbnwp-letkf_amd/csrc/cwbl_tq40_fill.hip
--- a/cwbnwp-letkf_amd/csrc/cwbl_tq40_fill.hip
+++ b/cwbnwp-letkf_amd/csrc/cwbl_tq40_fill.hip
@@ -1,377 +1,6 @@
-#include "cwbl_tq40_common.h"
-
-#include <utility>
+#include "cwbl_tq40_factor.h"
 
 namespace cwbl {
-
-namespace {
-
-__device__ __forceinline__ void rsum16x2(double &a, double &b) {
-  double ab[2] = {a, b};
-  rsum16xN(ab);
-  a = ab[0];
-  b = ab[1];
-}
-
-__device__ __forceinline__ void touch(double &x) { asm volatile("" : "+v"(x)); }
-__device__ __forceinline__ int touched(int x) {
-  asm volatile("" : "+v"(x));
-  return x;
-}
-__device__ __forceinline__ long long touched(long long x) {
-  asm volatile("" : "+v"(x));
-  return x;
-}
-
-template <int KP>
-__device__ __forceinline__ void tq40_load_xb(const SlabDev &slab, const long long g0,
-                                             const bool valid, const int gi, const int l,
-                                             const int k, float (&xv)[Tq40Layout<KP>::NV]) {
-  const float *__restrict__ const var = slab.var;
-  const long long P = tq40_var_index(slab, g0, valid ? gi : 0);
-  sfor<Tq40Layout<KP>::NV>([&](auto vv) {
-    constexpr int vs = decltype(vv)::value;
-    const int i = tq40_vrow<KP>(l, vs);
-    xv[vs] = var[P + slab.L * ((valid && i < k) ? i : 0)];
-  });
-}
-
-template <int KP, bool AHEAD>
-__device__ __forceinline__ void tq40_factor_solve(
-    const SolveConsts &c, const SlabDev &slab, Tq40Smem<KP> &sm,
-    double (&A)[Tq40Layout<KP>::NS][KP], const float (&xbv)[Tq40Layout<KP>::NV], const long long g0,
-    const bool valid, const int ptot, const int gi, const int q, const int l,
-    int2 *__restrict__ info) {
-  using LY = Tq40Layout<KP>;
-  constexpr int J0 = LY::J0, KT = LY::KT, NS = LY::NS, NV = LY::NV, H = LY::H;
-  using SM = Tq40Smem<KP>;
-  const int k = c.k;
-  const int lp = l < J0 ? l : 0;
-  const bool pre = l < J0;
-  auto vrow = [&](int vs) { return tq40_vrow<KP>(l, vs); };
-  int *const pkeep = reinterpret_cast<int *>(&sm.tq[q][KP][3]);
-  *pkeep = ptot;
-  const double trace = tq40_trace(sm, q, l, k);
-
-  const double m = (double)c.inflat;
-  const double ratio = trace / m - (double)(k - 1);
-  int level = 1;
-  double dec = 10.0;
-  while (level < kQuadLevels && dec < ratio) {
-    dec *= 10.0;
-    ++level;
-  }
-  const int R = tq40_wave_rounds(level);
-  const int NQ = 8 * R - 1;
-  const double2 *qtab = quad_rule(c.quad_r, R, level);
-  double2 twn;
-  if constexpr (AHEAD) twn = qtab[min(l & 7, NQ - 1)];
-  const int side = l >> 3, n8 = l & 7;
-  const double(*T)[4] = sm.tq[q];
-  char *const smb = reinterpret_cast<char *>(&sm);
-  auto lds = [&](unsigned off) { return *reinterpret_cast<const double *>(smb + off); };
-  auto sts = [&](unsigned off, double v) { *reinterpret_cast<double *>(smb + off) = v; };
-  const unsigned tq0 = (unsigned)(offsetof(SM, tq) + (size_t)q * sizeof(sm.tq[0])) +
-                       (side ? (KP - 1) * 32u : 0u);
-  const unsigned dirb = side ? (unsigned)-32 : 32u;
-  const unsigned csb = side ? 40u : 8u;
-  const unsigned qs0 = (unsigned)(offsetof(SM, qs) + (size_t)q * sizeof(sm.qs[0])) +
-                       (side ? (KP - H) * 8u : (H - 1) * 8u);
-  const unsigned qz0 = (unsigned)(offsetof(SM, qz) + (size_t)q * sizeof(sm.qz[0]));
-  const unsigned bdir = side ? 8u : (unsigned)-8;
-  const double sk = sqrt((double)(k - 1));
-  auto touch_cols = [&]() {
-    sfor<KT - 2>([&](auto jj) {
-      constexpr int jl = decltype(jj)::value, J1 = jl + 1, R1 = J1 / 16;
-      sfor<NS>([&](auto rr) {
-        constexpr int r = decltype(rr)::value;
-        if constexpr (16 * r + 15 > J1 || r == R1) touch(A[r][J0 + jl]);
-      });
-    });
-  };
-
-  float *__restrict__ const var = slab.var;
-  const int use_rtpp = c.use_rtpp, use_rtps = c.use_rtps;
-  const float rtpp_alpha = c.rtpp_alpha, rtps_alpha = c.rtps_alpha;
-
-  float xbl[NV];
-  double xb_mean;
-  {
-    sfor<NV>([&](auto vv) {
-      constexpr int vs = decltype(vv)::value;
-      const bool mem = valid && vrow(vs) < k;
-      xbl[vs] = mem ? xbv[vs] : 0.0f;
-    });
-    xb_mean = (double)(seq_sum_f32<KP>(xbl) * c.nmember_inv);
-  }
-  double uxP = pre && l < k ? (double)xbl[0] - xb_mean : 0.0, ux[NS];
-  sfor<NS>([&](auto rr) {
-    constexpr int r = decltype(rr)::value;
-    const int t = J0 + l + 16 * r;
-    ux[r] = t < k ? (double)xbl[r + 1] - xb_mean : 0.0;
-  });
-
-  sfor<J0>([&](auto jj) {
-    constexpr int j = decltype(jj)::value, J1 = j + 1;
-    const double *pj = sm.pv[q][j];
-    const double scal = pj[0], tau = sm.tau[q][j];
-    double u2a;
-    if constexpr (J1 < J0) u2a = rbcast<J1>(uxP);
-    else u2a = rbcast<0>(ux[0]);
-    const double xP = (pre && l > J1) ? pj[lp] : 0.0;
-    double x[NS], xu = xP * uxP;
-    sfor<NS>([&](auto rr) {
-      constexpr int r = decltype(rr)::value;
-      x[r] = pj[J0 + l + 16 * r];
-      xu = fma(x[r], ux[r], xu);
-    });
-    xu = rsum16(xu);
-    const double xsP = xP * scal;
-    const double vP = (pre && l == J1) ? 1.0 : xsP;
-    const double s2 = fma(scal, xu, u2a);
-    uxP = fma(-tau * s2, vP, uxP);
-    sfor<NS>([&](auto rr) {
-      constexpr int r = decltype(rr)::value;
-      const double xs = x[r] * scal;
-      double vr;
-      if constexpr (J1 == J0 && r == 0) vr = l == 0 ? 1.0 : xs;
-      else vr = xs;
-      ux[r] = fma(-tau * s2, vr, ux[r]);
-    });
-  });
-  sfor<KT - 2>([&](auto jj) {
-    constexpr int jl = decltype(jj)::value, j = J0 + jl;
-    constexpr int J1 = jl + 1, R1 = J1 / 16, L1 = J1 % 16;
-    sfor<NS>([&](auto rr) {
-      constexpr int r = decltype(rr)::value;
-      if constexpr (16 * r + 15 > J1 || r == R1) touch(A[r][j]);
-    });
-    const double scal = rbcast<L1>(A[R1][j]), tau = sm.tau[q][j];
-    double x[NS], xu = 0.0;
-    sfor<NS>([&](auto rr) {
-      constexpr int r = decltype(rr)::value;
-      if constexpr (16 * r + 15 > J1) {
-        const int t = l + 16 * r;
-        if constexpr (r == R1) x[r] = t == J1 ? 0.0 : A[r][j];
-        else x[r] = A[r][j];
-        xu = fma(x[r], ux[r], xu);
-      } else {
-        x[r] = 0.0;
-      }
-    });
-    xu = rsum16(xu);
-    const double s2 = fma(scal, xu, rbcast<L1>(ux[R1]));
-    sfor<NS>([&](auto rr) {
-      constexpr int r = decltype(rr)::value;
-      const int t = l + 16 * r;
-      const double xs = x[r] * scal;
-      const double vr = t == J1 ? 1.0 : xs;
-      ux[r] = fma(-tau * s2, vr, ux[r]);
-    });
-  });
-  if (pre) sm.tq[q][l][3] = uxP;
-  sfor<NS>([&](auto rr) {
-    constexpr int r = decltype(rr)::value;
-    sm.tq[q][J0 + l + 16 * r][3] = ux[r];
-  });
-  __syncthreads();
-
-  double ys[NV], z[NV];
-  sfor<NV>([&](auto vv) { ys[decltype(vv)::value] = 0.0; });
-  for (int round = 0; round < R; ++round) {
-    const int node = 8 * round + n8;
-    double2 tw;
-    if constexpr (AHEAD) {
-      tw = twn;
-      if (round + 1 < R) twn = qtab[min(node + 8, NQ - 1)];
-    } else {
-      tw = qtab[min(node, NQ - 1)];
-    }
-    const double sigma = node < NQ ? m * tw.x : 0.0;
-    const double omega = node < NQ ? sqrt(m) * tw.y : 1.0;
-    double hh[H], mm[H];
-    unsigned pw = tq0;
-    double dl = lds(pw) + sigma, gt = lds(pw + 24);
-    double nd, nc, ng;
-    auto next_row = [&]() {
-      pw += dirb;
-      nd = lds(pw);
-      nc = lds(pw + csb);
-      ng = lds(pw + 24);
-    };
-    if constexpr (AHEAD) next_row();
-    sfor<H - 1>([&](auto tt) {
-      constexpr int t = decltype(tt)::value + 1;
-      if constexpr (!AHEAD) {
-        asm volatile("" : "+v"(pw) : "v"(dl));
-        next_row();
-      }
-      const double dt = nd, ct = nc, g = ng;
-      if constexpr (AHEAD && t < H - 1) {
-        asm volatile("" : "+v"(pw) : "v"(dl));
-        next_row();
-      }
-      const double rdl = rcp64(dl);
-      const double lt = ct * rdl;
-      hh[t - 1] = gt * rdl;
-      mm[t - 1] = lt;
-      dl = fma(-lt, ct, dt + sigma);
-      gt = fma(-lt, gt, g);
-    });
-    const double cm = T[H][1];
-    const double dlo = ror8(dl), go = ror8(gt);
-    double xv = (gt * dlo - cm * go) / fma(dl, dlo, -cm * cm);
-    const bool last = round == R - 1;
-    const bool zlane = last && n8 == 7;
-    const double om = zlane ? 0.0 : omega;
-    unsigned ps = qs0;
-    unsigned pz = qz0 + (zlane ? qs0 - (unsigned)offsetof(SM, qs) - (unsigned)q * KP * 8u
-                               : KP * 8u);
-    const unsigned zdir = zlane ? bdir : 0u;
-    auto emit = [&](double x) {
-      double s = om * x;
-      s += dpp_f64<0xB1>(s);
-      s += dpp_f64<0x4E>(s);
-      s += dpp_f64<0x141>(s);
-      sts(ps, s);
-      sts(pz, x);
-    };
-    emit(xv);
-    sfor<H - 1>([&](auto tt) {
-      constexpr int t = H - 2 - decltype(tt)::value;
-      xv = fma(-mm[t], xv, hh[t]);
-      ps += bdir;
-      pz += zdir;
-      asm volatile("" : "+v"(ps), "+v"(pz) : "v"(xv));
-      emit(xv);
-    });
-    __syncthreads();
-    sfor<NV>([&](auto vv) {
-      constexpr int vs = decltype(vv)::value;
-      const int i = vrow(vs);
-      const int ic = i < KP ? i : 0;
-      ys[vs] += i < KP ? sm.qs[q][ic] : 0.0;
-      if (last) z[vs] = i < KP ? sm.qz[q][ic] : 0.0;
-    });
-    __syncthreads();
-  }
-  double dpart = 0.0;
-  sfor<NV>([&](auto vv) {
-    constexpr int vs = decltype(vv)::value;
-    const int i = vrow(vs);
-    const double u1 = sm.tq[q][i < KP ? i : 0][2];
-    dpart = i < KP ? fma(u1, z[vs], dpart) : dpart;
-  });
-  const double d = rsum16(dpart);
-
-  double y[NV];
-  sfor<NV>([&](auto vv) { y[decltype(vv)::value] = ys[decltype(vv)::value]; });
-  touch_cols();
-  const int lb = touched(l);
-  sfor<KT - 2>([&](auto jj) {
-    constexpr int jl = KT - 3 - decltype(jj)::value, j = J0 + jl, J1 = jl + 1;
-    constexpr int R1 = J1 / 16, L1 = J1 % 16;
-    const double tj = sm.tau[q][j];
-    const double scal = rbcast<L1>(A[R1][j]);
-    double vv[NS], a = 0.0;
-    sfor<NS>([&](auto rr) {
-      constexpr int r = decltype(rr)::value;
-      if constexpr (16 * r + 15 >= J1) {
-        const int t = lb + 16 * r;
-        if constexpr (16 * r + 15 > J1) vv[r] = t == J1 ? 1.0 : A[r][j] * scal;
-        else vv[r] = t == J1 ? 1.0 : 0.0;
-        a = fma(vv[r], y[r + 1], a);
-      } else {
-        vv[r] = 0.0;
-      }
-    });
-    a = rsum16(a);
-    sfor<NS>([&](auto rr) {
-      constexpr int r = decltype(rr)::value;
-      if constexpr (16 * r + 15 >= J1) y[r + 1] = fma(-tj * a, vv[r], y[r + 1]);
-    });
-  });
-  sfor<J0>([&](auto jj) {
-    constexpr int j = J0 - 1 - decltype(jj)::value, J1 = j + 1;
-    const double tj = sm.tau[q][j];
-    const double *pj = sm.pv[q][j];
-    const double scal = pj[0];
-    const double v0 = lb == J1 ? 1.0 : (lb < J0 && lb > J1) ? pj[lb] * scal : 0.0;
-    double vv[NS];
-    double a = v0 * y[0];
-    sfor<NS>([&](auto rr) {
-      constexpr int r = decltype(rr)::value;
-      const double pr = pj[J0 + lb + 16 * r] * scal;
-      if constexpr (J1 == J0 && r == 0) vv[r] = lb == 0 ? 1.0 : pr;
-      else vv[r] = pr;
-      a = fma(vv[r], y[r + 1], a);
-    });
-    a = rsum16(a);
-    y[0] = fma(-tj * a, v0, y[0]);
-    sfor<NS>([&](auto rr) {
-      constexpr int r = decltype(rr)::value;
-      y[r + 1] = fma(-tj * a, vv[r], y[r + 1]);
-    });
-  });
-
-  float xa[NV];
-  sfor<NV>([&](auto vv) {
-    constexpr int vs = decltype(vv)::value;
-    xa[vs] = vrow(vs) < k ? (float)(xb_mean + (d + sk * y[vs])) : 0.0f;
-  });
-  if (use_rtpp || use_rtps) {
-    const float xa_mean = seq_sum_f32<KP>(xa) * c.nmember_inv;
-    double xpl[NV];
-    float xap[NV];
-    sfor<NV>([&](auto vv) {
-      constexpr int vs = decltype(vv)::value;
-      const bool mem = vrow(vs) < k;
-      xpl[vs] = mem ? (double)xbl[vs] - xb_mean : 0.0;
-      xap[vs] = 0.0f;
-      if (mem) {
-        xap[vs] = xa[vs] - xa_mean;
-        if (use_rtpp)
-          xap[vs] = (float)((double)((1.0f - rtpp_alpha) * xap[vs]) +
-                            (double)rtpp_alpha * xpl[vs]);
-      }
-    });
-    if (use_rtps) {
-      double d8 = 0.0, sq8[NV];
-      sfor<NV>([&](auto vv) {
-        constexpr int vs = decltype(vv)::value;
-        sq8[vs] = xpl[vs] * xpl[vs];
-        dpp_pin(sq8[vs]);
-      });
-      sfor<KP>([&](auto mm) {
-        constexpr int mb = decltype(mm)::value;
-        constexpr int vs = mb < J0 ? 0 : 1 + (mb - J0) / 16, ln = mb < J0 ? mb : (mb - J0) % 16;
-        d8 = fmac_row<ln>(d8, sq8[vs], 1.0);
-      });
-      const float xb_std = (float)d8;
-      float sq[NV];
-      sfor<NV>([&](auto vv) {
-        constexpr int vs = decltype(vv)::value;
-        sq[vs] = xap[vs] * xap[vs];
-      });
-      const float xa_std = seq_sum_f32<KP>(sq);
-      const float f = rtps_alpha * sqrtf(xb_std / xa_std) - rtps_alpha + 1.0f;
-      sfor<NV>([&](auto vv) { xap[decltype(vv)::value] = xap[decltype(vv)::value] * f; });
-    }
-    sfor<NV>([&](auto vv) { xa[decltype(vv)::value] = xa_mean + xap[decltype(vv)::value]; });
-  }
-  const int pt = *pkeep;
-  if (valid && pt > 0) {
-    const long long P = tq40_var_index(slab, g0, touched(gi));
-    sfor<NV>([&](auto vv) {
-      constexpr int vs = decltype(vv)::value;
-      const int i = vrow(vs);
-      if (i < k) var[P + slab.L * i] = xa[vs];
-    });
-    if (l == 0) info[gi] = make_int2(pt, ratio > dec ? -level : level);
-  }
-}
-
-}
 
 template <int KP>
 __global__ void __launch_bounds__(64, 2)
@@ -689,121 +318,7 @@
 solve_tq40_factor_kernel(SolveConsts c, SlabDev slab, long long g0, int npts,
                          const double *__restrict__ ws, const double *__restrict__ aux,
                          int2 *__restrict__ info) {
-  using LY = Tq40Layout<KP>;
-  using FR = FactorRecord<KP>;
-  using FA = FactorAux<KP>;
-  constexpr int J0 = LY::J0, KT = LY::KT, NS = LY::NS;
-  using SM = Tq40Smem<KP>;
-  __shared__ SM sm;
-
-  const int lane = threadIdx.x, q = lane >> 4, l = lane & 15;
-  const int g4 = xcd_remap_rev(blockIdx.x, gridDim.x);
-  const int gi = 4 * g4 + q;
-  const bool valid = gi < npts;
-  const int ptot = valid ? info[gi].x : 0;
-  const bool pre = l < J0;
-
-  const __amdgpu_buffer_rsrc_t rs = rec_rsrc(ws + (size_t)(4 * g4) * FR::WORDS, 4 * FR::WORDS);
-  const unsigned rq = (unsigned)(valid ? q : npts - 4 * g4) * (unsigned)FR::WORDS;
-  auto rw = [&](unsigned vword, unsigned cword) {
-    const unsigned cb = 8u * cword;
-    const auto v = __builtin_amdgcn_raw_buffer_load_b64(rs, (int)(8u * vword + (cb & 4095u)),
-                                                        (int)(cb & ~4095u), 0);
-    return __longlong_as_double(((long long)v[1] << 32) | (unsigned)v[0]);
-  };
-  auto rwb = [&](unsigned vbyte, unsigned cword) {
-    const unsigned cb = 8u * cword;
-    const auto v = __builtin_amdgcn_raw_buffer_load_b64(rs, (int)(vbyte + (cb & 4095u)),
-                                                        (int)(cb & ~4095u), 0);
-    return __longlong_as_double(((long long)v[1] << 32) | (unsigned)v[0]);
-  };
-  const unsigned rl = rq + (unsigned)l;
-  double dg[(KP + 15) / 16];
-  sfor<(KP + 15) / 16>([&](auto rr) {
-    constexpr int r = decltype(rr)::value;
-    const int i = l + 16 * r;
-    dg[r] = rw(rq + (unsigned)(i < KP ? i : 0), (unsigned)FR::D);
-  });
-  double ubP, ub[NS];
-  {
-    const double b = rw(rq + (unsigned)(pre ? l : 0), (unsigned)FR::U1);
-    ubP = pre ? b : 0.0;
-  }
-  sfor<NS>([&](auto rr) {
-    constexpr int r = decltype(rr)::value;
-    ub[r] = rw(rl, (unsigned)(FR::U1 + J0 + 16 * r));
-  });
-  const __amdgpu_buffer_rsrc_t ra = rec_rsrc(aux + (size_t)(4 * g4) * FA::WORDS, 4 * FA::WORDS);
-  const unsigned aq = (unsigned)(valid ? q : npts - 4 * g4) * (unsigned)FA::WORDS;
-  constexpr int NA = (KP + 15) / 16;
-  static_assert(16 * (NA - 1) + 8 == KP, "the last run of an aux half is half a row");
-  const int l2 = l < 8 ? l + 16 * (NA - 1) : l + 16 * (NA - 2);
-  auto arow = [&](int r) { return r < NA - 1 ? l + 16 * r : l2; };
-  double bt[NA], ta[NA];
-  sfor<NA>([&](auto rr) {
-    constexpr int r = decltype(rr)::value;
-    const unsigned off = 8u * (aq + (unsigned)arow(r));
-    const auto vb = __builtin_amdgcn_raw_buffer_load_b64(ra, (int)(off + 8u * FA::B), 0, 0);
-    const auto vt = __builtin_amdgcn_raw_buffer_load_b64(ra, (int)(off + 8u * FA::T), 0, 0);
-    bt[r] = __longlong_as_double(((long long)vb[1] << 32) | (unsigned)vb[0]);
-    ta[r] = __longlong_as_double(((long long)vt[1] << 32) | (unsigned)vt[0]);
-  });
-  double A[NS][KP];
-  double c1P[J0], c1[J0][NS];
-  sfor<J0>([&](auto jj) {
-    constexpr int j = decltype(jj)::value, J1 = j + 1;
-    c1P[j] = rw(rq + (unsigned)((pre && l > J1) ? l - J1 : 0), (unsigned)FR::col(j));
-    sfor<NS>([&](auto rr) {
-      constexpr int r = decltype(rr)::value;
-      if constexpr (J1 == J0 && r == 0)
-        c1[j][r] = rwb(rec_off(l != 0, (int)rl), (unsigned)(FR::col(j) + J0 + 16 * r - J1));
-      else
-        c1[j][r] = rw(rl, (unsigned)(FR::col(j) + J0 + 16 * r - J1));
-    });
-  });
-  float xv[LY::NV];
-  tq40_load_xb<KP>(slab, g0, valid, gi, l, c.k, xv);
-  sfor<KT - 2>([&](auto jj) {
-    constexpr int jl = decltype(jj)::value, j = J0 + jl, J1 = jl + 1;
-    sfor<NS>([&](auto rr) {
-      constexpr int r = decltype(rr)::value;
-      if constexpr (16 * r >= J1) {
-        A[r][j] = rw(rl, (unsigned)(FR::col(j) + 16 * r - J1));
-      } else if constexpr (16 * r + 15 >= J1) {
-        const int t = l + 16 * r;
-        A[r][j] = rwb(rec_off(t >= J1, (int)rq + t - J1), (unsigned)FR::col(j));
-      }
-    });
-  });
-
-  sfor<(KP + 15) / 16>([&](auto rr) {
-    constexpr int r = decltype(rr)::value;
-    const int i = l + 16 * r;
-    sm.tq[q][i < KP ? i : KP][0] = dg[r];
-  });
-  sm.tq[q][pre ? l : KP][2] = ubP;
-  sfor<NS>([&](auto rr) {
-    constexpr int r = decltype(rr)::value;
-    sm.tq[q][J0 + l + 16 * r][2] = ub[r];
-  });
-  sfor<NA>([&](auto rr) {
-    constexpr int r = decltype(rr)::value;
-    sm.tq[q][arow(r)][1] = bt[r];
-    sm.tau[q][arow(r)] = ta[r];
-  });
-  sm.tq[q][KP][1] = 0.0;
-
-  sfor<J0>([&](auto jj) {
-    constexpr int j = decltype(jj)::value, J1 = j + 1;
-    sm.pv[q][j][(pre && l > J1) ? l : 0] = c1P[j];
-    sfor<NS>([&](auto rr) {
-      constexpr int r = decltype(rr)::value;
-      sm.pv[q][j][J0 + l + 16 * r] = c1[j][r];
-    });
-  });
-  __syncthreads();
-
-  tq40_factor_solve<KP, true>(c, slab, sm, A, xv, g0, valid, ptot, gi, q, l, info);
+  tq40_factor_hit<KP>(c, slab, g0, npts, ws, aux, info, blockIdx.x, gridDim.x);
 }
 
 hipError_t launch_fill_tq40_factor(hipStream_t s, int kp, SolveConsts c, SlabDev slab,
diff --git a/cwbnwp-letkf_amd/csrc/cwbl_tq40_hit_merge.hip b/cwbnwp-letkf_amd/csrc/cwbl_tq40_hit_merge.hip
--- /dev/null
+++ b/cwbnwp-letkf_amd/csrc/cwbl_tq40_hit_merge.hip
@@ -0,0 +1,31 @@
+#include "cwbl_tq40_factor.h"
+
+namespace cwbl {
+
+template <int KP>
+__global__ void __launch_bounds__(64, 2)
+solve_tq40_factor_merged_kernel(SolveConsts c, SlabDev slab, const HitSeg *__restrict__ seg,
+                                const double *__restrict__ ws, const double *__restrict__ aux,
+                                int2 *__restrict__ info) {
+  const HitSeg sg = seg[blockIdx.y];
+  const int nblk = (sg.ns + 3) >> 2;
+  if ((int)blockIdx.x >= nblk) return;
+  tq40_factor_hit<KP>(c, slab, sg.g0, sg.ns, ws + (size_t)sg.ord * FactorRecord<KP>::WORDS,
+                      aux + (size_t)sg.ord * FactorAux<KP>::WORDS, info + sg.info, blockIdx.x,
+                      nblk);
+}
+
+hipError_t launch_solve_tq40_factor_merged(hipStream_t s, int kp, SolveConsts c, SlabDev slab,
+                                           const HitSeg *seg, int nseg, int maxns,
+                                           const double *ws, const double *aux, int2 *info) {
+  if (nseg <= 0 || maxns <= 0) return hipSuccess;
+  if (c.quad_r == nullptr || aux == nullptr || seg == nullptr || kp != kTq4KP || nseg > 65535 ||
+      maxns > (1 << 19))
+    return hipErrorInvalidValue;
+  const dim3 grid((maxns + 3) / 4, nseg);
+  hipLaunchKernelGGL((solve_tq40_factor_merged_kernel<kTq4KP>), grid, dim3(64), 0, s, c, slab,
+                     seg, ws, aux, info);
+  return hipGetLastError();
+}
+
+}
diff --git a/cwbnwp-letkf_amd/cwbl/abi.py b/cwbnwp-letkf_amd/cwbl/abi.py
--- a/cwbnwp-letkf_amd/cwbl/abi.py
+++ b/cwbnwp-letkf_amd/cwbl/abi.py
@@ -19,14 +19,15 @@
 OPT_SOLVER, OPT_SPLIT40, OPT_SPLIT40_BATCH, OPT_SEARCH = 1, 2, 3, 5
 OPT_BIG_PATH, OPT_BIG_BATCH, OPT_PAGEABLE, OPT_BIN_DIV, OPT_LEAD_DIV, OPT_MAX_BATCH = 6, 7, 8, 9, 10, 11
 OPT_INFO_WINDOW, OPT_INDEX, OPT_RECORD_REUSE = 12, 13, 14
-OPT_COLUMN_SHARE, OPT_COLUMN_LEVELS, OPT_FACTOR_REUSE = 15, 16, 17
+OPT_COLUMN_SHARE, OPT_COLUMN_LEVELS, OPT_FACTOR_REUSE, OPT_HIT_MERGE = 15, 16, 17, 18
 OPTIONS = {"solver": OPT_SOLVER, "split40": OPT_SPLIT40, "split40_batch": OPT_SPLIT40_BATCH,
            "search": OPT_SEARCH,
            "big_path": OPT_BIG_PATH, "big_batch": OPT_BIG_BATCH, "pageable": OPT_PAGEABLE,
            "bin_div": OPT_BIN_DIV, "lead_div": OPT_LEAD_DIV, "max_batch": OPT_MAX_BATCH,
            "info_window": OPT_INFO_WINDOW, "index": OPT_INDEX,
            "record_reuse": OPT_RECORD_REUSE, "column_share": OPT_COLUMN_SHARE,
-           "column_levels": OPT_COLUMN_LEVELS, "factor_reuse": OPT_FACTOR_REUSE}
+           "column_levels": OPT_COLUMN_LEVELS, "factor_reuse": OPT_FACTOR_REUSE,
+           "hit_merge": OPT_HIT_MERGE}
 
 (COLUMN_SHARED, COLUMN_REASON_OFF, COLUMN_REASON_3D, COLUMN_REASON_Q1, COLUMN_REASON_NZ,
  COLUMN_REASON_PATH, COLUMN_REASON_GROUP, COLUMN_REASON_NO_TREES) = range(8)
diff --git a/include/cwb_letkf_core.h b/include/cwb_letkf_core.h
--- a/include/cwb_letkf_core.h
+++ b/include/cwb_letkf_core.h
@@ -184,7 +184,8 @@
   CWBL_OPT_RECORD_REUSE = 14,
   CWBL_OPT_COLUMN_SHARE = 15,
   CWBL_OPT_COLUMN_LEVELS = 16,
-  CWBL_OPT_FACTOR_REUSE = 17
+  CWBL_OPT_FACTOR_REUSE = 17,
+  CWBL_OPT_HIT_MERGE = 18
 };
 int         cwbl_set_option(int option, long long value);
 
```
